# pangenome/smoothxg

Hardware: AMD Instinct MI355X
Metric: POA blocks/sec (+ DP cells/sec) on 1000-block synthetic (higher is better)
Workload: dtype int16

## Files before the change

### include/sxg_poa.h

```cpp
#ifndef SXG_POA_H
#define SXG_POA_H
#include <stdint.h>

#ifdef __cplusplus
extern "C" {
#endif

#define SXG_POA_ABI_VERSION 5

#define SXG_MODE_LOCAL 0
#define SXG_MODE_GLOBAL 1
#define SXG_ORDER_SPOA 0x10

#define SXG_OK 0
#define SXG_E_INVALID (-1)
#define SXG_E_NODEVICE (-2)
#define SXG_E_NOMEM (-3)
#define SXG_E_BLOCK (-4)
#define SXG_NOT_ROOT 1

#define SXG_ST_OK 0
#define SXG_ST_ROWS_OVERFLOW 1
#define SXG_ST_POOL_OVERFLOW 2
#define SXG_ST_TBX_OVERFLOW 3
#define SXG_ST_NODES_OVERFLOW 4
#define SXG_ST_TOO_LONG 5
#define SXG_ST_RANGE_OVERFLOW 6
#define SXG_ST_INTERNAL 8
#define SXG_ST_BAND_MISS 7

#define SXG_POA_MAX_SEQ_LEN 26623
#define SXG_POA_MAX_SEQ_LEN_WIDE 12287

typedef struct sxg_poa_params {
    int8_t m, n, g, e, q, c;
    uint8_t mode;
    uint8_t banded;
} sxg_poa_params;

typedef struct sxg_poa_handle sxg_poa_handle;

typedef struct sxg_poa_batch_in {
    int32_t n_blocks;
    const int32_t *blk_off;
    const int64_t *seq_off;
    const uint8_t *bases;
    const uint32_t *weights;
    const sxg_poa_params *params;
    int32_t per_block_params;
    int32_t want_consensus;
    int32_t want_msa;
    int32_t want_block_graph;
    int32_t bg_consensus_visited_only;
    const int32_t *bg_trim;
} sxg_poa_batch_in;

typedef struct sxg_poa_batch_out {
    int32_t n_blocks;
    int64_t n_seqs;
    int32_t *status;
    int64_t *node_off;
    uint8_t *node_code;
    int32_t *node_rank;
    int32_t *node_group;
    int64_t *edge_off;
    int32_t *edge_tail;
    int32_t *edge_head;
    uint32_t *edge_weight;
    int32_t *seq_path_nodes;
    int32_t *score;
    uint64_t *cells;
    int64_t *cons_off;
    int32_t *cons_nodes;
    int64_t *msa_off;
    int32_t *msa_cols;
    char *msa;
    int64_t *bg_node_off;
    int32_t *bg_node_len;
    int32_t *bg_node_outdeg;
    uint8_t *bg_node_indeg;
    int64_t *bg_seq_off;
    char *bg_seq;
    int64_t *bg_edge_off;
    int32_t *bg_edge_to;
    int64_t *bg_step_off;
    int32_t *bg_steps;
    int64_t *bg_cons_off;
    int32_t *bg_cons_steps;
    uint64_t *block_cycles;
    void *_owner;
} sxg_poa_batch_out;

typedef struct sxg_poa_align_in {
    int32_t n;
    const int64_t *row_off;
    const uint8_t *row_code;
    const uint8_t *row_sink;
    const int64_t *pred_off;
    const int32_t *preds;
    const int64_t *seq_off;
    const uint8_t *bases;
    const sxg_poa_params *params;
    int32_t per_problem_params;
} sxg_poa_align_in;

typedef struct sxg_poa_align_out {
    int32_t n;
    int32_t *status;
    int32_t *score;
    int64_t *pair_off;
    int32_t *pair_row;
    int32_t *pair_pos;
    void *_owner;
} sxg_poa_align_out;

typedef struct sxg_poa_stats {
    double kernel_ms;
    uint64_t cells;
    uint64_t dp_launches;
    uint64_t algo_bytes;
    int32_t n_slots;
    int32_t retries;
    uint64_t device_bytes;
    double dom_kernel_ms;
    uint64_t dom_cells, dom_algo_bytes;
    int32_t dom_threads, dom_cols_per_lane;
    int32_t dom_row_mode;
    int32_t dom_clock_mhz;
    double bg_ms;
} sxg_poa_stats;

int sxg_poa_abi_version(void);
int sxg_poa_measure_copy(sxg_poa_handle *h, uint64_t bytes, int reps, double *gbps);
int sxg_poa_roctx_available(void);
int sxg_poa_device_count(void);
const char *sxg_poa_last_error(void);

int sxg_poa_create(int device, sxg_poa_handle **out);
void sxg_poa_destroy(sxg_poa_handle *h);

int sxg_poa_batch_run(sxg_poa_handle *h, const sxg_poa_batch_in *in, sxg_poa_batch_out *out);
int sxg_poa_batch_upload(sxg_poa_handle *h, const sxg_poa_batch_in *in);
int sxg_poa_batch_execute(sxg_poa_handle *h);
int sxg_poa_batch_download(sxg_poa_handle *h, sxg_poa_batch_out *out);
void sxg_poa_batch_free(sxg_poa_batch_out *out);

typedef struct sxg_poa_device_view {
    int32_t n_blocks;
    int64_t n_seqs, n_bases;
    const int32_t *status, *n_nodes, *n_edges;
    const uint8_t *node_code;
    const int32_t *node_rank, *node_group;
    const int32_t *edge_tail, *edge_head;
    const uint32_t *edge_weight;
    const int32_t *seq_path_nodes;
    const int32_t *score;
} sxg_poa_device_view;
int sxg_poa_batch_device_view(sxg_poa_handle *h, sxg_poa_device_view *out);

#define SXG_POA_COMM_ID_BYTES 128
int sxg_poa_comm_unique_id(uint8_t *id);
int sxg_poa_comm_init(sxg_poa_handle *h, const uint8_t *id, int nranks, int rank);
int sxg_poa_comm_attach(sxg_poa_handle *h, void *nccl_comm, int nranks, int rank);
void sxg_poa_comm_destroy(sxg_poa_handle *h);
int sxg_poa_batch_run_sharded(sxg_poa_handle *h, const sxg_poa_batch_in *in, sxg_poa_batch_out *out);
int sxg_poa_batch_upload_sharded(sxg_poa_handle *h, const sxg_poa_batch_in *in);
int sxg_poa_batch_execute_sharded(sxg_poa_handle *h);
int sxg_poa_batch_download_sharded(sxg_poa_handle *h, const sxg_poa_batch_in *in, sxg_poa_batch_out *out);
int sxg_poa_sharded_info(sxg_poa_handle *h, int32_t *ranks_seen, uint64_t *bytes_received);
int sxg_poa_sharded_timing(sxg_poa_handle *h, double *pack_ms, double *exchange_ms);
int sxg_poa_batch_run_sharded_local(sxg_poa_handle *h, const sxg_poa_batch_in *in, int nranks, sxg_poa_batch_out *out);

int sxg_poa_align_batch(sxg_poa_handle *h, const sxg_poa_align_in *in, sxg_poa_align_out *out);
void sxg_poa_align_free(sxg_poa_align_out *out);

#define SXG_POA_SPLIT_PANEL 512
int sxg_poa_pair_identity_batch(sxg_poa_handle *h, int64_t n_seqs, const int64_t *seq_off, const uint8_t *bases, int64_t n_pairs,
                                const int32_t *pair_a, const int32_t *pair_b, const uint8_t *b_rev, const int32_t *cap,
                                int32_t *penalty, int32_t *cols, int32_t *matches);
typedef struct sxg_poa_split_in {
    int32_t n_blocks;
    const int32_t *blk_off;
    const int64_t *seq_off;
    const uint8_t *bases;
    const double *identity;
    const double *length_ratio_min;
} sxg_poa_split_in;
typedef struct sxg_poa_split_out {
    int32_t n_blocks;
    int64_t n_seqs;
    int32_t *group;
    int32_t *n_groups;
    int64_t *n_pairs;
    int32_t *status;
    void *_owner;
} sxg_poa_split_out;
int sxg_poa_split_batch(sxg_poa_handle *h, const sxg_poa_split_in *in, sxg_poa_split_out *out);
void sxg_poa_split_free(sxg_poa_split_out *out);

#define SXG_POA_MASH_SORT_TILE 1024
int sxg_poa_kmer_jaccard_batch(sxg_poa_handle *h, int64_t n_seqs, const int64_t *seq_off, const uint8_t *bases, int32_t kmer_size,
                               int64_t n_pairs, const int32_t *pair_a, const int32_t *pair_b,
                               int32_t *set_size, int32_t *inter, uint64_t *kmers);
typedef struct sxg_poa_split_mash {
    int32_t kmer_size;
    const int32_t *min_len;
    const double *est_identity;
} sxg_poa_split_mash;
int sxg_poa_split_mash_batch(sxg_poa_handle *h, const sxg_poa_split_in *in, const sxg_poa_split_mash *mash,
                             sxg_poa_split_out *out, int64_t *n_mash);

#define SXG_POA_SGD_LDS_NODES 8192
#define SXG_POA_SGD_LDS_TERMS (1ull << 30)
typedef struct sxg_poa_sgd_in {
    int64_t n_nodes; const int32_t *node_len;
    int64_t n_paths; const int64_t *path_off;
    const int32_t *step_node; const int64_t *step_pos;
    int32_t iter_max, cooling_start; const double *eta;
    uint64_t terms_per_iter, seed;
    int32_t mode;
} sxg_poa_sgd_in;
int sxg_poa_path_sgd_order(sxg_poa_handle *h, const sxg_poa_sgd_in *in, int32_t *order, int64_t *x);

int sxg_poa_get_stats(sxg_poa_handle *h, sxg_poa_stats *out);
int sxg_poa_set_memory_budget(sxg_poa_handle *h, uint64_t bytes);

uint64_t sxg_xxh64(const void *data, uint64_t len, uint64_t seed);

#ifdef __cplusplus
}
#endif
#endif
```

### smoothxg_amd/csrc/poa_classes.h

```cpp
#pragma once

struct Variant {
    int W, NW, TMAX, RM;
    int CB = 4;
    bool DS = false;
    constexpr int T() const { return 64 * NW; }
    constexpr int Lpad() const { return 64 * NW * W * (RM >= 2 ? 2 : 1); }
    constexpr bool operator==(const Variant& o) const { return W == o.W && NW == o.NW && TMAX == o.TMAX && RM == o.RM && CB == o.CB && DS == o.DS; }
    constexpr bool operator!=(const Variant& o) const { return !(*this == o); }
};
constexpr bool same_kind(const Variant& a, const Variant& b) { return a.RM == b.RM && a.CB == b.CB && a.DS == b.DS; }

struct ClassTraits {
    int rp;
    int tfix;
    int min_waves;
    int graph_batch;
};
constexpr ClassTraits class_traits(int TMAX, int W, int RM, int CB) {
    const bool p2 = RM == 2 && CB == 2;
    ClassTraits t{};
    t.rp = (p2 && TMAX <= 128) ? ((TMAX == 64 && W <= 11) ? 2 : 1) : 0;
#ifdef SXG_DEV_TFIX128
    t.tfix = (p2 && TMAX <= 512) ? TMAX : 0;
#else
    t.tfix = (p2 && TMAX <= 512 && TMAX != 128) ? TMAX : 0;
#endif
#ifdef SXG_DEV_WAVES
    t.min_waves = SXG_DEV_WAVES;
#else
    t.min_waves = TMAX > 512 ? 4 : (RM == 2 ? 4 : (W <= 12 ? 4 : 3));
#endif
    t.graph_batch = TMAX == 64 ? 16 : (TMAX <= 128 ? 8 : 4);
    return t;
}

enum ClassKind { CLASS_BLOCK = 0, CLASS_ALIGN = 1 };
enum : unsigned { CLS_LOCAL = 1, CLS_GLOBAL = 2, CLS_BOTH = 3, CLS_DS = 4 };
struct ClassRow { int part; ClassKind kind; unsigned rms; int cb, tmax; unsigned widths, modes; };
constexpr unsigned cw(int w) { return 1u << w; }
constexpr unsigned RM0 = cw(0), RM1 = cw(1), RM2 = cw(2), RM3 = cw(3), RM01 = RM0 | RM1;
constexpr unsigned cw_range(int lo, int hi) { unsigned m = 0; for (int w = lo; w <= hi; ++w) m |= cw(w); return m; }
constexpr int CLASS_W_MIN = 4, CLASS_W_MAX = 16, CLASS_RM_MAX = 3, CLASS_PARTS = 9;
constexpr ClassRow kClasses[] = {
    {1, CLASS_BLOCK, RM3, 2, 64, cw(6) | cw(8) | cw(11), CLS_LOCAL},
    {1, CLASS_BLOCK, RM3, 4, 64, cw(6) | cw(8) | cw(11), CLS_BOTH},
    {1, CLASS_BLOCK, RM01, 4, 256, cw(8) | cw(12) | cw(16), CLS_BOTH},
    {1, CLASS_BLOCK, RM01, 4, 512, cw(8) | cw(12) | cw(16), CLS_BOTH},
    {1, CLASS_BLOCK, RM01, 4, 1024, cw(8) | cw(12), CLS_BOTH},
    {1, CLASS_ALIGN, RM01, 4, 256, cw(8) | cw(12) | cw(16), CLS_BOTH},
    {1, CLASS_ALIGN, RM01, 4, 512, cw(8) | cw(12) | cw(16), CLS_BOTH},
    {1, CLASS_ALIGN, RM01, 4, 1024, cw(8) | cw(12), CLS_BOTH},
    {2, CLASS_BLOCK, RM2, 2, 256, cw_range(4, 12), CLS_BOTH | CLS_DS},
    {3, CLASS_BLOCK, RM2, 2, 512, cw_range(8, 12), CLS_BOTH | CLS_DS},
    {3, CLASS_BLOCK, RM2, 2, 1024, cw(8), CLS_BOTH | CLS_DS},
    {3, CLASS_BLOCK, RM2, 2, 1024, cw(10) | cw(12) | cw(13), CLS_LOCAL | CLS_DS},
    {4, CLASS_BLOCK, RM2, 4, 256, cw_range(4, 12), CLS_BOTH},
    {5, CLASS_BLOCK, RM2, 4, 512, cw_range(8, 12), CLS_BOTH},
    {5, CLASS_BLOCK, RM2, 4, 1024, cw(8), CLS_BOTH},
    {5, CLASS_BLOCK, RM2, 4, 1024, cw(10) | cw(12) | cw(13), CLS_LOCAL},
    {6, CLASS_ALIGN, RM2, 4, 256, cw_range(4, 12), CLS_BOTH},
    {6, CLASS_ALIGN, RM2, 4, 512, cw_range(8, 12), CLS_BOTH},
    {6, CLASS_ALIGN, RM2, 4, 1024, cw(8), CLS_BOTH},
    {6, CLASS_ALIGN, RM2, 4, 1024, cw(10) | cw(12) | cw(13), CLS_LOCAL},
    {7, CLASS_BLOCK, RM2, 2, 128, cw_range(4, 12), CLS_BOTH | CLS_DS},
    {8, CLASS_BLOCK, RM2, 2, 64, cw_range(4, 12), CLS_BOTH | CLS_DS},
    {9, CLASS_BLOCK, RM2, 2, 192, cw_range(4, 12), CLS_BOTH | CLS_DS},
};
constexpr int kNumClasses = (int)(sizeof(kClasses) / sizeof(kClasses[0]));

constexpr int class_row(ClassKind kind, const Variant& v, bool sw) {
    if (v.W < CLASS_W_MIN || v.W > CLASS_W_MAX || v.RM < 0 || v.RM > CLASS_RM_MAX) return -1;
    for (int r = 0; r < kNumClasses; ++r) {
        const ClassRow& c = kClasses[r];
        if (c.kind == kind && (c.rms & cw(v.RM)) && c.cb == v.CB && c.tmax == v.TMAX && (c.widths & cw(v.W)) && (c.modes & (sw ? CLS_LOCAL : CLS_GLOBAL)))
            return r;
    }
    return -1;
}
constexpr bool class_built(const Variant& v, bool , bool sw, ClassKind kind = CLASS_BLOCK) { return class_row(kind, v, sw) >= 0; }

constexpr int class_tmax(int W, int NW, int RM, int CB, bool full_plane) {
    if (RM == 3) return 64;
    int t = NW <= 4 ? 256 : (NW <= 8 ? 512 : 1024);
    if (RM == 2 && CB == 2 && NW <= 4) t = 64 * NW;
    if (class_traits(t, W, RM, CB).rp == 2 && !full_plane) t = 128;
    return t;
}

constexpr bool variant_for_len(int maxlen, int rm, Variant* v, bool sw = false, int cb = 4, int force_w = 0, int force_nw = 0) {
    constexpr int kNW[] = {1, 2, 3, 4, 8, 12, 16};
    if (rm == 2 && force_w > 0 && 128L * force_nw * force_w >= maxlen + 1 && (force_nw <= 4 || force_nw == 8 || force_nw == 12 || force_nw == 16)) {
        *v = Variant{force_w, force_nw, class_tmax(force_w, force_nw, rm, cb, true), rm, cb};
        return true;
    }
    constexpr int kW32[] = {16, 12, 8}, kW16[] = {13, 12, 11, 10, 9, 8, 7, 6, 5, 4};
    const int* ws = rm == 2 ? kW16 : kW32;
    const int nws = rm == 2 ? 10 : 3;
    const int need = maxlen + 1;
    long best_cols = -1;
    for (int wi = 0; wi < nws; ++wi)
        for (int NW : kNW) {
            const int W = ws[wi];
            const long cols = 64L * NW * W * (rm == 2 ? 2 : 1);
            if (cols < need) continue;
            const bool wide = rm == 2 ? W > 8 : W > 12;
            const bool long_class = rm == 2 && sw && NW == 16 && (W == 10 || W == 12 || W == 13);
            if (W == 13 && !long_class) continue;
            if (rm == 2 && W < 8 && NW > 4) continue;
            if (wide && NW > 8 && !long_class) continue;
            if (best_cols < 0 || cols < best_cols) {
                best_cols = cols;
                *v = Variant{W, NW, class_tmax(W, NW, rm, cb, true), rm, cb};
            }
            break;
        }
    return best_cols >= 0;
}
```

### smoothxg_amd/csrc/poa_kern_tables.hip.h

```cpp
#pragma once
#include <type_traits>
#include <utility>

#include "poa_kernels.hip.h"

template <class Args> using KernelFn = void (*)(const Args);
template <class Args> constexpr ClassKind kind_of = std::is_same_v<Args, AlignArgs> ? CLASS_ALIGN : CLASS_BLOCK;

template <class Args, int PART> KernelFn<Args> sxg_part_kernel(const Variant& v, bool cvx, bool sw);

#if defined(SXG_KERN_PART) || defined(SXG_DEV_ONLY_W)
template <class Args, int PART, int R, int W, int RM> constexpr bool class_here() {
    constexpr ClassRow c = kClasses[R];
#ifdef SXG_DEV_ONLY_W
#ifdef SXG_DEV_CB4
    constexpr bool dev = c.kind == CLASS_BLOCK && RM == 2 && c.tmax == SXG_DEV_ONLY_TMAX && W == SXG_DEV_ONLY_W;
#else
    constexpr bool dev = c.kind == CLASS_BLOCK && RM == 2 && c.cb == 2 && c.tmax == SXG_DEV_ONLY_TMAX && W == SXG_DEV_ONLY_W;
#endif
#else
    constexpr bool dev = true;
#endif
    return dev && c.part == PART && c.kind == kind_of<Args> && (c.widths & cw(W)) != 0 && (c.rms & cw(RM)) != 0;
}
template <class Args, int R, int W, int RM, bool CVX, bool SW, bool DS> static KernelFn<Args> class_kernel() {
    constexpr ClassRow c = kClasses[R];
    if constexpr (std::is_same_v<Args, AlignArgs>) return poa_align_kernel<c.tmax, W, CVX, RM, SW>;
    else return poa_block_kernel<c.tmax, W, CVX, RM, SW, c.cb, DS>;
}
template <class Args, int R, int W, int RM> static KernelFn<Args> pick_mode(bool cvx, bool sw, bool ds) {
    constexpr unsigned m = kClasses[R].modes;
    if constexpr ((m & CLS_DS) != 0) {
        if (cvx && ds) {
            if constexpr ((m & CLS_LOCAL) != 0) if (sw) return class_kernel<Args, R, W, RM, true, true, true>();
            if constexpr ((m & CLS_GLOBAL) != 0) if (!sw) return class_kernel<Args, R, W, RM, true, false, true>();
        }
    }
    if (cvx) {
        if constexpr ((m & CLS_LOCAL) != 0) if (sw) return class_kernel<Args, R, W, RM, true, true, false>();
        if constexpr ((m & CLS_GLOBAL) != 0) if (!sw) return class_kernel<Args, R, W, RM, true, false, false>();
    } else {
        if constexpr ((m & CLS_LOCAL) != 0) if (sw) return class_kernel<Args, R, W, RM, false, true, false>();
        if constexpr ((m & CLS_GLOBAL) != 0) if (!sw) return class_kernel<Args, R, W, RM, false, false, false>();
    }
    return nullptr;
}
template <int N, int... I> using rev_seq = std::integer_sequence<int, (N - 1 - I)...>;
template <int N, int... I> constexpr rev_seq<N, I...> rev_of(std::integer_sequence<int, I...>) { return {}; }
template <int N> constexpr auto rev_range() { return rev_of<N>(std::make_integer_sequence<int, N>()); }
template <class Args, int PART, int R, int W, int... RM> static void pick_rm(KernelFn<Args>& k, int row, const Variant& v, bool cvx, bool sw, std::integer_sequence<int, RM...>) {
    ((void)([&] { if constexpr (class_here<Args, PART, R, W, RM>()) if (row == R && v.W == W && v.RM == RM) k = pick_mode<Args, R, W, RM>(cvx, sw, v.DS); }()), ...);
}
template <class Args, int PART, int R, int... Wo> static void pick_width(KernelFn<Args>& k, int row, const Variant& v, bool cvx, bool sw, std::integer_sequence<int, Wo...>) {
    (pick_rm<Args, PART, R, CLASS_W_MIN + Wo>(k, row, v, cvx, sw, rev_range<CLASS_RM_MAX + 1>()), ...);
}
template <class Args, int PART, int... R> static KernelFn<Args> pick_class(const Variant& v, bool cvx, bool sw, std::integer_sequence<int, R...>) {
    KernelFn<Args> k = nullptr;
    const int row = class_row(kind_of<Args>, v, sw);
    (pick_width<Args, PART, R>(k, row, v, cvx, sw, rev_range<CLASS_W_MAX - CLASS_W_MIN + 1>()), ...);
    return k;
}
template <class Args, int PART> KernelFn<Args> sxg_part_kernel(const Variant& v, bool cvx, bool sw) {
    return pick_class<Args, PART>(v, cvx, sw, rev_range<kNumClasses>());
}
#endif
#ifdef SXG_KERN_PART
template KernelFn<BlockArgs> sxg_part_kernel<BlockArgs, SXG_KERN_PART>(const Variant&, bool, bool);
template KernelFn<AlignArgs> sxg_part_kernel<AlignArgs, SXG_KERN_PART>(const Variant&, bool, bool);
#endif

#ifndef SXG_KERN_PART
template <class Args, int... P> static KernelFn<Args> kernel_of(const Variant& v, bool cvx, bool sw, std::integer_sequence<int, P...>) {
    const int row = class_row(kind_of<Args>, v, sw);
    KernelFn<Args> k = nullptr;
    if (row >= 0) ((void)(kClasses[row].part == P + 1 ? (k = sxg_part_kernel<Args, P + 1>(v, cvx, sw), 0) : 0), ...);
    return k;
}
static inline KernelFn<BlockArgs> block_kernel(const Variant& v, bool cvx, bool sw) { return kernel_of<BlockArgs>(v, cvx, sw, std::make_integer_sequence<int, CLASS_PARTS>()); }
static inline KernelFn<AlignArgs> align_kernel(const Variant& v, bool cvx, bool sw) { return kernel_of<AlignArgs>(v, cvx, sw, std::make_integer_sequence<int, CLASS_PARTS>()); }
#endif
```

### smoothxg_amd/csrc/poa_kernels.hip.h

```cpp
#pragma once
#include <hip/hip_runtime.h>
#include <algorithm>
#include <cstring>

#include "../../include/sxg_poa.h"
#include "poa_classes.h"
#include "poa_dp.hip.h"
#include "poa_dp16.hip.h"
#include "poa_band16.hip.h"
#include "poa_graph_dev.h"
#include "poa_bgraph_dev.h"

using namespace sxg;


struct SlotLayout {
    size_t hdr, code, rank, order, order_tmp, leader, gmem, in_head, in_tail, out_head, out_tail, in_deg,
        out_deg, e_tail, e_head, e_next_in, e_next_out, e_w, posnode, target, newidx, nexta, preva, slotadd,
        kind, xpos, via, dfs_stack, dfs_rec, sp_rank, sp_first, sp_cnt, r_code, r_flags, r_pred_off, r_preds, r_slot, r_tbx, r_sseq, r_row_node, r_meta, tb, steps, pool,
        row0, park, cons_sc, cons_pr, pair_row, pair_pos, total;
    int nodes_cap, rows_cap, pool_slots, step_cap, scratch_len, Lpad, word_bytes, threads;
    int band_strips;
    int lds_rows;
};

inline size_t lay(size_t& cur, size_t bytes) {
    size_t o = cur;
    cur += (bytes + 255) & ~(size_t)255;
    return o;
}

inline SlotLayout make_layout(int nodes_cap, int rows_cap, int pool_slots, int step_cap, int threads, int Lpad,
                              int word_bytes, bool pairs, int band_strips = 0, int cell_bytes = 4, bool spoa_scratch = false) {
    SlotLayout L;
    memset(&L, 0, sizeof(L));
    L.nodes_cap = nodes_cap; L.rows_cap = rows_cap; L.pool_slots = pool_slots;
    L.step_cap = step_cap; L.threads = threads; L.Lpad = Lpad; L.word_bytes = word_bytes;
    L.band_strips = band_strips;
    const bool packed = band_strips > 0;
    const size_t C = (size_t)nodes_cap + 4, S = (size_t)std::max(nodes_cap, Lpad) + 4, Rr = (size_t)rows_cap + 4;
    L.scratch_len = (int)S;
    size_t cur = 0;
    L.hdr = lay(cur, 512);
    L.code = lay(cur, C);
    L.rank = lay(cur, 4 * C); L.order = lay(cur, 4 * C); L.order_tmp = lay(cur, 4 * C); L.leader = lay(cur, 4 * C);
    L.gmem = lay(cur, 20 * C);
    L.in_head = lay(cur, 4 * C); L.in_tail = lay(cur, 4 * C); L.out_head = lay(cur, 4 * C);
    L.out_tail = lay(cur, 4 * C); L.in_deg = lay(cur, 4 * C); L.out_deg = lay(cur, 4 * C);
    L.e_tail = lay(cur, 4 * C); L.e_head = lay(cur, 4 * C); L.e_next_in = lay(cur, 4 * C);
    L.e_next_out = lay(cur, 4 * C); L.e_w = lay(cur, 4 * C);
    L.posnode = lay(cur, 4 * S); L.target = lay(cur, 4 * S); L.newidx = lay(cur, 4 * S);
    L.nexta = lay(cur, 4 * S); L.preva = lay(cur, 4 * S); L.slotadd = lay(cur, 4 * S); L.kind = lay(cur, S);
    L.xpos = lay(cur, 4 * C);
    L.via = lay(cur, 4 * C);
    L.dfs_stack = lay(cur, spoa_scratch ? 4 * (7 * C + 8) : 256);
    L.dfs_rec = lay(cur, spoa_scratch ? 64 * C : 256);
    L.sp_rank = lay(cur, spoa_scratch ? 4 * C : 256); L.sp_first = lay(cur, spoa_scratch ? 4 * C : 256); L.sp_cnt = lay(cur, spoa_scratch ? 4 * C : 256);
    L.r_code = lay(cur, Rr); L.r_flags = lay(cur, Rr); L.r_pred_off = lay(cur, 4 * Rr);
    L.r_preds = lay(cur, 4 * C); L.r_slot = lay(cur, 4 * Rr); L.r_tbx = lay(cur, 4 * Rr);
    L.r_sseq = lay(cur, 4 * Rr); L.r_row_node = lay(cur, 4 * Rr); L.r_meta = lay(cur, 32 * Rr);
    L.tb = lay(cur, ((size_t)rows_cap + 1) * (packed ? (size_t)band_strips * (size_t)p16_slot_dwords(Lpad / (2 * threads), cell_bytes) * 4 : (size_t)Lpad));
    L.steps = lay(cur, packed ? 256 : (size_t)std::max(step_cap, 1) * 3 * threads * 4);
    const size_t row_bytes = (size_t)Lpad * (packed && cell_bytes == 2 ? 2 : word_bytes) + (size_t)threads * 4;
    L.pool = lay(cur, (size_t)pool_slots * row_bytes);
    L.row0 = lay(cur, row_bytes);
    L.park = lay(cur, (size_t)Lpad * word_bytes);
    L.cons_sc = lay(cur, 8 * C); L.cons_pr = lay(cur, 4 * C);
    if (pairs) { L.pair_row = lay(cur, 4 * (Rr + Lpad)); L.pair_pos = lay(cur, 4 * (Rr + Lpad)); }
    L.total = cur;
    return L;
}

struct SlotViews {
    GraphView G;
    RowsView R;
    DpBuffers B;
    int64_t* cons_sc;
    int32_t* cons_pr;
    int32_t *pair_row, *pair_pos;
};

__device__ static SlotViews slot_views(uint8_t* base, const SlotLayout& L) {
    SlotViews V;
    SXG_GP int32_t* hdr = (SXG_GP int32_t*)(base + L.hdr);
    V.G.n_nodes = hdr; V.G.n_edges = hdr + 1;
    V.G.code = (SXG_GP uint8_t*)(base + L.code);
#define P32(f) (SXG_GP int32_t*)(base + L.f)
    V.G.rank = P32(rank); V.G.order = P32(order); V.G.order_tmp = P32(order_tmp); V.G.leader = P32(leader);
    V.G.gmem = P32(gmem); V.G.in_head = P32(in_head); V.G.in_tail = P32(in_tail); V.G.out_head = P32(out_head);
    V.G.out_tail = P32(out_tail); V.G.in_deg = P32(in_deg); V.G.out_deg = P32(out_deg);
    V.G.e_tail = P32(e_tail); V.G.e_head = P32(e_head); V.G.e_next_in = P32(e_next_in);
    V.G.e_next_out = P32(e_next_out); V.G.e_w = (SXG_GP uint32_t*)(base + L.e_w);
    V.G.posnode = P32(posnode); V.G.target = P32(target); V.G.newidx = P32(newidx); V.G.nexta = P32(nexta);
    V.G.preva = P32(preva); V.G.slotadd = P32(slotadd); V.G.kind = (SXG_GP int8_t*)(base + L.kind);
    V.G.xpos = P32(xpos); V.G.via = P32(via); V.G.dfs_stack = P32(dfs_stack); V.G.dfs_rec = P32(dfs_rec);
    V.G.sp_rank = P32(sp_rank); V.G.sp_first = P32(sp_first); V.G.sp_cnt = P32(sp_cnt);
    V.R.code = (SXG_GP uint8_t*)(base + L.r_code); V.R.flags = (SXG_GP uint8_t*)(base + L.r_flags); V.R.pred_off = P32(r_pred_off);
    V.R.preds = P32(r_preds); V.R.slot = P32(r_slot); V.R.tbx = P32(r_tbx); V.R.sseq = P32(r_sseq);
    V.R.row_node = P32(r_row_node); V.R.meta = P32(r_meta);
    V.B.tb = base + L.tb; V.B.steps = (uint32_t*)(base + L.steps);
    V.B.pool = base + L.pool; V.B.row0 = base + L.row0; V.B.park = base + L.park;
    V.B.band_strips = L.band_strips; V.B.lds_rows = L.lds_rows;
    V.cons_sc = (int64_t*)(base + L.cons_sc); V.cons_pr = (int32_t*)(base + L.cons_pr);
    V.pair_row = (int32_t*)(base + L.pair_row); V.pair_pos = (int32_t*)(base + L.pair_pos);
#undef P32
    return V;
}

__host__ __device__ static inline Scoring normalise(const sxg_poa_params& p) {
    Scoring S;
    S.m = p.m; S.n = p.n; S.g = p.g; S.e = p.e; S.q = p.q; S.c = p.c;
    S.sw = (p.mode & 1) == SXG_MODE_LOCAL;
    S.convex = 0;
    if (S.g >= S.e) { S.e = S.g; S.q = S.g; S.c = S.g; }
    else if (S.g <= S.q || S.e >= S.c) { S.q = S.g; S.c = S.e; }
    else S.convex = 1;
    return S;
}

struct BlockArgs {
    const int32_t* blk_off; const int64_t* seq_off; const uint8_t* bases; const uint32_t* weights;
    const sxg_poa_params* params; int per_block_params;
    const int32_t* work; int n_work; int32_t* queue;
    uint8_t* arena; SlotLayout lay;
    int32_t* status; int32_t* n_nodes; int32_t* n_edges; int32_t* n_cons;
    uint8_t* node_code; int32_t* node_rank; int32_t* node_group;
    int32_t* edge_tail; int32_t* edge_head; uint32_t* edge_weight;
    int32_t* paths; int32_t* score; unsigned long long* cells; int32_t* cons_nodes;
    int want_consensus;
    int park_in_lds;
    int pf_off;
    int num_cu;
    uint32_t* prio_board;
    int prio_base;
    const unsigned long long* est;
    int lds_bytes;
    unsigned long long* blk_cycles;
    int band_floor, band_margin, band_full;
};

__host__ __device__ constexpr int sxg_min_waves(int TMAX, int W, int RM) { return class_traits(TMAX, W, RM, 4).min_waves; }

template <int TMAX, int W, bool CVX, int RM, bool SW, int CB = 4, bool DS = false>
__global__ __launch_bounds__(TMAX, sxg_min_waves(TMAX, W, RM)) void poa_block_kernel(const BlockArgs A) {
    constexpr bool H16 = RM != 1;
    constexpr int CPL = RM >= 2 ? 2 * W : W;
    constexpr ClassTraits CT = class_traits(TMAX, W, RM, CB);
    const int T = (int)blockDim.x;
    extern __shared__ __attribute__((aligned(16))) char smem[];
    int* lds = (int*)smem;
    int& s_work = lds[200];
    WgCtx ctx{(sxg_lds_int*)(size_t)((unsigned)__builtin_amdgcn_groupstaticsize() + 128u * 4u)};
    const int t = threadIdx.x;
    SlotViews V = slot_views(A.arena + (size_t)blockIdx.x * A.lay.total, A.lay);
    V.B.prio_rank = (int)(blockIdx.x / (unsigned)A.num_cu + (unsigned)A.prio_base) & (PRIO_BOARD_SLOTS - 1);
    V.B.prio_board = A.prio_board ? A.prio_board + (size_t)(__smid() & (PRIO_BOARD_CUS - 1)) * PRIO_BOARD_SLOTS : nullptr;
    const RowCaps caps{A.lay.rows_cap, A.lay.pool_slots, A.lay.step_cap, A.lay.lds_rows};
    bool first = true;
    for (;;) {
        __syncthreads();
        if (t == 0) s_work = first ? (int)blockIdx.x : (int)gridDim.x + atomicAdd(A.queue, 1);
        first = false;
        __syncthreads();
        const int wi = s_work;
        if (wi >= A.n_work) break;
        const int b = A.work[wi];
        const unsigned long long est_total = A.est ? A.est[wi] : 0ull;
        unsigned long long done_cells = 0;
        const int s0 = A.blk_off[b], s1 = A.blk_off[b + 1];
        const int64_t base0 = A.seq_off[s0];
        const Scoring S = normalise(A.params[A.per_block_params ? b : 0]);
        if (t == 0) { *V.G.n_nodes = 0; *V.G.n_edges = 0; }
        __syncthreads();
        int status = ST_OK;
        unsigned long long* prof = (unsigned long long*)(A.arena + (size_t)blockIdx.x * A.lay.total + A.lay.hdr + 64);
        V.B.row_prof = prof + 28;
        if ((t & 63) == 0) {
            prof[10 + (t >> 6)] = ((unsigned long long)__smid() << 32) | (unsigned long long)__builtin_amdgcn_s_getreg(GETREG_IMMED(31, 0, HW_ID));
            if (t == 0 && prof[8] == 0) { prof[8] = (unsigned long long)wall_clock64(); prof[6] = (unsigned long long)clock64(); }
        }
        unsigned long long tc0 = clock64(), tc1;
        const unsigned long long tblk0 = tc0;
        int band_drift = 0, band_min = 0;
#define PROF(k) do { if (t == 0) { tc1 = clock64(); prof[k] += tc1 - tc0; tc0 = tc1; } } while (0)
        for (int s = s0; s < s1 && status == ST_OK; ++s) {
            const int64_t so = A.seq_off[s];
            const int len = (int)(A.seq_off[s + 1] - so);
            const uint8_t* seq = A.bases + so;
            for (int i = t; i < len; i += T) V.G.posnode[i] = -1;
            __syncthreads();
            const int N = *V.G.n_nodes;
            int score = 0;
            if (RM != 3 && len + 1 > T * CPL) { status = ST_TOO_LONG; break; }
            if (N + len > A.lay.nodes_cap || *V.G.n_edges + len > A.lay.nodes_cap) { status = ST_NODES_OVERFLOW; break; }
            if (RM != 1 && RM != 2 && !S.sw &&
                -(sxg_gap_cost(S.g, S.e, S.q, S.c, N) + sxg_gap_cost(S.g, S.e, S.q, S.c, len)) >= (RM >= 2 ? 15800 : 30000)) {
                status = ST_RANGE_OVERFLOW;
                break;
            }
            if (N > 0 && len > 0) {
                PROF(0);
                const int band_mode = RM == 3 ? (int)A.params[A.per_block_params ? b : 0].banded : 0;
                const int hinted_ = RM == 3 ? (band_mode == 2 ? 3 : 2) : (RM == 2 ? 1 : 0);
                if (CT.graph_batch == 16 || (CT.graph_batch == 8 && T <= 64)) { WgCtxT<16> c16{ctx.lds}; status = prep_rows(c16, V.G, V.R, caps, hinted_); }
                else if (CT.graph_batch == 8) { WgCtxT<8> c8{ctx.lds}; status = prep_rows(c8, V.G, V.R, caps, hinted_); }
                else status = prep_rows(ctx, V.G, V.R, caps, hinted_);
                if (status != ST_OK) break;
                PROF(1);
                DpResult res;
                V.B.prio_rem0 = est_total > done_cells ? est_total - done_cells : 0ull;
                if constexpr (RM == 3) {
                    V.B.band_w = band_half_width(len);
                    V.B.band_mode = band_mode;
                    res = dp_fill_band16<CVX, W, SW, SW ? CB : 4>(S, V.R, N, seq, len, V.B, smem, A.cells + s);
                    __syncthreads();
                    PROF(2);
                    if (t == 0) lds[TBM_FLAG] = 0;
                    __syncthreads();
                    if (res.bi >= 0)
                        traceback_p16<false, W, CVX, true, SW ? CB : 4>(V.R, V.B, S, seq, len, res.best, T, min(256, (len << 8) / max(N, 1)), res.bi, res.bj,
                                                                        V.G.posnode, nullptr, nullptr, smem);
                    __syncthreads();
                    PROF(3);
                    if (lds[TBM_FLAG]) { status = ST_INTERNAL; break; }
                } else if constexpr (RM == 2) {
                    const int bs_cap = A.lay.band_strips;
                    int bs = bs_cap;
                    if (A.band_floor > 0 && bs_cap < 2 * T && s - s0 > A.band_full)
                        bs = max(p16_drift_strips(band_drift, A.band_margin, W, A.band_floor, bs_cap), band_min);
                    for (int att = 0;; ++att) {
                        V.B.band_strips = bs;
                        if (t == 0) { prof[47] += (unsigned long long)bs; prof[48] += 1; }
#ifdef SXG_EXP
                        if (att == 0) { res = dp_fill_p16<W, CVX, SW, CB, CT.rp, CT.tfix, DS, SXG_EXP>(S, V.R, N, seq, len, V.B, smem); __syncthreads(); if (res.best == 0x7fffffff) break; }
#endif
                        res = dp_fill_p16<W, CVX, SW, CB, CT.rp, CT.tfix, DS>(S, V.R, N, seq, len, V.B, smem);
                        __syncthreads();
                        PROF(2);
                        if (t == 0) { lds[TBM_FLAG] = 0; lds[TBM_RANGE] = 0; }
                        __syncthreads();
                        if (t < 64 && res.bi >= 0)
                            traceback_p16<false, W, CVX, false, CB>(V.R, V.B, S, seq, len, res.best, T, min(256, (len << 8) / max(N, 1)), res.bi, res.bj,
                                                                    V.G.posnode, nullptr, nullptr, smem);
                        __syncthreads();
                        PROF(3);
                        if (lds[TBM_RANGE]) { status = ST_RANGE_OVERFLOW; break; }
                        if (!lds[TBM_FLAG]) break;
                        if (att == 5) { status = ST_BAND_MISS; break; }
                        const int mrow = lds[TBM_ROW], mdelta = lds[TBM_DELTA];
                        __syncthreads();
                        for (int r2 = t; r2 < mrow; r2 += T) V.R.meta[8 * (size_t)r2 + 7] += mdelta;
                        for (int i2 = t; i2 < len; i2 += T) V.G.posnode[i2] = -1;
                        if (t == 0) prof[27] += 1;
                        band_min = bs = min(plane_round4(2 * bs), bs_cap);
                        __syncthreads();
                    }
                    if (status != ST_OK) break;
                    if (A.band_floor > 0 && bs_cap < 2 * T) {
                        int d = 0;
                        for (int j2 = t; j2 < len; j2 += T) {
                            const int v = V.G.posnode[j2];
                            if (v >= 0) d = max(d, abs(j2 + 1 - V.G.xpos[v]));
                        }
                        band_drift = max(band_drift, ctx.reduce_max(d));
                    }
                } else {
                    dp_fill<W, CVX, H16, SW>(S, V.R, N, seq, len, V.B, smem, A.park_in_lds != 0, A.pf_off, res);
                    __syncthreads();
                    PROF(2);
                    if (t == 0 && res.bi >= 0) traceback<false>(V.R, V.B, T, W, S.sw, res.bi, res.bj, V.G.posnode, nullptr, nullptr);
                    __syncthreads();
                    PROF(3);
                }
                score = res.bi >= 0 ? res.best : 0;
            }
            if (t == 0) { A.score[s] = score; if (RM != 3 || N == 0 || len == 0) A.cells[s] = RM == 3 ? 0ull : (unsigned long long)N * (unsigned long long)len; }
            done_cells += (unsigned long long)N * (unsigned long long)len;
            const bool spoa_order = (A.params[A.per_block_params ? b : 0].mode & SXG_ORDER_SPOA) != 0;
            if (CT.graph_batch == 16 || (CT.graph_batch == 8 && T <= 64)) { WgCtxT<16> c16{ctx.lds}; add_alignment(c16, V.G, seq, len, A.weights ? A.weights[s] : 1u, A.paths + so, !spoa_order); }
            else if (CT.graph_batch == 8) { WgCtxT<8> c8{ctx.lds}; add_alignment(c8, V.G, seq, len, A.weights ? A.weights[s] : 1u, A.paths + so, !spoa_order); }
            else add_alignment(ctx, V.G, seq, len, A.weights ? A.weights[s] : 1u, A.paths + so, !spoa_order);
            if (spoa_order) {
                typedef __attribute__((address_space(3))) uint8_t lds_u8;
                spoa_resort(ctx, V.G, (lds_u8*)(size_t)((unsigned)__builtin_amdgcn_groupstaticsize() + (unsigned)LDS_CTL_BYTES), A.lds_bytes - LDS_CTL_BYTES,
                            (int)(A.seq_off[s0 + 1] - A.seq_off[s0]), len, N, s == s0, prof + 41);
                __syncthreads();
            }
            PROF(4);
        }
        PROF(0);
        __syncthreads();
        const int N = *V.G.n_nodes, E = *V.G.n_edges;
        if (status == ST_OK) {
            for (int v = t; v < N; v += T) {
                A.node_code[base0 + v] = V.G.code[v];
                A.node_rank[base0 + v] = V.G.rank[v];
                A.node_group[base0 + v] = V.G.leader[v];
            }
            for (int e = t; e < E; e += T) {
                A.edge_tail[base0 + e] = V.G.e_tail[e];
                A.edge_head[base0 + e] = V.G.e_head[e];
                A.edge_weight[base0 + e] = V.G.e_w[e];
            }
            int nc = 0;
            if (A.want_consensus && t == 0) nc = consensus_serial(V.G, V.cons_sc, V.cons_pr, A.cons_nodes + base0);
            if (t == 0) { A.n_nodes[b] = N; A.n_edges[b] = E; A.n_cons[b] = nc; }
        } else if (t == 0) { A.n_nodes[b] = 0; A.n_edges[b] = 0; A.n_cons[b] = 0; }
        if (t == 0) { A.status[b] = status; if (A.blk_cycles) A.blk_cycles[b] = (unsigned long long)clock64() - tblk0; }
        if (t == 0 && V.B.prio_board) __hip_atomic_store(V.B.prio_board + V.B.prio_rank, 0u, __ATOMIC_RELAXED, __HIP_MEMORY_SCOPE_AGENT);
        PROF(5);
        if (t == 0) { prof[9] = (unsigned long long)wall_clock64(); prof[7] = (unsigned long long)clock64(); }
#undef PROF
    }
}

struct AlignArgs {
    const int64_t* row_off; const uint8_t* row_code; const uint8_t* row_sink; const int64_t* pred_off;
    const int32_t* preds; const int64_t* seq_off; const uint8_t* bases; const sxg_poa_params* params;
    int per_problem_params;
    const int32_t* work; int n_work; int32_t* queue;
    uint8_t* arena; SlotLayout lay;
    int32_t* status; int32_t* score; int32_t* n_pairs;
    int32_t* pair_row; int32_t* pair_pos;
    int park_in_lds;
    int pf_off;
    int num_cu;
};

template <int TMAX, int W, bool CVX, int RM, bool SW>
__global__ __launch_bounds__(TMAX, sxg_min_waves(TMAX, W, RM)) void poa_align_kernel(const AlignArgs A) {
    constexpr bool H16 = RM != 1;
    constexpr int CPL = RM == 2 ? 2 * W : W;
    const int T = (int)blockDim.x;
    extern __shared__ __attribute__((aligned(16))) char smem[];
    int* lds = (int*)smem;
    int& s_work = lds[200];
    WgCtx ctx{(sxg_lds_int*)(size_t)((unsigned)__builtin_amdgcn_groupstaticsize() + 128u * 4u)};
    const int t = threadIdx.x;
    SlotViews V = slot_views(A.arena + (size_t)blockIdx.x * A.lay.total, A.lay);
    V.B.prio_rank = (int)(blockIdx.x / (unsigned)A.num_cu) & (PRIO_BOARD_SLOTS - 1);
    V.B.prio_board = nullptr; V.B.prio_rem0 = 0; V.B.row_prof = nullptr;
    const RowCaps caps{A.lay.rows_cap, A.lay.pool_slots, A.lay.step_cap, A.lay.lds_rows};
    for (;;) {
        __syncthreads();
        if (t == 0) s_work = atomicAdd(A.queue, 1);
        __syncthreads();
        const int wi = s_work;
        if (wi >= A.n_work) break;
        const int p = A.work[wi];
        const int64_t r0 = A.row_off[p];
        const int N = (int)(A.row_off[p + 1] - r0);
        const int64_t so = A.seq_off[p];
        const int len = (int)(A.seq_off[p + 1] - so);
        const Scoring S = normalise(A.params[A.per_problem_params ? p : 0]);
        const int64_t e0 = A.pred_off[r0];
        int status = ST_OK, score = 0, npairs = 0;
        if (len + 1 > T * CPL) status = ST_TOO_LONG;
        else if (N > A.lay.rows_cap) status = ST_ROWS_OVERFLOW;
        else if (N > 0 && len > 0) {
            for (int r = t; r < N; r += T) {
                V.R.code[r] = A.row_code[r0 + r];
                V.R.pred_off[r] = (int)(A.pred_off[r0 + r] - e0);
                V.R.row_node[r] = r;
                V.R.slot[r] = r;
                V.R.tbx[r] = 0;
                int fl = A.row_sink[r0 + r] ? ROW_SINK : 0;
                for (int64_t k = A.pred_off[r0 + r]; k < A.pred_off[r0 + r + 1]; ++k)
                    if (A.preds[k] == r) fl |= ROW_REGPRED;
                V.R.flags[r] = (uint8_t)fl;
            }
            if (t == 0) V.R.pred_off[N] = (int)(A.pred_off[r0 + N] - e0);
            __syncthreads();
            const int E = V.R.pred_off[N];
            for (int k = t; k < E; k += T) V.R.preds[k] = A.preds[e0 + k];
            __syncthreads();
            for (int r = t; r < N; r += T)
                for (int k = V.R.pred_off[r]; k < V.R.pred_off[r + 1]; ++k) {
                    const int pr = V.R.preds[k];
                    if (pr >= 1 && pr != r) {
                        atomicOr((unsigned*)(V.R.flags + ((pr - 1) & ~3)), (unsigned)ROW_STORE << (8 * ((pr - 1) & 3)));
                        atomicMax(&V.R.slot[pr - 1], r);
                    }
                }
            status = finish_rows(ctx, N, V.R, caps, RM == 2 ? 1 : 0);
            if (status == ST_OK) {
                DpResult res;
                if constexpr (RM == 2) res = dp_fill_p16<W, CVX, SW, 4>(S, V.R, N, A.bases + so, len, V.B, smem);
                else dp_fill<W, CVX, H16, SW>(S, V.R, N, A.bases + so, len, V.B, smem, A.park_in_lds != 0, A.pf_off, res);
                __syncthreads();
                if constexpr (RM == 2) {
                    if (t == 0) { lds[TBM_FLAG] = 0; lds[TBM_RANGE] = 0; }
                    __syncthreads();
                    if (t < 64 && res.bi >= 0) npairs = traceback_p16<true, W, CVX, false, 4, true>(V.R, V.B, S, A.bases + so, len, res.best, T, min(256, (len << 8) / max(N, 1)), res.bi, res.bj, nullptr, V.pair_row, V.pair_pos, smem);
                    __syncthreads();
                    if (lds[TBM_FLAG]) status = ST_BAND_MISS;
                    else if (lds[TBM_RANGE]) status = ST_RANGE_OVERFLOW;
                } else if (t == 0 && res.bi >= 0) npairs = traceback<true>(V.R, V.B, T, W, S.sw, res.bi, res.bj, nullptr, V.pair_row, V.pair_pos);
                if (t == 0 && res.bi >= 0 && status == ST_OK) {
                    score = res.best;
                    const int64_t out0 = A.row_off[p] + A.seq_off[p];
                    for (int k = 0; k < npairs; ++k) {
                        A.pair_row[out0 + k] = V.pair_row[npairs - 1 - k] - 1;
                        A.pair_pos[out0 + k] = V.pair_pos[npairs - 1 - k];
                    }
                }
            }
        }
        if (t == 0) { A.status[p] = status; A.score[p] = score; A.n_pairs[p] = npairs; }
    }
}
```

### smoothxg_amd/csrc/sxg_poa.hip

```cpp
#include <hip/hip_runtime.h>
#include <algorithm>
#include <chrono>
#include <cmath>
#include <cstdio>
#include <cstdlib>
#include <cstring>
#include <memory>
#include <new>
#include <string>
#include <sys/mman.h>
#include <thread>
#include <vector>

#include "../../include/sxg_poa.h"
#include <rccl/rccl.h>
#include <dlfcn.h>
#include "poa_kernels.hip.h"
#include "poa_kern_tables.hip.h"
#include "poa_split.hip.h"
#include "poa_mash.hip.h"
#include "poa_sgd.hip.h"


struct BgArgs {
    const int32_t* blk_off; const int64_t* seq_off; const uint8_t* bases; const int32_t* paths;
    const uint8_t* node_code; const int32_t* edge_tail; const int32_t* edge_head; const int32_t* cons;
    const int32_t *nn, *ne, *nc; const int32_t* trim; int cons_mode;
    const int32_t* work; int n_work; int32_t* queue;
    uint8_t* arena; size_t slot_bytes; int capV, capE, capC, capT;
    const int64_t *node_o, *edge_o;
    int32_t *o_len, *o_outdeg; uint8_t* o_indeg; char* o_seq; int32_t* o_eto; int32_t* o_steps; int32_t* o_nsteps;
    int32_t* o_cons; int32_t* o_counts;
};
constexpr int BG_THREADS = 256, BG_HEAP = 3072;
static size_t bg_slot_bytes(int capV, int capE, int capC, int capT) {
    return 4 * (27 * ((size_t)capV + 2) + 3 * ((size_t)capE + capC + 2) + ((size_t)capC + 2) + ((size_t)capT + 2) + 4) + 256;
}
struct BgCtx : WgCtx {
    int* hp;
    __device__ __forceinline__ int load_fresh(const int32_t* p) const { return __hip_atomic_load(p, __ATOMIC_RELAXED, __HIP_MEMORY_SCOPE_AGENT); }
    __device__ __forceinline__ int* heap() const { return hp; }
    __device__ __forceinline__ int heap_cap() const { return BG_HEAP; }
};
__global__ __launch_bounds__(BG_THREADS) void block_graph_kernel(const BgArgs A) {
    __shared__ int s_scan[64];
    __shared__ int s_heap[BG_HEAP];
    __shared__ int s_work;
    BgCtx ctx;
    ctx.lds = (sxg_lds_int*)s_scan;
    ctx.hp = s_heap;
    const int t = threadIdx.x;
    int32_t* w = (int32_t*)(A.arena + (size_t)blockIdx.x * A.slot_bytes);
    const size_t C = (size_t)A.capV + 2, EC = (size_t)A.capE + A.capC + 2;
    BgScratch W;
    auto take = [&](size_t n) { int32_t* q = w; w += n; return q; };
    W.vis = take(C); W.front = take(C); W.back = take(C); W.ecnt = take(C); W.eoff = take(C);
    W.ehead = take(EC); W.eused = take(EC);
    W.outdeg = take(C); W.indeg = take(C); W.only = take(C); W.nxt = take(C); W.prv = take(C);
    W.pj0 = take(C); W.pj1 = take(C); W.pd0 = take(C); W.pd1 = take(C); W.cid = take(C);
    W.head_of = take(C); W.tail_of = take(C); W.clen = take(C); W.indc = take(C); W.coff = take(C); W.newid = take(C);
    W.csucc = take(EC); W.cc = take((size_t)A.capC + 2); W.tmp = take((size_t)A.capT + 2);
    W.lenN = take(C); W.odN = take(C); W.soffN = take(C); W.eoffN = take(C); W.flag = take(4);
    for (;;) {
        __syncthreads();
        if (t == 0) s_work = atomicAdd(A.queue, 1);
        __syncthreads();
        const int wi = s_work;
        if (wi >= A.n_work) break;
        const int b = A.work[wi];
        const int s0 = A.blk_off[b], s1 = A.blk_off[b + 1];
        const int64_t base0 = A.seq_off[s0];
        BgIn I;
        I.node_code = A.node_code + base0; I.V = A.nn[b]; I.E = A.ne[b];
        I.e_tail = A.edge_tail + base0; I.e_head = A.edge_head + base0;
        I.paths = A.paths + base0; I.bases = A.bases + base0; I.seq_off = A.seq_off; I.s0 = s0; I.s1 = s1;
        I.trim = A.trim ? A.trim[b] : 0;
        I.cons = A.cons ? A.cons + base0 : nullptr; I.n_cons = A.cons ? A.nc[b] : 0; I.cons_mode = A.cons ? A.cons_mode : 0;
        BgOut O;
        const int64_t no = A.node_o[b], eo = A.edge_o[b];
        O.node_len = A.o_len + no; O.node_outdeg = A.o_outdeg + no; O.node_indeg = A.o_indeg + no; O.seq = A.o_seq + no;
        O.eto = A.o_eto + eo; O.steps = A.o_steps + base0; O.nsteps = A.o_nsteps + s0; O.cons_steps = A.o_cons + no;
        O.counts = A.o_counts + (size_t)BGC_N * b;
        block_graph(ctx, I, W, O);
    }
}

__global__ void clamp_bases_kernel(uint8_t* bases, const int64_t n) {
    const int64_t n16 = (n + 15) / 16;
    for (int64_t i = (int64_t)blockIdx.x * blockDim.x + threadIdx.x; i < n16; i += (int64_t)gridDim.x * blockDim.x) {
        u32x4 v = ((const u32x4*)bases)[i];
        unsigned w[4] = {v.x, v.y, v.z, v.w};
        bool any = false;
#pragma unroll
        for (int k = 0; k < 4; ++k) {
            unsigned o = 0;
#pragma unroll
            for (int b = 0; b < 4; ++b) { const unsigned c = (w[k] >> (8 * b)) & 0xffu; o |= (c > 4u ? 4u : c) << (8 * b); }
            any |= o != w[k];
            w[k] = o;
        }
        if (any) ((u32x4*)bases)[i] = u32x4{w[0], w[1], w[2], w[3]};
    }
}

template <class Tv>
__global__ void gather_kernel(const Tv* __restrict__ src, Tv* __restrict__ dst, const int64_t* __restrict__ src_off,
                              const int64_t* __restrict__ dst_off, int n) {
    for (int b = blockIdx.x; b < n; b += gridDim.x) {
        const int64_t s = src_off[b], d = dst_off[b], cnt = dst_off[b + 1] - d;
        for (int64_t i = threadIdx.x; i < cnt; i += blockDim.x) dst[d + i] = src[s + i];
    }
}


static thread_local std::string g_err;
#include <mutex>
static std::mutex g_err_mu;
static std::string g_err_any;
static thread_local std::string g_err_ret;
static int fail(int code, const std::string& msg) {
    g_err = msg;
    { std::lock_guard<std::mutex> lk(g_err_mu); g_err_any = msg; }
    return code;
}
#define HIPCHK(x)                                                                              \
    do {                                                                                       \
        hipError_t _e = (x);                                                                   \
        if (_e != hipSuccess)                                                                  \
            return fail(_e == hipErrorOutOfMemory ? SXG_E_NOMEM : SXG_E_NODEVICE,              \
                        std::string(#x) + ": " + hipGetErrorString(_e));                       \
    } while (0)

static int p16_lds_rows(const int T, const int W, const int CB) {
    if (const char* e = getenv("SXG_POA_LDS_ROWS")) return std::max(0, std::min(8, atoi(e)));
    const int wg_per_cu = std::max(1, 16 / std::max(T / 64, 1));
    const int share = (160 * 1024) / wg_per_cu - 512;
    const int rows = (share - dp16_lds_bytes(T, W, 0, CB)) / dp16_row_bytes(T, W, CB);
    return std::max(0, std::min(8, rows));
}

static int plane_cell_bytes(const Scoring& S) {
    if (const char* e = getenv("SXG_POA_CELL_BYTES")) if (atoi(e) == 4) return 4;
    return p16_delta_fits(S) ? 2 : 4;
}
static int band_cell_bytes(const Scoring& S) {
    if (const char* e = getenv("SXG_POA_BAND_CELL_BYTES")) if (atoi(e) == 4) return 4;
    return S.sw ? plane_cell_bytes(S) : 4;
}

static long score_floor(const Scoring& S, int maxlen, int rows) {
    if (S.sw) return 0;
    return -(sxg_gap_cost(S.g, S.e, S.q, S.c, rows) + sxg_gap_cost(S.g, S.e, S.q, S.c, maxlen));
}
static bool h16_safe(const Scoring& S, int maxlen, int rows) {
    return (long)std::abs(S.m) * maxlen < 30000 && score_floor(S, maxlen, rows) < 30000;
}
static bool p16_safe(const Scoring& S, int maxlen, int rows, bool clamp_ok = false) {
    if (getenv("SXG_POA_NO_PACKED")) return false;
    if (std::abs(S.g) > 120 || std::abs(S.q) > 120) return false;
    if (S.sw) return (long)std::abs(S.m) * maxlen < 30000;
    if ((long)std::abs(S.m) * maxlen >= 15800) return false;
    if (clamp_ok && !getenv("SXG_POA_NO_NW_CLAMP")) return (long)std::abs(S.m) * maxlen + std::abs(S.m) < 14500;
    return score_floor(S, maxlen, rows) < 15800;
}
static int row_mode(const Scoring& S, int maxlen, int rows, int at_least = 2, bool clamp_ok = false) {
    if (at_least == 2 && p16_safe(S, maxlen, rows, clamp_ok)) return 2;
    if (at_least != 1 && h16_safe(S, maxlen, rows)) return 0;
    return 1;
}

static void forced_p16(int* w, int* nw) {
    *w = *nw = 0;
    if (const char* e = getenv("SXG_POA_FORCE_P16"))
        if (sscanf(e, "%d,%d", w, nw) != 2) *w = *nw = 0;
}

struct HostLaps {
    bool on = getenv("SXG_POA_DEBUG") != nullptr;
    std::chrono::steady_clock::time_point t0 = std::chrono::steady_clock::now();
    void lap(const char* what) {
        if (!on) return;
        const auto t1 = std::chrono::steady_clock::now();
        fprintf(stderr, "[sxg] host %-22s %.3f ms\n", what, std::chrono::duration<double, std::milli>(t1 - t0).count());
        t0 = t1;
    }
};

struct DevBuf {
    void* p = nullptr;
    size_t cap = 0;
    int ensure(size_t bytes) {
        if (bytes <= cap) return SXG_OK;
        if (p) { (void)hipFree(p); p = nullptr; cap = 0; }
        size_t want = bytes + bytes / 8 + 256;
        hipError_t e = hipMalloc(&p, want);
        if (e != hipSuccess) {
            want = bytes;
            e = hipMalloc(&p, want);
        }
        if (e != hipSuccess) { p = nullptr; return fail(SXG_E_NOMEM, "hipMalloc failed for " + std::to_string(bytes) + " bytes"); }
        cap = want;
        return SXG_OK;
    }
    void release() { if (p) (void)hipFree(p); p = nullptr; cap = 0; }
    template <class Tp> Tp* as() const { return (Tp*)p; }
};

struct BlockMeta {
    int maxlen = 0, nseq = 0, rm = 0; bool fits = false; Variant variant{16, 1, 256, 0};
    int tier = 0;
    bool wide_band = false;
    bool no_wide = false;
    int64_t sumlen = 0;
    double cost = 0;
    bool cvx = false, sw = true;
    Scoring S;
};

static void classify_block(BlockMeta& m, int at_least, bool clamp_ok) {
    m.rm = row_mode(m.S, m.maxlen, m.maxlen, at_least, clamp_ok);
    const int cb = m.rm == 2 ? plane_cell_bytes(m.S) : 4;
    int fw, fnw;
    forced_p16(&fw, &fnw);
    m.fits = variant_for_len(m.maxlen, m.rm, &m.variant, m.S.sw, cb, fw, fnw);
    m.variant.CB = cb;
    m.variant.DS = m.rm == 2 && cb == 2 && p16_default_scores(m.S) && !getenv("SXG_POA_NO_DEFAULT_CLASS");
}

struct PlanRes {
    DevBuf arena, work, queue, est;
    hipStream_t stream = nullptr;
    hipEvent_t e0 = nullptr, e1 = nullptr;
};

struct PinPool {
    struct Buf { void* p; size_t cap; bool busy; };
    std::mutex mu;
    std::vector<Buf> bufs;
    void* acquire(size_t bytes) {
        std::lock_guard<std::mutex> g(mu);
        for (auto& b : bufs) if (!b.busy && b.cap >= bytes) { b.busy = true; return b.p; }
        for (size_t i = 0; i < bufs.size(); ++i)
            if (!bufs[i].busy) { (void)hipHostFree(bufs[i].p); bufs.erase(bufs.begin() + (long)i); break; }
        if (bufs.size() >= 4) return nullptr;
        void* q = nullptr;
        const size_t cap = bytes + bytes / 8;
        if (hipHostMalloc(&q, cap, hipHostMallocDefault) != hipSuccess || !q) { (void)hipGetLastError(); return nullptr; }
        bufs.push_back(Buf{q, cap, true});
        return q;
    }
    void release(void* p) {
        std::lock_guard<std::mutex> g(mu);
        for (auto& b : bufs) if (b.p == p) b.busy = false;
    }
    void prewarm(size_t bytes) { if (void* p = acquire(bytes)) release(p); }
    ~PinPool() { for (auto& b : bufs) (void)hipHostFree(b.p); }
};
struct sxg_poa_handle {
    std::vector<PlanRes*> planres;
    int device = 0;
    hipStream_t stream = nullptr;
    hipEvent_t ev0 = nullptr, ev1 = nullptr;
    int num_cu = 256;
    uint64_t mem_budget = 0;
    bool have_batch = false, executed = false;
    int n_blocks = 0;
    int64_t n_seqs = 0, n_bases = 0;
    int want_consensus = 0, want_msa = 0, per_block_params = 0;
    std::vector<int32_t> h_blk_off;
    std::vector<int64_t> h_seq_off;
    std::vector<sxg_poa_params> h_params;
    std::vector<BlockMeta> meta;
    DevBuf d_blk_off, d_seq_off, d_bases, d_weights, d_params;
    bool has_weights = false;
    DevBuf d_status, d_nn, d_ne, d_nc, d_node_code, d_node_rank, d_node_group, d_edge_tail, d_edge_head, d_edge_w,
        d_paths, d_score, d_cells, d_cons, d_work, d_queue, d_arena, d_blk_cycles;
    DevBuf d_tmp_a, d_tmp_b, d_tmp_c, d_tmp_d;
    DevBuf d_board;
    int want_block_graph = 0, bg_cons_visited_only = 0;
    std::shared_ptr<PinPool> pins;
    std::thread pin_thread;
    bool bg_done = false;
    DevBuf d_trim, d_bg_no, d_bg_eo, d_bg_len, d_bg_od, d_bg_id, d_bg_seq, d_bg_eto, d_bg_steps, d_bg_nsteps, d_bg_cons, d_bg_counts,
        d_bg_work, d_bg_queue, d_bg_arena;
    std::vector<int64_t> bg_node_o, bg_edge_o;
    std::vector<int32_t> bg_counts;
    sxg_poa_stats stats{};
    ncclComm_t comm = nullptr;
    bool own_comm = false;
    int nranks = 1, rank = 0;
    DevBuf d_blob, d_recv, d_counts;
    std::vector<std::vector<int32_t>> sh_parts;
    std::vector<int64_t> sh_counts;
    std::vector<size_t> sh_at;
    bool sh_dealt = false, sh_exchanged = false;
    uint64_t sh_bytes_received = 0;
    int sh_ranks_seen = 0;
    double sh_pack_ms = 0, sh_exchange_ms = 0;
};

namespace {
struct Roctx {
    int (*push)(const char*) = nullptr;
    int (*pop)() = nullptr;
    Roctx() {
        if (getenv("SXG_POA_NO_ROCTX")) return;
        void* lib = dlopen("librocprofiler-sdk-roctx.so", RTLD_NOW | RTLD_GLOBAL);
        if (!lib) lib = dlopen("librocprofiler-sdk-roctx.so.1", RTLD_NOW | RTLD_GLOBAL);
        if (!lib) lib = dlopen("libroctx64.so", RTLD_NOW | RTLD_GLOBAL);
        if (!lib) lib = dlopen("libroctx64.so.4", RTLD_NOW | RTLD_GLOBAL);
        if (!lib) return;
        push = (int (*)(const char*))dlsym(lib, "roctxRangePushA");
        pop = (int (*)())dlsym(lib, "roctxRangePop");
        if (!push || !pop) { push = nullptr; pop = nullptr; }
    }
};
static Roctx& roctx() { static Roctx r; return r; }
struct RoctxRange {
    bool on;
    explicit RoctxRange(const char* name) : on(roctx().push != nullptr) { if (on) roctx().push(name); }
    ~RoctxRange() { if (on) roctx().pop(); }
    RoctxRange(const RoctxRange&) = delete;
    RoctxRange& operator=(const RoctxRange&) = delete;
};
}
extern "C" int sxg_poa_roctx_available(void) { return roctx().push != nullptr ? 1 : 0; }

__global__ __launch_bounds__(256) void sxg_copy_kernel(const u32x4* __restrict__ src, u32x4* __restrict__ dst, const size_t n16) {
    const size_t stride = (size_t)gridDim.x * blockDim.x;
    for (size_t i = (size_t)blockIdx.x * blockDim.x + threadIdx.x; i < n16; i += stride)
        __builtin_nontemporal_store(__builtin_nontemporal_load(src + i), dst + i);
}
extern "C" int sxg_poa_measure_copy(sxg_poa_handle* h, uint64_t bytes, int reps, double* gbps) {
    if (!h || !gbps) return fail(SXG_E_INVALID, "NULL argument");
    *gbps = 0;
    HIPCHK(hipSetDevice(h->device));
    const size_t n16 = (size_t)std::max<uint64_t>(bytes, 1u << 20) / 16;
    DevBuf a, b;
    if (int rc = a.ensure(n16 * 16)) return rc;
    if (int rc = b.ensure(n16 * 16)) return rc;
    HIPCHK(hipMemsetAsync(a.p, 1, n16 * 16, h->stream));
    hipEvent_t e0, e1;
    HIPCHK(hipEventCreate(&e0)); HIPCHK(hipEventCreate(&e1));
    const int grid = std::max(h->num_cu, 1) * 16;
    reps = std::max(reps, 1);
    hipLaunchKernelGGL(sxg_copy_kernel, dim3((unsigned)grid), dim3(256), 0, h->stream, a.as<u32x4>(), b.as<u32x4>(), n16);
    HIPCHK(hipEventRecord(e0, h->stream));
    for (int r = 0; r < reps; ++r)
        hipLaunchKernelGGL(sxg_copy_kernel, dim3((unsigned)grid), dim3(256), 0, h->stream, a.as<u32x4>(), b.as<u32x4>(), n16);
    HIPCHK(hipEventRecord(e1, h->stream));
    HIPCHK(hipEventSynchronize(e1));
    float ms = 0;
    HIPCHK(hipEventElapsedTime(&ms, e0, e1));
    (void)hipEventDestroy(e0); (void)hipEventDestroy(e1);
    a.release(); b.release();
    if (ms > 0) *gbps = 2.0 * (double)(n16 * 16) * reps / ((double)ms * 1e-3) / 1e9;
    return SXG_OK;
}

extern "C" int sxg_poa_abi_version(void) { return SXG_POA_ABI_VERSION; }
extern "C" const char* sxg_poa_last_error(void) {
    if (!g_err.empty()) return g_err.c_str();
    { std::lock_guard<std::mutex> lk(g_err_mu); g_err_ret = g_err_any; }
    return g_err_ret.c_str();
}
extern "C" int sxg_poa_device_count(void) {
    int n = 0;
    if (hipGetDeviceCount(&n) != hipSuccess) return 0;
    return n;
}

extern "C" int sxg_poa_create(int device, sxg_poa_handle** out) {
    if (!out) return fail(SXG_E_INVALID, "out is NULL");
    *out = nullptr;
    setenv("GPU_MAX_HW_QUEUES", "16", 0);
    int n = 0;
    if (hipGetDeviceCount(&n) != hipSuccess || n <= 0) return fail(SXG_E_NODEVICE, "no HIP device available");
    if (device < 0 || device >= n) return fail(SXG_E_INVALID, "device index out of range");
    HIPCHK(hipSetDevice(device));
    sxg_poa_handle* h = new sxg_poa_handle();
    h->device = device;
    h->pins = std::make_shared<PinPool>();
    hipDeviceProp_t prop;
    HIPCHK(hipGetDeviceProperties(&prop, device));
    h->num_cu = prop.multiProcessorCount;
    HIPCHK(hipStreamCreateWithFlags(&h->stream, hipStreamNonBlocking));
    HIPCHK(hipEventCreate(&h->ev0));
    HIPCHK(hipEventCreate(&h->ev1));
    *out = h;
    return SXG_OK;
}

static void release_all(sxg_poa_handle* h) {
    DevBuf* bufs[] = {&h->d_blk_off, &h->d_seq_off, &h->d_bases, &h->d_weights, &h->d_params, &h->d_status, &h->d_nn,
                      &h->d_ne, &h->d_nc, &h->d_node_code, &h->d_node_rank, &h->d_node_group, &h->d_edge_tail,
                      &h->d_edge_head, &h->d_edge_w, &h->d_paths, &h->d_score, &h->d_cells, &h->d_cons, &h->d_work,
                      &h->d_queue, &h->d_arena, &h->d_blk_cycles, &h->d_tmp_a, &h->d_tmp_b, &h->d_tmp_c, &h->d_tmp_d, &h->d_board, &h->d_trim, &h->d_bg_no, &h->d_bg_eo,
                      &h->d_bg_len, &h->d_bg_od, &h->d_bg_id, &h->d_bg_seq, &h->d_bg_eto, &h->d_bg_steps, &h->d_bg_nsteps, &h->d_bg_cons,
                      &h->d_bg_counts, &h->d_bg_work, &h->d_bg_queue, &h->d_bg_arena};
    for (DevBuf* b : bufs) b->release();
}

extern "C" void sxg_poa_comm_destroy(sxg_poa_handle* h);
extern "C" void sxg_poa_destroy(sxg_poa_handle* h) {
    if (!h) return;
    if (h->pin_thread.joinable()) h->pin_thread.join();
    (void)hipSetDevice(h->device);
    sxg_poa_comm_destroy(h);
    h->d_blob.release(); h->d_recv.release(); h->d_counts.release();
    release_all(h);
    for (PlanRes* r : h->planres) {
        r->arena.release(); r->work.release(); r->queue.release(); r->est.release();
        if (r->e0) (void)hipEventDestroy(r->e0);
        if (r->e1) (void)hipEventDestroy(r->e1);
        if (r->stream) (void)hipStreamDestroy(r->stream);
        delete r;
    }
    if (h->ev0) (void)hipEventDestroy(h->ev0);
    if (h->ev1) (void)hipEventDestroy(h->ev1);
    if (h->stream) (void)hipStreamDestroy(h->stream);
    delete h;
}

extern "C" int sxg_poa_set_memory_budget(sxg_poa_handle* h, uint64_t bytes) {
    if (!h) return fail(SXG_E_INVALID, "handle is NULL");
    h->mem_budget = bytes;
    return SXG_OK;
}

extern "C" int sxg_poa_get_stats(sxg_poa_handle* h, sxg_poa_stats* out) {
    if (!h || !out) return fail(SXG_E_INVALID, "NULL argument");
    *out = h->stats;
    return SXG_OK;
}

static uint64_t arena_budget(sxg_poa_handle* h) {
    size_t fr = 0, tot = 0;
    if (hipMemGetInfo(&fr, &tot) != hipSuccess) return 8ull << 30;
    uint64_t avail = (uint64_t)fr + h->d_arena.cap;
    for (PlanRes* r : h->planres) avail += r->arena.cap;
    uint64_t b = avail / 4 * 3;
    if (h->mem_budget && h->mem_budget < b) b = h->mem_budget;
    return b;
}

extern "C" int sxg_poa_batch_upload(sxg_poa_handle* h, const sxg_poa_batch_in* in) {
    if (!h || !in) return fail(SXG_E_INVALID, "NULL argument");
    if (in->n_blocks < 0 || (in->n_blocks > 0 && (!in->blk_off || !in->seq_off || !in->params)))
        return fail(SXG_E_INVALID, "batch_in has NULL arrays");
    HIPCHK(hipSetDevice(h->device));
    const RoctxRange range_("sxg_poa_batch_upload");
    HostLaps laps;
    h->have_batch = false; h->executed = false;
    const int nb = in->n_blocks;
    if (nb > 0 && in->blk_off[0] != 0) return fail(SXG_E_INVALID, "blk_off[0] must be 0");
    const int64_t ns = nb ? in->blk_off[nb] : 0;
    for (int b = 0; b < nb; ++b)
        if (in->blk_off[b + 1] < in->blk_off[b]) return fail(SXG_E_INVALID, "blk_off not monotone");
    if (ns > 0 && in->seq_off[0] != 0) return fail(SXG_E_INVALID, "seq_off[0] must be 0");
    for (int64_t s = 0; s < ns; ++s)
        if (in->seq_off[s + 1] < in->seq_off[s]) return fail(SXG_E_INVALID, "seq_off not monotone");
    const int64_t nbases = ns ? in->seq_off[ns] : 0;
    if (nbases > 0 && !in->bases) return fail(SXG_E_INVALID, "bases is NULL");
    const int np = in->per_block_params ? nb : 1;
    for (int k = 0; k < np && nb > 0; ++k) {
        const sxg_poa_params& p = in->params[k];
        if (p.m < 0 || p.n > 0 || p.g > 0 || p.e > 0 || p.q > 0 || p.c > 0 || (p.mode & ~(1 | SXG_ORDER_SPOA)) != 0 || p.banded > 2)
            return fail(SXG_E_INVALID, "scores must follow spoa's sign convention (m>=0, others <=0), mode 0|1");
    }
    h->n_blocks = nb; h->n_seqs = ns; h->n_bases = nbases;
    h->want_consensus = in->want_consensus; h->want_msa = in->want_msa;
    h->want_block_graph = in->want_block_graph < 0 || in->want_block_graph > 3 ? 0 : in->want_block_graph;
    if (h->want_block_graph >= 2 && in->want_msa) h->want_block_graph = 1;
    h->bg_cons_visited_only = in->bg_consensus_visited_only ? 1 : 0;
    h->bg_done = false;
    h->per_block_params = in->per_block_params;
    h->h_blk_off.assign(in->blk_off, in->blk_off + nb + 1);
    h->h_seq_off.assign(in->seq_off, in->seq_off + ns + 1);
    h->h_params.assign(in->params, in->params + np);
    h->meta.assign(nb, BlockMeta());
    for (int b = 0; b < nb; ++b) {
        BlockMeta& m = h->meta[b];
        m.S = normalise(h->h_params[in->per_block_params ? b : 0]);
        m.cvx = m.S.convex; m.sw = m.S.sw;
        m.nseq = in->blk_off[b + 1] - in->blk_off[b];
        double prev = 0;
        for (int s = in->blk_off[b]; s < in->blk_off[b + 1]; ++s) {
            const int64_t len = in->seq_off[s + 1] - in->seq_off[s];
            m.maxlen = (int)std::max<int64_t>(m.maxlen, len);
            m.sumlen += len;
            const double l1 = (double)(in->seq_off[in->blk_off[b] + 1] - in->seq_off[in->blk_off[b]]);
            if (s > in->blk_off[b]) m.cost += (double)len * (l1 + 0.05 * prev);
            prev += (double)len;
        }
        classify_block(m, 2, h->h_params[in->per_block_params ? b : 0].banded == 0);
        const int bnd = h->h_params[in->per_block_params ? b : 0].banded;
        if (bnd && (m.S.sw || bnd == 2) && m.rm == 2 && m.maxlen <= SXG_POA_MAX_SEQ_LEN) {
            m.rm = 3;
            const int bw = band_strip_width(m.maxlen), bcb = band_cell_bytes(m.S);
            m.variant = Variant{bw, 1, class_tmax(bw, 1, 3, bcb, true), 3, bcb};
            m.fits = true;
        }
    }
    laps.lap("upload: checks");
    const uint8_t* host_bases = in->bases;
    int rc;
    if ((rc = h->d_blk_off.ensure(4 * (size_t)(nb + 1)))) return rc;
    if ((rc = h->d_seq_off.ensure(8 * (size_t)(ns + 1)))) return rc;
    if ((rc = h->d_bases.ensure((size_t)nbases + 16))) return rc;
    if ((rc = h->d_params.ensure(sizeof(sxg_poa_params) * (size_t)std::max(np, 1)))) return rc;
    HIPCHK(hipMemcpyAsync(h->d_blk_off.p, in->blk_off, 4 * (size_t)(nb + 1), hipMemcpyHostToDevice, h->stream));
    HIPCHK(hipMemcpyAsync(h->d_seq_off.p, in->seq_off, 8 * (size_t)(ns + 1), hipMemcpyHostToDevice, h->stream));
    if (nbases) HIPCHK(hipMemcpyAsync(h->d_bases.p, host_bases, (size_t)nbases, hipMemcpyHostToDevice, h->stream));
    if (nbases) {
        hipLaunchKernelGGL(clamp_bases_kernel, dim3((unsigned)std::min<int64_t>((nbases / 16 + 255) / 256 + 1, 16384)), dim3(256), 0, h->stream,
                           h->d_bases.as<uint8_t>(), nbases);
        HIPCHK(hipGetLastError());
    }
    if (nb) HIPCHK(hipMemcpyAsync(h->d_params.p, in->params, sizeof(sxg_poa_params) * (size_t)np, hipMemcpyHostToDevice, h->stream));
    h->has_weights = in->weights != nullptr;
    if (h->has_weights) {
        if ((rc = h->d_weights.ensure(4 * (size_t)std::max<int64_t>(ns, 1)))) return rc;
        if (ns) HIPCHK(hipMemcpyAsync(h->d_weights.p, in->weights, 4 * (size_t)ns, hipMemcpyHostToDevice, h->stream));
    }
    if (h->want_block_graph) {
        std::vector<int32_t> trim((size_t)std::max(nb, 1), 0);
        for (int b = 0; b < nb; ++b) {
            trim[b] = in->bg_trim ? in->bg_trim[b] : 0;
            if (trim[b] < 0) return fail(SXG_E_INVALID, "bg_trim must not be negative");
        }
        if ((rc = h->d_trim.ensure(4 * trim.size()))) return rc;
        HIPCHK(hipMemcpy(h->d_trim.p, trim.data(), 4 * trim.size(), hipMemcpyHostToDevice));
    }
    const size_t NB = (size_t)std::max<int64_t>(nbases, 1), NS = (size_t)std::max<int64_t>(ns, 1), NBL = (size_t)std::max(nb, 1);
    if ((rc = h->d_status.ensure(4 * NBL)) || (rc = h->d_nn.ensure(4 * NBL)) || (rc = h->d_ne.ensure(4 * NBL)) ||
        (rc = h->d_nc.ensure(4 * NBL)) || (rc = h->d_node_code.ensure(NB)) || (rc = h->d_node_rank.ensure(4 * NB)) ||
        (rc = h->d_node_group.ensure(4 * NB)) || (rc = h->d_edge_tail.ensure(4 * NB)) ||
        (rc = h->d_edge_head.ensure(4 * NB)) || (rc = h->d_edge_w.ensure(4 * NB)) || (rc = h->d_paths.ensure(4 * NB)) ||
        (rc = h->d_score.ensure(4 * NS)) || (rc = h->d_cells.ensure(8 * NS)) || (rc = h->d_queue.ensure(256)) ||
        (rc = h->d_work.ensure(4 * NBL)) || (rc = h->d_blk_cycles.ensure(8 * NBL)))
        return rc;
    if (h->want_consensus && (rc = h->d_cons.ensure(4 * NB))) return rc;
    HIPCHK(hipStreamSynchronize(h->stream));
    laps.lap("upload: copies");
    h->have_batch = true;
    h->sh_dealt = false; h->sh_exchanged = false;
    return SXG_OK;
}

struct LaunchPlan {
    Variant variant; bool cvx, sw; int tier = 0; bool wide_band = false;
    std::vector<int32_t> work;
    std::vector<unsigned long long> est;
    SlotLayout lay; KernelFn<BlockArgs> kern = nullptr; std::string why; int per_cu = 1; int64_t want_slots = 0, n_slots = 0;
    int clock_mhz = 0;
    int smem = 0, pf_off = -1; bool park_lds = true; uint64_t cells = 0, bytes = 0; float ms = 0;
};

static int plane_strips_p16(int T, int W) {
    if (const char* e = getenv("SXG_POA_BAND_COLS")) {
        const int cols = std::max(atoi(e), W);
        return std::min(plane_round4((cols + W - 1) / W), 2 * T);
    }
    return p16_band_strips(T, W);
}

static void band_adapt_args(BlockArgs& A) {
    A.band_floor = P16_BAND_FLOOR; A.band_margin = P16_BAND_MARGIN; A.band_full = P16_BAND_FULL;
    if (const char* e = getenv("SXG_POA_BAND_ADAPT")) {
        int f = 0, m = A.band_margin, n = A.band_full;
        const int k = sscanf(e, "%d,%d,%d", &f, &m, &n);
        A.band_floor = k >= 1 && f > 0 ? plane_round4(f) : 0;
        if (k >= 2) A.band_margin = std::max(m, 0);
        if (k >= 3) A.band_full = std::max(n, 0);
    }
}

static void prepare_plan(sxg_poa_handle* h, LaunchPlan& P, int attempt) {
    const Variant V = P.variant;
    const int Lpad = V.Lpad();
    int nodes_cap = 0, maxlen = 0;
    bool any_adaptive = false;
    bool any_spoa = false;
    double rows_est = 0;
    for (int b : P.work) {
        const BlockMeta& m = h->meta[b];
        any_adaptive = any_adaptive || h->h_params[h->per_block_params ? b : 0].banded == 2;
        any_spoa = any_spoa || (h->h_params[h->per_block_params ? b : 0].mode & SXG_ORDER_SPOA) != 0;
        nodes_cap = (int)std::max<int64_t>(nodes_cap, m.sumlen);
        maxlen = std::max(maxlen, m.maxlen);
        rows_est = std::max(rows_est, (double)m.maxlen * std::max(2.0, 1.0 + 0.0165 * m.nseq));
    }
    nodes_cap += 8;
    const int nodes_full = nodes_cap;
    int rows_cap, pool_slots, step_cap;
    if (attempt == 0) {
        rows_cap = (int)std::min<double>(nodes_cap, rows_est + 1024);
        pool_slots = std::min(rows_cap + 1, 768);
        step_cap = rows_cap;
        nodes_cap = (int)std::min<int64_t>(nodes_full, 2LL * rows_cap + maxlen + 8);
    } else if (attempt == 1) {
        rows_cap = (int)std::min<double>(nodes_cap, 2.5 * rows_est + 4096);
        pool_slots = std::min(rows_cap + 1, 4096);
        step_cap = 3 * rows_cap;
        nodes_cap = (int)std::min<int64_t>(nodes_full, 2LL * rows_cap + maxlen + 8);
    } else if (attempt == 2) {
        rows_cap = nodes_cap; pool_slots = std::min(rows_cap + 1, 32768); step_cap = nodes_cap;
    } else {
        rows_cap = nodes_cap; pool_slots = rows_cap + 1; step_cap = nodes_cap;
    }
    if (rows_cap >= (1 << 20)) rows_cap = (1 << 20) - 1;
    const int wb = V.RM == 1 ? 8 : 4;
    if (V.RM == 3) pool_slots = 1;
    P.lay = make_layout(nodes_cap, rows_cap, pool_slots, step_cap, V.T(), Lpad, wb, false,
                        V.RM == 3 ? (any_adaptive ? BAND_WIN : band_plane_strips(maxlen, V.W)) : (V.RM == 2 ? (P.wide_band ? 2 * V.T() : plane_strips_p16(V.T(), V.W)) : 0),
                        V.RM >= 2 ? V.CB : 4, any_spoa);
    P.variant.TMAX = class_tmax(V.W, V.NW, V.RM, V.CB, P.lay.band_strips == 2 * V.T());
    P.kern = block_kernel(P.variant, P.cvx, P.sw);
    const int tfix = class_traits(P.variant.TMAX, V.W, V.RM, V.CB).tfix;
    if (tfix && tfix != V.T()) { P.kern = nullptr; P.why = "kernel class compiled for " + std::to_string(tfix) + " threads asked to run at " + std::to_string(V.T()); }
    if (!P.kern && P.why.empty()) P.why = "no kernel class built for this geometry";
    P.smem = dp_lds_launch_bytes(Lpad, wb);
    P.park_lds = dp_park_in_lds(Lpad, wb);
    if (V.RM == 2) { P.lay.lds_rows = p16_lds_rows(V.T(), V.W, V.CB); P.smem = dp16_lds_bytes(V.T(), V.W, P.lay.lds_rows, V.CB); P.park_lds = true; }
    if (V.RM == 3) { P.smem = band_lds_bytes(V.W); P.park_lds = true; }
    P.pf_off = (V.RM < 2 && getenv("SXG_POA_PREFETCH")) ? dp_pf_offset(Lpad, wb, V.T()) : -1;
    if (P.pf_off >= 0) P.smem += dp_pf_bytes(Lpad, wb, V.T());
    if (P.smem > 48 * 1024)
        (void)hipFuncSetAttribute((const void*)P.kern, hipFuncAttributeMaxDynamicSharedMemorySize, P.smem);
    P.per_cu = 1;
    if (hipOccupancyMaxActiveBlocksPerMultiprocessor(&P.per_cu, (const void*)P.kern, V.T(), (size_t)P.smem) != hipSuccess || P.per_cu < 1)
        P.per_cu = 1;
    P.want_slots = std::min<int64_t>((int64_t)P.work.size(), (int64_t)h->num_cu * P.per_cu);
}

static int sample_clock(const LaunchPlan& P, const PlanRes& R) {
    unsigned long long cyc = 0, ticks = 0;
    const int64_t step = std::max<int64_t>(1, P.n_slots / 24);
    for (int64_t sl = 0; sl < P.n_slots; sl += step) {
        unsigned long long v[10];
        if (hipMemcpy(v, R.arena.as<uint8_t>() + (size_t)sl * P.lay.total + P.lay.hdr + 64, sizeof(v), hipMemcpyDeviceToHost) != hipSuccess) return 0;
        if (v[9] <= v[8] || v[7] <= v[6]) continue;
        cyc += v[7] - v[6];
        ticks += v[9] - v[8];
    }
    return ticks ? (int)((double)cyc / (double)ticks * 100.0 + 0.5) : 0;
}

static int launch_plan(sxg_poa_handle* h, LaunchPlan& P, PlanRes& R, const int prio_base) {
    const Variant V = P.variant;
    int rc;
    if (!P.kern) return fail(SXG_E_INVALID, P.why);
    if ((rc = R.arena.ensure((size_t)P.n_slots * P.lay.total))) return rc;
    {
        const int64_t ns = P.n_slots, ncu = std::max(h->num_cu, 1);
        const int64_t rem = ns % ncu, full = ns / ncu;
        if (rem > 0 && full >= 1 && (int64_t)P.work.size() >= ns) {
            std::vector<int32_t> first((size_t)ns, -1);
            size_t next = 0;
            for (int64_t p = 0; p < ns; ++p)
                if (p % ncu >= rem && p / ncu < full) first[(size_t)p] = P.work[next++];
            for (int64_t round = 0; round <= full; ++round)
                for (int64_t c = 0; c < rem; ++c) {
                    const int64_t cu = (round & 1) ? rem - 1 - c : c, p = round * ncu + cu;
                    if (p < ns && first[(size_t)p] < 0) first[(size_t)p] = P.work[next++];
                }
            std::copy(first.begin(), first.end(), P.work.begin());
        }
    }
    if ((rc = R.work.ensure(4 * P.work.size())) || (rc = R.queue.ensure(256)) || (rc = R.est.ensure(8 * P.work.size()))) return rc;
    HIPCHK(hipMemcpyAsync(R.work.p, P.work.data(), 4 * P.work.size(), hipMemcpyHostToDevice, R.stream));
    P.est.resize(P.work.size());
    for (size_t k = 0; k < P.work.size(); ++k) P.est[k] = (unsigned long long)std::max(h->meta[P.work[k]].cost, 1.0);
    HIPCHK(hipMemcpyAsync(R.est.p, P.est.data(), 8 * P.est.size(), hipMemcpyHostToDevice, R.stream));
    HIPCHK(hipMemsetAsync(R.queue.p, 0, 256, R.stream));
    BlockArgs A;
    A.blk_off = h->d_blk_off.as<int32_t>(); A.seq_off = h->d_seq_off.as<int64_t>(); A.bases = h->d_bases.as<uint8_t>();
    A.weights = h->has_weights ? h->d_weights.as<uint32_t>() : nullptr;
    A.params = h->d_params.as<sxg_poa_params>(); A.per_block_params = h->per_block_params;
    A.work = R.work.as<int32_t>(); A.n_work = (int)P.work.size(); A.queue = R.queue.as<int32_t>();
    A.arena = R.arena.as<uint8_t>(); A.lay = P.lay;
    A.status = h->d_status.as<int32_t>(); A.n_nodes = h->d_nn.as<int32_t>(); A.n_edges = h->d_ne.as<int32_t>();
    A.n_cons = h->d_nc.as<int32_t>(); A.node_code = h->d_node_code.as<uint8_t>();
    A.node_rank = h->d_node_rank.as<int32_t>(); A.node_group = h->d_node_group.as<int32_t>();
    A.edge_tail = h->d_edge_tail.as<int32_t>(); A.edge_head = h->d_edge_head.as<int32_t>();
    A.edge_weight = h->d_edge_w.as<uint32_t>(); A.paths = h->d_paths.as<int32_t>(); A.score = h->d_score.as<int32_t>();
    A.cells = h->d_cells.as<unsigned long long>(); A.cons_nodes = h->d_cons.as<int32_t>();
    A.want_consensus = h->want_consensus;
    A.park_in_lds = P.park_lds ? 1 : 0;
    A.pf_off = P.pf_off;
    A.num_cu = std::max(h->num_cu, 1);
    A.prio_board = getenv("SXG_POA_NO_BALANCE") ? nullptr : h->d_board.as<uint32_t>();
    A.prio_base = prio_base;
    A.est = R.est.as<unsigned long long>();
    A.blk_cycles = h->d_blk_cycles.as<unsigned long long>();
    A.lds_bytes = getenv("SXG_POA_RESORT_NO_LDS") ? 0 : P.smem;
    band_adapt_args(A);
    HIPCHK(hipMemset2DAsync(R.arena.as<uint8_t>() + P.lay.hdr, P.lay.total, 0, 512, (size_t)P.n_slots, R.stream));
    HIPCHK(hipStreamWaitEvent(R.stream, h->ev0, 0));
    HIPCHK(hipEventRecord(R.e0, R.stream));
    hipLaunchKernelGGL(P.kern, dim3((unsigned)P.n_slots), dim3(V.T()), (size_t)P.smem, R.stream, A);
    HIPCHK(hipGetLastError());
    HIPCHK(hipEventRecord(R.e1, R.stream));
    HIPCHK(hipStreamWaitEvent(h->stream, R.e1, 0));
    return SXG_OK;
}

static int debug_plan(sxg_poa_handle* h, LaunchPlan& P, PlanRes& R, int attempt) {
    const Variant V = P.variant;
    unsigned long long acc[8] = {0}, smin = ~0ull, smax = 0;
    for (int64_t sl = 0; sl < P.n_slots; ++sl) {
        unsigned long long one[8];
        HIPCHK(hipMemcpy(one, R.arena.as<uint8_t>() + (size_t)sl * P.lay.total + P.lay.hdr + 64, 64, hipMemcpyDeviceToHost));
        for (int k = 0; k < 8; ++k) acc[k] += one[k];
        unsigned long long st = 0;
        for (int k = 0; k < 6; ++k) st += one[k];
        smin = std::min(smin, st); smax = std::max(smax, st);
    }
    if (V.RM == 2) {
        unsigned long long rep = 0, wsum = 0, nsw = 0;
        for (int64_t sl = 0; sl < P.n_slots; ++sl) {
            unsigned long long v[49];
            HIPCHK(hipMemcpy(v, R.arena.as<uint8_t>() + (size_t)sl * P.lay.total + P.lay.hdr + 64, sizeof(v), hipMemcpyDeviceToHost));
            rep += v[27]; wsum += v[47]; nsw += v[48];
        }
        fprintf(stderr, "[sxg]   band: %llu sweeps, mean width %.1f strips of %d (%.0f columns), %llu hint-shift repeats\n", nsw,
                (double)wsum / (double)std::max(nsw, 1ull), P.lay.band_strips, (double)wsum / (double)std::max(nsw, 1ull) * V.W, rep);
    }
    if (const char* path = getenv("SXG_POA_SLOT_CSV")) {
        if (FILE* f = fopen(path, "a")) {
            for (int64_t sl = 0; sl < P.n_slots; ++sl) {
                unsigned long long v[26];
                HIPCHK(hipMemcpy(v, R.arena.as<uint8_t>() + (size_t)sl * P.lay.total + P.lay.hdr + 64, sizeof(v), hipMemcpyDeviceToHost));
                fprintf(f, "%lld,%llu,%llu", (long long)sl, v[8], v[9]);
                for (int w = 0; w < V.NW && w < 16; ++w) fprintf(f, ",%llx", v[10 + w]);
                fprintf(f, "\n");
            }
            fclose(f);
        }
    }
#ifdef SXG_ROW_PROF
    {
        unsigned long long ra[13] = {0};
        for (int64_t sl = 0; sl < P.n_slots; ++sl) {
            unsigned long long one[13];
            HIPCHK(hipMemcpy(one, R.arena.as<uint8_t>() + (size_t)sl * P.lay.total + P.lay.hdr + 64 + 28 * 8, sizeof(one), hipMemcpyDeviceToHost));
            for (int k = 0; k < 13; ++k) ra[k] += one[k];
        }
        double rt = 1e-9;
        for (int k = 0; k < 8; ++k) rt += (double)ra[k];
        static const char* seg16[8] = {"setup", "pass1+scan", "wait left wave", "combine+pass2", "wait right wave", "hand-over+end cell", "stored row fetch", "outgoing+row store"};
        static const char* segb[8] = {"descriptor+band", "predecessor fetch+fold", "pass1+scan+pass2", "end cell+best-cell search", "outgoing+band stores", "-", "-", "-"};
        const char* const* seg = V.RM == 3 ? segb : seg16;
        fprintf(stderr, "[sxg]   row profile:");
        for (int k = 0; k < 8; ++k) fprintf(stderr, " %s %.1f%%", seg[k], 100.0 * (double)ra[k] / rt);
        fprintf(stderr, "\n");
        fprintf(stderr, "[sxg]   traceback: %.3g steps, %.1f steps per window, %.0f %% of the windows prefetched, %.0f cycles per step of which %.0f in window fills\n",
                (double)ra[8], (double)ra[8] / std::max<double>((double)ra[9], 1), 100.0 * (double)ra[12] / std::max<double>((double)ra[9], 1),
                (double)ra[10] / std::max<double>((double)ra[8], 1), (double)ra[11] / std::max<double>((double)ra[8], 1));
    }
#endif
#ifdef SXG_RESORT_PROF
    {
        unsigned long long ra[6] = {0};
        for (int64_t sl = 0; sl < P.n_slots; ++sl) {
            unsigned long long one[6];
            HIPCHK(hipMemcpy(one, R.arena.as<uint8_t>() + (size_t)sl * P.lay.total + P.lay.hdr + 64 + 41 * 8, sizeof(one), hipMemcpyDeviceToHost));
            for (int k = 0; k < 6; ++k) ra[k] += one[k];
        }
        double rt = 1e-9;
        for (int k = 0; k < 5; ++k) rt += (double)ra[k];
        fprintf(stderr, "[sxg]   re-sort: records %.1f%% first() %.1f%% counts %.1f%% walks %.1f%% ranks %.1f%%; %.3g cycles per slot, %.1f rounds per slot\n",
                100 * ra[0] / rt, 100 * ra[1] / rt, 100 * ra[2] / rt, 100 * ra[3] / rt, 100 * ra[4] / rt, rt / (double)P.n_slots, (double)ra[5] / (double)P.n_slots);
    }
#endif
    double tot = 1e-9;
    for (int k = 0; k < 6; ++k) tot += (double)acc[k];
    size_t fr = 0, tt = 0;
    (void)hipMemGetInfo(&fr, &tt);
    fprintf(stderr, "[sxg] variant T=%d W=%d cvx=%d rowmode=%d attempt=%d work=%zu slots=%lld per_cu=%d smem=%d slot_bytes=%zu free=%zu ms=%.2f\n",
            V.T(), V.W, (int)P.cvx, V.RM, attempt, P.work.size(), (long long)P.n_slots, P.per_cu, P.smem, P.lay.total, fr, P.ms);
    fprintf(stderr, "[sxg]   slot busy (of the longest slot): min %.1f%% mean %.1f%%\n", 100.0 * (double)smin / (double)std::max(smax, 1ull),
            100.0 * tot / (double)P.n_slots / (double)std::max(smax, 1ull));
    fprintf(stderr, "[sxg]   slot time: other %.1f%% prep_rows %.1f%% dp_fill %.1f%% traceback %.1f%% add_alignment %.1f%% output %.1f%%\n",
            100 * acc[0] / tot, 100 * acc[1] / tot, 100 * acc[2] / tot, 100 * acc[3] / tot, 100 * acc[4] / tot, 100 * acc[5] / tot);
    return SXG_OK;
}

static int run_block_graphs(sxg_poa_handle* h, std::vector<int32_t>& status) {
    const int nb = h->n_blocks;
    h->bg_done = false;
    std::vector<int32_t> nn(std::max(nb, 1), 0), ne(std::max(nb, 1), 0), nc(std::max(nb, 1), 0);
    if (nb) {
        HIPCHK(hipMemcpy(nn.data(), h->d_nn.p, 4 * (size_t)nb, hipMemcpyDeviceToHost));
        HIPCHK(hipMemcpy(ne.data(), h->d_ne.p, 4 * (size_t)nb, hipMemcpyDeviceToHost));
        HIPCHK(hipMemcpy(nc.data(), h->d_nc.p, 4 * (size_t)nb, hipMemcpyDeviceToHost));
    }
    h->bg_node_o.assign((size_t)nb + 1, 0); h->bg_edge_o.assign((size_t)nb + 1, 0);
    int capV = 1, capE = 1, capC = 1, capT = 1;
    std::vector<int32_t> work;
    for (int b = 0; b < nb; ++b) {
        const bool ok = status[b] == ST_OK && h->meta[b].nseq > 0;
        const int cn = h->want_consensus ? nc[b] : 0;
        h->bg_node_o[(size_t)b + 1] = h->bg_node_o[(size_t)b] + (ok ? nn[b] : 0);
        h->bg_edge_o[(size_t)b + 1] = h->bg_edge_o[(size_t)b] + (ok ? ne[b] + cn : 0);
        if (!ok) continue;
        work.push_back(b);
        capV = std::max(capV, nn[b]); capE = std::max(capE, ne[b]); capC = std::max(capC, cn);
        capT = std::max(capT, std::max(std::max(nn[b], h->meta[b].maxlen), cn));
    }
    std::stable_sort(work.begin(), work.end(), [&](int a, int b) { return h->meta[a].sumlen > h->meta[b].sumlen; });
    const size_t NT = (size_t)std::max<int64_t>(h->bg_node_o[(size_t)nb], 1), ET = (size_t)std::max<int64_t>(h->bg_edge_o[(size_t)nb], 1);
    const size_t NB = (size_t)std::max<int64_t>(h->n_bases, 1), NS = (size_t)std::max<int64_t>(h->n_seqs, 1), NBL = (size_t)std::max(nb, 1);
    int rc;
    if ((rc = h->d_bg_no.ensure(8 * (NBL + 1))) || (rc = h->d_bg_eo.ensure(8 * (NBL + 1))) || (rc = h->d_bg_len.ensure(4 * NT)) ||
        (rc = h->d_bg_od.ensure(4 * NT)) || (rc = h->d_bg_id.ensure(NT)) || (rc = h->d_bg_seq.ensure(NT)) || (rc = h->d_bg_eto.ensure(4 * ET)) ||
        (rc = h->d_bg_steps.ensure(4 * NB)) || (rc = h->d_bg_nsteps.ensure(4 * NS)) || (rc = h->d_bg_cons.ensure(4 * NT)) ||
        (rc = h->d_bg_counts.ensure(4 * (size_t)BGC_N * NBL)) || (rc = h->d_bg_work.ensure(4 * std::max<size_t>(work.size(), 1))) ||
        (rc = h->d_bg_queue.ensure(256)))
        return rc;
    HIPCHK(hipMemcpyAsync(h->d_bg_no.p, h->bg_node_o.data(), 8 * ((size_t)nb + 1), hipMemcpyHostToDevice, h->stream));
    HIPCHK(hipMemcpyAsync(h->d_bg_eo.p, h->bg_edge_o.data(), 8 * ((size_t)nb + 1), hipMemcpyHostToDevice, h->stream));
    HIPCHK(hipMemsetAsync(h->d_bg_counts.p, 0, 4 * (size_t)BGC_N * NBL, h->stream));
    HIPCHK(hipMemsetAsync(h->d_bg_nsteps.p, 0, 4 * NS, h->stream));
    HIPCHK(hipMemsetAsync(h->d_bg_queue.p, 0, 256, h->stream));
    if (!work.empty()) {
        HIPCHK(hipMemcpyAsync(h->d_bg_work.p, work.data(), 4 * work.size(), hipMemcpyHostToDevice, h->stream));
        const size_t slot = bg_slot_bytes(capV, capE, capC, capT);
        int per_cu = 1;
        if (hipOccupancyMaxActiveBlocksPerMultiprocessor(&per_cu, (const void*)block_graph_kernel, BG_THREADS, 0) != hipSuccess || per_cu < 1) per_cu = 1;
        int64_t slots = std::min<int64_t>((int64_t)work.size(), (int64_t)h->num_cu * per_cu);
        slots = std::max<int64_t>(1, std::min<int64_t>(slots, (int64_t)(arena_budget(h) / slot)));
        if ((rc = h->d_bg_arena.ensure((size_t)slots * slot))) return rc;
        BgArgs A;
        A.blk_off = h->d_blk_off.as<int32_t>(); A.seq_off = h->d_seq_off.as<int64_t>(); A.bases = h->d_bases.as<uint8_t>();
        A.paths = h->d_paths.as<int32_t>(); A.node_code = h->d_node_code.as<uint8_t>(); A.edge_tail = h->d_edge_tail.as<int32_t>();
        A.edge_head = h->d_edge_head.as<int32_t>(); A.cons = h->want_consensus ? h->d_cons.as<int32_t>() : nullptr;
        A.nn = h->d_nn.as<int32_t>(); A.ne = h->d_ne.as<int32_t>(); A.nc = h->d_nc.as<int32_t>(); A.trim = h->d_trim.as<int32_t>();
        A.cons_mode = h->bg_cons_visited_only ? 2 : 1;
        A.work = h->d_bg_work.as<int32_t>(); A.n_work = (int)work.size(); A.queue = h->d_bg_queue.as<int32_t>();
        A.arena = h->d_bg_arena.as<uint8_t>(); A.slot_bytes = slot; A.capV = capV; A.capE = capE; A.capC = capC; A.capT = capT;
        A.node_o = h->d_bg_no.as<int64_t>(); A.edge_o = h->d_bg_eo.as<int64_t>();
        A.o_len = h->d_bg_len.as<int32_t>(); A.o_outdeg = h->d_bg_od.as<int32_t>(); A.o_indeg = h->d_bg_id.as<uint8_t>();
        A.o_seq = h->d_bg_seq.as<char>(); A.o_eto = h->d_bg_eto.as<int32_t>(); A.o_steps = h->d_bg_steps.as<int32_t>();
        A.o_nsteps = h->d_bg_nsteps.as<int32_t>(); A.o_cons = h->d_bg_cons.as<int32_t>(); A.o_counts = h->d_bg_counts.as<int32_t>();
        HIPCHK(hipEventRecord(h->ev0, h->stream));
        hipLaunchKernelGGL(block_graph_kernel, dim3((unsigned)slots), dim3(BG_THREADS), 0, h->stream, A);
        HIPCHK(hipGetLastError());
        HIPCHK(hipEventRecord(h->ev1, h->stream));
    }
    HIPCHK(hipStreamSynchronize(h->stream));
    if (!work.empty()) { float ms = 0; HIPCHK(hipEventElapsedTime(&ms, h->ev0, h->ev1)); h->stats.bg_ms = ms; }
    h->bg_counts.assign((size_t)BGC_N * NBL, 0);
    if (nb) HIPCHK(hipMemcpy(h->bg_counts.data(), h->d_bg_counts.p, 4 * (size_t)BGC_N * (size_t)nb, hipMemcpyDeviceToHost));
    bool changed = false;
    for (int b : work)
        if (h->bg_counts[(size_t)BGC_N * b + BGC_STATUS] != ST_OK) { status[b] = ST_INTERNAL; changed = true; }
    if (changed) HIPCHK(hipMemcpy(h->d_status.p, status.data(), 4 * (size_t)nb, hipMemcpyHostToDevice));
    h->bg_done = true;
    return SXG_OK;
}

extern "C" int sxg_poa_batch_execute(sxg_poa_handle* h) {
    if (!h) return fail(SXG_E_INVALID, "handle is NULL");
    if (!h->have_batch) return fail(SXG_E_INVALID, "no batch uploaded");
    HIPCHK(hipSetDevice(h->device));
    const RoctxRange range_("sxg_poa_batch_execute");
    h->stats = sxg_poa_stats{};
    const bool dbg = getenv("SXG_POA_DEBUG") != nullptr;
    auto T0 = std::chrono::steady_clock::now();
    auto lap = [&](const char* what) {
        if (!dbg) return;
        auto T1 = std::chrono::steady_clock::now();
        fprintf(stderr, "[sxg] host %-18s %.3f ms\n", what, std::chrono::duration<double, std::milli>(T1 - T0).count());
        T0 = T1;
    };
    const int nb = h->n_blocks;
    std::vector<int32_t> status(std::max(nb, 1), 0);
    float ms_total = 0;
    std::vector<int32_t> pending;
    for (int b = 0; b < nb; ++b) {
        if (!h->meta[b].fits) status[b] = ST_TOO_LONG; else pending.push_back(b);
    }
    if (nb) HIPCHK(hipMemcpyAsync(h->d_status.p, status.data(), 4 * (size_t)nb, hipMemcpyHostToDevice, h->stream));
    if (nb) {
        HIPCHK(hipMemsetAsync(h->d_nn.p, 0, 4 * (size_t)nb, h->stream));
        HIPCHK(hipMemsetAsync(h->d_ne.p, 0, 4 * (size_t)nb, h->stream));
        HIPCHK(hipMemsetAsync(h->d_nc.p, 0, 4 * (size_t)nb, h->stream));
        HIPCHK(hipMemsetAsync(h->d_blk_cycles.p, 0, 8 * (size_t)nb, h->stream));
    }
    lap("setup");
    std::vector<LaunchPlan> all_plans;
    std::vector<int32_t> nomem_blocks;
    for (int b = 0; b < nb; ++b) h->meta[b].tier = 0;
    for (int attempt = 0; attempt < 7 && !pending.empty(); ++attempt) {
        std::vector<LaunchPlan> plans;
        for (int b : pending) {
            const BlockMeta& m = h->meta[b];
            LaunchPlan* pl = nullptr;
            for (auto& q : plans)
                if (q.variant == m.variant && q.cvx == m.cvx && q.sw == m.sw && q.tier == m.tier && q.wide_band == m.wide_band) { pl = &q; break; }
            if (!pl) { plans.emplace_back(); pl = &plans.back(); pl->variant = m.variant; pl->cvx = m.cvx; pl->sw = m.sw; pl->tier = m.tier; pl->wide_band = m.wide_band; }
            pl->work.push_back(b);
        }
        std::sort(plans.begin(), plans.end(), [](const LaunchPlan& a, const LaunchPlan& b) { return a.variant.Lpad() > b.variant.Lpad(); });
        const double merge_env = getenv("SXG_POA_MERGE") ? atof(getenv("SXG_POA_MERGE")) : 0.0;
        for (size_t i = 0; i < plans.size(); ++i)
            for (size_t j = i + 1; j < plans.size();) {
                const LaunchPlan &a = plans[i], &b = plans[j];
                if (same_kind(a.variant, b.variant) && a.variant.RM != 3 && a.cvx == b.cvx && a.sw == b.sw && a.tier == b.tier && a.wide_band == b.wide_band &&
                    (double)b.variant.Lpad() >= (merge_env > 0 ? merge_env : (a.variant.Lpad() >= 4096 ? 0.92 : 0.75)) * (double)a.variant.Lpad()) {
                    plans[i].work.insert(plans[i].work.end(), b.work.begin(), b.work.end());
                    plans.erase(plans.begin() + (long)j);
                } else ++j;
            }
        if (!getenv("SXG_POA_NO_SPREAD")) {
            uint64_t waves = 0;
            for (auto& pl : plans) waves += (uint64_t)pl.work.size() * (uint64_t)pl.variant.NW;
            for (auto& pl : plans) {
                Variant& v = pl.variant;
                while (v.RM == 2 && v.NW <= 2 && v.W % 2 == 0 && v.W / 2 >= 4 && 2 * waves <= (uint64_t)h->num_cu * 16u) {
                    waves += (uint64_t)pl.work.size() * (uint64_t)v.NW;
                    v = Variant{v.W / 2, 2 * v.NW, class_tmax(v.W / 2, 2 * v.NW, 2, v.CB, true), 2, v.CB, v.DS};
                }
            }
        }
        const uint64_t budget = arena_budget(h);
        uint64_t want_bytes = 0;
        for (auto& pl : plans) {
            std::stable_sort(pl.work.begin(), pl.work.end(), [&](int a, int b) { return h->meta[a].cost > h->meta[b].cost; });
            prepare_plan(h, pl, pl.tier);
            want_bytes += (uint64_t)pl.want_slots * pl.lay.total;
        }
        for (size_t i = 0; i < plans.size();) {
            if ((uint64_t)plans[i].lay.total > budget && plans[i].wide_band) {
                for (int b : plans[i].work) { h->meta[b].wide_band = false; h->meta[b].no_wide = true; }
                plans.erase(plans.begin() + (long)i);
            } else if ((uint64_t)plans[i].lay.total > budget) {
                for (int b : plans[i].work) status[b] = plans[i].tier >= 2 ? ST_POOL_OVERFLOW : ST_ROWS_OVERFLOW;
                g_err = "memory budget too small for a block arena of " + std::to_string(plans[i].lay.total) + " bytes";
                nomem_blocks.insert(nomem_blocks.end(), plans[i].work.begin(), plans[i].work.end());
                plans.erase(plans.begin() + (long)i);
            } else ++i;
        }
        std::vector<double> pcost(plans.size(), 0.0);
        for (size_t i = 0; i < plans.size(); ++i)
            for (int b : plans[i].work)
                pcost[i] += std::max(h->meta[b].cost, 1.0) * (plans[i].variant.RM == 3 ? 1.0 : (double)plans[i].variant.Lpad() / (double)std::max(h->meta[b].maxlen, 1));
        const int oversub = getenv("SXG_POA_OVERSUB") ? std::max(1, atoi(getenv("SXG_POA_OVERSUB"))) : 2;
        auto slots_at = [&](size_t i, double lambda) {
            const double s = lambda * pcost[i] / (double)plans[i].variant.NW;
            return (int64_t)std::min<double>((double)plans[i].want_slots, std::max(1.0, std::floor(s)));
        };
        auto fits = [&](double lambda) {
            uint64_t bytes = 0, waves = 0;
            for (size_t i = 0; i < plans.size(); ++i) {
                const int64_t n = slots_at(i, lambda);
                bytes += (uint64_t)n * plans[i].lay.total;
                waves += (uint64_t)n * (uint64_t)plans[i].variant.NW;
            }
            return bytes <= budget && (plans.size() == 1 || waves <= (uint64_t)h->num_cu * 16u * (uint64_t)oversub);
        };
        double lam_lo = 0.0, lam_hi = 1.0;
        while (lam_hi < 1e30 && fits(lam_hi)) {
            bool all_full = true;
            for (size_t i = 0; i < plans.size(); ++i) all_full = all_full && slots_at(i, lam_hi) >= plans[i].want_slots;
            if (all_full) break;
            lam_hi *= 2.0;
        }
        if (!fits(lam_hi))
            for (int it = 0; it < 100; ++it) {
                const double mid = 0.5 * (lam_lo + lam_hi);
                if (fits(mid)) lam_lo = mid; else lam_hi = mid;
            }
        const double lambda = fits(lam_hi) ? lam_hi : lam_lo;
        (void)want_bytes;
        while (h->planres.size() < plans.size()) {
            PlanRes* r = new PlanRes();
            HIPCHK(hipStreamCreateWithFlags(&r->stream, hipStreamNonBlocking));
            HIPCHK(hipEventCreate(&r->e0));
            HIPCHK(hipEventCreate(&r->e1));
            h->planres.push_back(r);
        }
        for (size_t i = 0; i < plans.size(); ++i) plans[i].n_slots = slots_at(i, lambda);
        lap("plan");
        {
            const size_t board_bytes = (size_t)PRIO_BOARD_CUS * PRIO_BOARD_SLOTS * 4;
            int rcb = h->d_board.ensure(board_bytes);
            if (rcb) return rcb;
            HIPCHK(hipMemsetAsync(h->d_board.p, 0, board_bytes, h->stream));
        }
        HIPCHK(hipEventRecord(h->ev0, h->stream));
        int prio_base = 0;
        for (size_t i = 0; i < plans.size(); ++i) {
            int rc = launch_plan(h, plans[i], *h->planres[i], prio_base);
            if (rc) return rc;
            prio_base += (int)((plans[i].n_slots + h->num_cu - 1) / std::max(h->num_cu, 1));
        }
        HIPCHK(hipEventRecord(h->ev1, h->stream));
        if (attempt == 0 && h->want_block_graph && h->pins && h->n_bases >= ((int64_t)16 << 20) && !getenv("SXG_POA_NO_PINNED")) {
            if (h->pin_thread.joinable()) h->pin_thread.join();
            try {
                h->pin_thread = std::thread([pool = h->pins, dev = h->device, bytes = 4 * (size_t)h->n_bases] {
                    if (hipSetDevice(dev) == hipSuccess) pool->prewarm(bytes);
                });
            } catch (...) {}
        }
        HIPCHK(hipStreamSynchronize(h->stream));
        float ms = 0;
        HIPCHK(hipEventElapsedTime(&ms, h->ev0, h->ev1));
        ms_total += ms;
        for (size_t i = 0; i < plans.size(); ++i) {
            HIPCHK(hipEventElapsedTime(&plans[i].ms, h->planres[i]->e0, h->planres[i]->e1));
            plans[i].clock_mhz = sample_clock(plans[i], *h->planres[i]);
            h->stats.dp_launches += 1;
            h->stats.n_slots += (int)plans[i].n_slots;
            h->stats.device_bytes += (uint64_t)plans[i].n_slots * plans[i].lay.total;
            if (dbg) debug_plan(h, plans[i], *h->planres[i], attempt);
        }
        lap("launches");
        {
            std::vector<int32_t> dev(std::max(nb, 1));
            HIPCHK(hipMemcpy(dev.data(), h->d_status.p, 4 * (size_t)nb, hipMemcpyDeviceToHost));
            for (auto& pl : plans) for (int b : pl.work) status[b] = dev[b];
        }
        std::vector<int32_t> again;
        if (dbg) {
            int cnt[16] = {0};
            for (int b : pending) cnt[status[b] & 15]++;
            fprintf(stderr, "[sxg] round %d: ok %d rows %d pool %d steps %d nodes %d long %d range %d band %d\n", attempt, cnt[0], cnt[1], cnt[2], cnt[3],
                    cnt[4], cnt[5], cnt[6], cnt[7]);
        }
        for (int b : pending) {
            BlockMeta& m = h->meta[b];
            if (std::find(nomem_blocks.begin(), nomem_blocks.end(), b) != nomem_blocks.end()) continue;
            if (status[b] == ST_ROWS_OVERFLOW || status[b] == ST_POOL_OVERFLOW || status[b] == ST_TBX_OVERFLOW || status[b] == ST_NODES_OVERFLOW) {
                if (m.tier < 3) { m.tier += 1; again.push_back(b); }
            } else if (status[b] == ST_BAND_MISS && m.rm == 2 && !m.wide_band && !m.no_wide) {
                m.wide_band = true;
                again.push_back(b);
            } else if (status[b] == ST_RANGE_OVERFLOW || status[b] == ST_BAND_MISS) {
                if (m.rm != 1) {
                    classify_block(m, m.rm >= 2 ? 0 : 1, false);
                    if (m.fits) again.push_back(b);
                    else status[b] = ST_TOO_LONG;
                } else status[b] = ST_TOO_LONG;
            }
        }
        h->stats.retries += (int)again.size();
        pending.swap(again);
        for (auto& pl : plans) all_plans.push_back(std::move(pl));
    }
    for (int b : pending) status[b] = ST_POOL_OVERFLOW;
    if (nb) HIPCHK(hipMemcpy(h->d_status.p, status.data(), 4 * (size_t)nb, hipMemcpyHostToDevice));
    lap("status");
    std::vector<unsigned long long> cells((size_t)std::max<int64_t>(h->n_seqs, 1));
    if (h->n_seqs) HIPCHK(hipMemcpy(cells.data(), h->d_cells.p, 8 * (size_t)h->n_seqs, hipMemcpyDeviceToHost));
    uint64_t total = 0, bytes = 0;
    std::vector<uint64_t> blk_cells(std::max(nb, 1), 0), blk_bytes(std::max(nb, 1), 0);
    for (int b = 0; b < nb; ++b) {
        if (status[b] != ST_OK) continue;
        uint64_t cb = 0;
        for (int s = h->h_blk_off[b]; s < h->h_blk_off[b + 1]; ++s) cb += cells[s];
        const BlockMeta& m = h->meta[b];
        const int ncross = m.S.convex ? 3 : (m.S.g == m.S.e ? 1 : 2);
        const int sz = m.rm == 1 ? 4 : 2;
        blk_cells[b] = cb; blk_bytes[b] = cb * (uint64_t)(2 * ncross * sz + 1);
        total += cb;
        bytes += blk_bytes[b];
    }
    for (auto& pl : all_plans) {
        for (int b : pl.work) if (status[b] == ST_OK) { pl.cells += blk_cells[b]; pl.bytes += blk_bytes[b]; }
        if (pl.cells >= h->stats.dom_cells) {
            h->stats.dom_cells = pl.cells; h->stats.dom_algo_bytes = pl.bytes; h->stats.dom_kernel_ms = pl.ms;
            h->stats.dom_threads = pl.variant.T(); h->stats.dom_cols_per_lane = pl.variant.W * (pl.variant.RM >= 2 ? 2 : 1);
            h->stats.dom_row_mode = pl.variant.RM;
            h->stats.dom_clock_mhz = pl.clock_mhz;
        }
    }
    lap("accounting");
    h->stats.kernel_ms = ms_total;
    h->stats.cells = total;
    h->stats.algo_bytes = bytes;
    h->executed = true;
    if (h->want_block_graph) {
        int rc = run_block_graphs(h, status);
        if (rc) return rc;
        lap("block graphs");
    }
    for (int b = 0; b < nb; ++b)
        if (status[b] != ST_OK) return fail(SXG_E_BLOCK, "block " + std::to_string(b) + " failed with status " + std::to_string(status[b]));
    return SXG_OK;
}

static void* host_big_alloc(size_t bytes) {
    if (bytes < ((size_t)8 << 20)) return malloc(bytes ? bytes : 1);
    void* q = nullptr;
    if (posix_memalign(&q, (size_t)2 << 20, bytes)) return nullptr;
    madvise(q, bytes, MADV_HUGEPAGE);
    return q;
}
template <class T> struct host_noinit_alloc : std::allocator<T> {
    template <class U> struct rebind { typedef host_noinit_alloc<U> other; };
    T* allocate(size_t n) {
        void* q = host_big_alloc(n * sizeof(T));
        if (!q) throw std::bad_alloc();
        return (T*)q;
    }
    void deallocate(T* q, size_t) noexcept { free(q); }
    template <class U> void construct(U* q) noexcept { ::new ((void*)q) U; }
    template <class U, class... A> void construct(U* q, A&&... a) { ::new ((void*)q) U(std::forward<A>(a)...); }
};
template <class T> using hvec = std::vector<T, host_noinit_alloc<T>>;
struct OutOwner {
    std::shared_ptr<PinPool> pin_pool;
    int32_t* bg_steps_pinned = nullptr;
    std::vector<int32_t> status, score, msa_cols;
    hvec<int32_t> node_rank, node_group, edge_tail, edge_head, cons_nodes;
    int32_t* seq_path_nodes = nullptr;
    ~OutOwner() { free(seq_path_nodes); if (bg_steps_pinned && pin_pool) pin_pool->release(bg_steps_pinned); }
    std::vector<int64_t> node_off, edge_off, cons_off, msa_off;
    hvec<uint8_t> node_code;
    hvec<uint32_t> edge_weight;
    std::vector<uint64_t> cells, block_cycles;
    std::vector<char> msa;
    std::vector<int64_t> bg_node_off, bg_seq_off, bg_edge_off, bg_step_off, bg_cons_off;
    hvec<int32_t> bg_node_len, bg_node_outdeg, bg_edge_to, bg_steps, bg_cons_steps;
    hvec<uint8_t> bg_node_indeg, bg_seq;
};

template <class Tv>
static int gather_download(sxg_poa_handle* h, const DevBuf& src, const std::vector<int64_t>& dst_off, DevBuf& d_srcoff,
                           DevBuf& d_dstoff, DevBuf& d_dense, hvec<Tv>& out) {
    const int nb = h->n_blocks;
    const int64_t total = dst_off[nb];
    out.resize((size_t)std::max<int64_t>(total, 1));
    if (total == 0) return SXG_OK;
    int rc;
    if ((rc = d_dense.ensure(sizeof(Tv) * (size_t)total))) return rc;
    hipLaunchKernelGGL((gather_kernel<Tv>), dim3((unsigned)std::min(nb, 4096)), dim3(256), 0, h->stream, src.as<Tv>(),
                       d_dense.as<Tv>(), d_srcoff.as<int64_t>(), d_dstoff.as<int64_t>(), nb);
    HIPCHK(hipGetLastError());
    HIPCHK(hipMemcpyAsync(out.data(), d_dense.p, sizeof(Tv) * (size_t)total, hipMemcpyDeviceToHost, h->stream));
    HIPCHK(hipStreamSynchronize(h->stream));
    return SXG_OK;
}

extern "C" int sxg_poa_batch_download(sxg_poa_handle* h, sxg_poa_batch_out* out) {
    if (!h || !out) return fail(SXG_E_INVALID, "NULL argument");
    memset(out, 0, sizeof(*out));
    if (!h->have_batch || !h->executed) return fail(SXG_E_INVALID, "no executed batch to download");
    HIPCHK(hipSetDevice(h->device));
    const RoctxRange range_("sxg_poa_batch_download");
    HostLaps laps;
    const int nb = h->n_blocks;
    const int64_t ns = h->n_seqs;
    OutOwner* o = new OutOwner();
    out->_owner = o;
    out->n_blocks = nb; out->n_seqs = ns;
    o->status.resize(std::max(nb, 1));
    std::vector<int32_t> nn(std::max(nb, 1)), ne(std::max(nb, 1)), nc(std::max(nb, 1));
    if (nb) {
        HIPCHK(hipMemcpy(o->status.data(), h->d_status.p, 4 * (size_t)nb, hipMemcpyDeviceToHost));
        HIPCHK(hipMemcpy(nn.data(), h->d_nn.p, 4 * (size_t)nb, hipMemcpyDeviceToHost));
        HIPCHK(hipMemcpy(ne.data(), h->d_ne.p, 4 * (size_t)nb, hipMemcpyDeviceToHost));
        HIPCHK(hipMemcpy(nc.data(), h->d_nc.p, 4 * (size_t)nb, hipMemcpyDeviceToHost));
    }
    o->node_off.assign(nb + 1, 0); o->edge_off.assign(nb + 1, 0); o->cons_off.assign(nb + 1, 0);
    std::vector<int64_t> src_off(nb + 1, 0);
    for (int b = 0; b < nb; ++b) {
        o->node_off[b + 1] = o->node_off[b] + nn[b];
        o->edge_off[b + 1] = o->edge_off[b] + ne[b];
        o->cons_off[b + 1] = o->cons_off[b] + nc[b];
        src_off[b] = h->h_seq_off[h->h_blk_off[b]];
    }
    int rc;
    if ((rc = h->d_tmp_a.ensure(8 * (size_t)(nb + 1))) || (rc = h->d_tmp_b.ensure(8 * (size_t)(nb + 1)))) { sxg_poa_batch_free(out); return rc; }
    HIPCHK(hipMemcpy(h->d_tmp_a.p, src_off.data(), 8 * (size_t)(nb + 1), hipMemcpyHostToDevice));
    auto put_off = [&](const std::vector<int64_t>& off) -> int {
        hipError_t e = hipMemcpy(h->d_tmp_b.p, off.data(), 8 * (size_t)(nb + 1), hipMemcpyHostToDevice);
        return e == hipSuccess ? SXG_OK : fail(SXG_E_NODEVICE, hipGetErrorString(e));
    };
#define GD(T, src, off, dst)                                                                         \
    if ((rc = put_off(off)) || (rc = gather_download<T>(h, src, off, h->d_tmp_a, h->d_tmp_b, h->d_tmp_c, dst))) { \
        sxg_poa_batch_free(out);                                                                     \
        return rc;                                                                                   \
    }
    const bool with_graphs = !(h->want_block_graph == 3 && h->bg_done);
    if (with_graphs) {
    GD(uint8_t, h->d_node_code, o->node_off, o->node_code)
    GD(int32_t, h->d_node_rank, o->node_off, o->node_rank)
    GD(int32_t, h->d_node_group, o->node_off, o->node_group)
    GD(int32_t, h->d_edge_tail, o->edge_off, o->edge_tail)
    GD(int32_t, h->d_edge_head, o->edge_off, o->edge_head)
    GD(uint32_t, h->d_edge_w, o->edge_off, o->edge_weight)
    if (h->want_consensus) { GD(int32_t, h->d_cons, o->cons_off, o->cons_nodes) }
    }
#undef GD
    laps.lap("download: POA graphs");
    const bool with_paths = !(h->want_block_graph >= 2 && h->bg_done);
    if (with_paths) {
        o->seq_path_nodes = (int32_t*)host_big_alloc(4 * (size_t)std::max<int64_t>(h->n_bases, 1));
        if (!o->seq_path_nodes) { sxg_poa_batch_free(out); return fail(SXG_E_NOMEM, "host allocation of the path array failed"); }
        if (h->n_bases) HIPCHK(hipMemcpy(o->seq_path_nodes, h->d_paths.p, 4 * (size_t)h->n_bases, hipMemcpyDeviceToHost));
    }
    o->score.resize((size_t)std::max<int64_t>(ns, 1));
    o->cells.resize((size_t)std::max<int64_t>(ns, 1));
    laps.lap("download: paths");
    if (h->want_block_graph && h->bg_done) {
        o->bg_node_off.assign(nb + 1, 0); o->bg_seq_off.assign(nb + 1, 0); o->bg_edge_off.assign(nb + 1, 0); o->bg_cons_off.assign(nb + 1, 0);
        std::vector<int64_t> blk_steps(nb + 1, 0), src_no(nb + 1, 0), src_eo(nb + 1, 0);
        std::vector<int32_t> nsteps((size_t)std::max<int64_t>(ns, 1), 0);
        if (ns) HIPCHK(hipMemcpy(nsteps.data(), h->d_bg_nsteps.p, 4 * (size_t)ns, hipMemcpyDeviceToHost));
        o->bg_step_off.assign((size_t)ns + 1, 0);
        for (int64_t sq = 0; sq < ns; ++sq) o->bg_step_off[(size_t)sq + 1] = o->bg_step_off[(size_t)sq] + nsteps[(size_t)sq];
        for (int b = 0; b < nb; ++b) {
            const int32_t* c = h->bg_counts.data() + (size_t)BGC_N * b;
            const bool ok = o->status[b] == ST_OK;
            o->bg_node_off[b + 1] = o->bg_node_off[b] + (ok ? c[BGC_NODES] : 0);
            o->bg_seq_off[b + 1] = o->bg_seq_off[b] + (ok ? c[BGC_SEQ] : 0);
            o->bg_edge_off[b + 1] = o->bg_edge_off[b] + (ok ? c[BGC_EDGES] : 0);
            o->bg_cons_off[b + 1] = o->bg_cons_off[b] + (ok && h->want_consensus ? c[BGC_CONS] : 0);
            blk_steps[b + 1] = o->bg_step_off[(size_t)h->h_blk_off[b + 1]];
            src_no[b] = h->bg_node_o[(size_t)b]; src_eo[b] = h->bg_edge_o[(size_t)b];
        }
        auto put_src = [&](const std::vector<int64_t>& off) -> int {
            hipError_t e = hipMemcpy(h->d_tmp_a.p, off.data(), 8 * (size_t)(nb + 1), hipMemcpyHostToDevice);
            return e == hipSuccess ? SXG_OK : fail(SXG_E_NODEVICE, hipGetErrorString(e));
        };
#define GB_(T, srcoff, src, off, dst)                                                                                      \
        if ((rc = put_src(srcoff)) || (rc = put_off(off)) || (rc = gather_download<T>(h, src, off, h->d_tmp_a, h->d_tmp_b, h->d_tmp_c, dst))) { \
            sxg_poa_batch_free(out);                                                                                       \
            return rc;                                                                                                     \
        }
        GB_(int32_t, src_no, h->d_bg_len, o->bg_node_off, o->bg_node_len)
        GB_(int32_t, src_no, h->d_bg_od, o->bg_node_off, o->bg_node_outdeg)
        GB_(uint8_t, src_no, h->d_bg_id, o->bg_node_off, o->bg_node_indeg)
        GB_(uint8_t, src_no, h->d_bg_seq, o->bg_seq_off, o->bg_seq)
        GB_(int32_t, src_eo, h->d_bg_eto, o->bg_edge_off, o->bg_edge_to)
        {
            const int64_t total = blk_steps[nb];
            if (h->pin_thread.joinable()) h->pin_thread.join();
            if (total >= ((int64_t)16 << 20) && h->pins && !getenv("SXG_POA_NO_PINNED")) {
                if (void* q = h->pins->acquire(4 * (size_t)total)) { o->pin_pool = h->pins; o->bg_steps_pinned = (int32_t*)q; }
            }
            if (o->bg_steps_pinned) {
                if ((rc = put_src(src_off)) || (rc = put_off(blk_steps)) || (rc = h->d_tmp_c.ensure(4 * (size_t)total))) { sxg_poa_batch_free(out); return rc; }
                hipLaunchKernelGGL((gather_kernel<int32_t>), dim3((unsigned)std::min(nb, 4096)), dim3(256), 0, h->stream, h->d_bg_steps.as<int32_t>(),
                                   h->d_tmp_c.as<int32_t>(), h->d_tmp_a.as<int64_t>(), h->d_tmp_b.as<int64_t>(), nb);
                hipError_t e = hipGetLastError();
                if (e == hipSuccess) e = hipMemcpyAsync(o->bg_steps_pinned, h->d_tmp_c.p, 4 * (size_t)total, hipMemcpyDeviceToHost, h->stream);
                if (e == hipSuccess) e = hipStreamSynchronize(h->stream);
                if (e != hipSuccess) { sxg_poa_batch_free(out); return fail(SXG_E_NODEVICE, std::string("download of the step lists: ") + hipGetErrorString(e)); }
            } else {
                GB_(int32_t, src_off, h->d_bg_steps, blk_steps, o->bg_steps)
            }
        }
        if (h->want_consensus) { GB_(int32_t, src_no, h->d_bg_cons, o->bg_cons_off, o->bg_cons_steps) }
#undef GB_
        out->bg_node_off = o->bg_node_off.data(); out->bg_node_len = o->bg_node_len.data(); out->bg_node_outdeg = o->bg_node_outdeg.data();
        out->bg_node_indeg = o->bg_node_indeg.data(); out->bg_seq_off = o->bg_seq_off.data(); out->bg_seq = (char*)o->bg_seq.data();
        out->bg_edge_off = o->bg_edge_off.data(); out->bg_edge_to = o->bg_edge_to.data(); out->bg_step_off = o->bg_step_off.data();
        out->bg_steps = o->bg_steps_pinned ? o->bg_steps_pinned : o->bg_steps.data();
        if (h->want_consensus) { out->bg_cons_off = o->bg_cons_off.data(); out->bg_cons_steps = o->bg_cons_steps.data(); }
        laps.lap("download: block graphs");
    }
    o->block_cycles.assign((size_t)std::max(nb, 1), 0);
    if (nb) HIPCHK(hipMemcpy(o->block_cycles.data(), h->d_blk_cycles.p, 8 * (size_t)nb, hipMemcpyDeviceToHost));
    out->block_cycles = o->block_cycles.data();
    if (ns) {
        HIPCHK(hipMemcpy(o->score.data(), h->d_score.p, 4 * (size_t)ns, hipMemcpyDeviceToHost));
        HIPCHK(hipMemcpy(o->cells.data(), h->d_cells.p, 8 * (size_t)ns, hipMemcpyDeviceToHost));
    }
    out->status = o->status.data();
    out->node_off = o->node_off.data(); out->edge_off = o->edge_off.data();
    if (with_graphs) {
        out->node_code = o->node_code.data(); out->node_rank = o->node_rank.data(); out->node_group = o->node_group.data();
        out->edge_tail = o->edge_tail.data(); out->edge_head = o->edge_head.data(); out->edge_weight = o->edge_weight.data();
    }
    out->seq_path_nodes = o->seq_path_nodes; out->score = o->score.data(); out->cells = o->cells.data();
    if (h->want_consensus) { out->cons_off = o->cons_off.data(); if (with_graphs) out->cons_nodes = o->cons_nodes.data(); }
    if (h->want_msa && o->seq_path_nodes) {
        static const char dec[5] = {'A', 'C', 'G', 'T', 'N'};
        o->msa_off.assign(nb + 1, 0); o->msa_cols.assign(std::max(nb, 1), 0);
        std::vector<std::vector<int32_t>> cols(nb);
        for (int b = 0; b < nb; ++b) {
            const int64_t n0 = o->node_off[b];
            const int n = nn[b];
            std::vector<int32_t> by_rank(n);
            for (int v = 0; v < n; ++v) by_rank[o->node_rank[n0 + v]] = v;
            cols[b].assign(n, 0);
            int ncol = 0;
            for (int r = 0; r < n; ++r) {
                const int v = by_rank[r];
                if (r > 0 && o->node_group[n0 + by_rank[r - 1]] == o->node_group[n0 + v]) cols[b][v] = ncol - 1;
                else cols[b][v] = ncol++;
            }
            o->msa_cols[b] = ncol;
            const int rows = (h->h_blk_off[b + 1] - h->h_blk_off[b]) + (h->want_consensus ? 1 : 0);
            o->msa_off[b + 1] = o->msa_off[b] + (o->status[b] == ST_OK ? (int64_t)rows * ncol : 0);
        }
        o->msa.assign((size_t)std::max<int64_t>(o->msa_off[nb], 1), '-');
        for (int b = 0; b < nb; ++b) {
            if (o->status[b] != ST_OK) continue;
            const int64_t n0 = o->node_off[b];
            const int ncol = o->msa_cols[b];
            char* base = o->msa.data() + o->msa_off[b];
            int row = 0;
            for (int s = h->h_blk_off[b]; s < h->h_blk_off[b + 1]; ++s, ++row)
                for (int64_t k = h->h_seq_off[s]; k < h->h_seq_off[s + 1]; ++k) {
                    const int v = o->seq_path_nodes[k];
                    base[(int64_t)row * ncol + cols[b][v]] = dec[o->node_code[n0 + v]];
                }
            if (h->want_consensus)
                for (int64_t k = o->cons_off[b]; k < o->cons_off[b + 1]; ++k) {
                    const int v = o->cons_nodes[k];
                    base[(int64_t)row * ncol + cols[b][v]] = dec[o->node_code[n0 + v]];
                }
        }
        out->msa_off = o->msa_off.data(); out->msa_cols = o->msa_cols.data(); out->msa = o->msa.data();
    }
    return SXG_OK;
}

extern "C" int sxg_poa_batch_device_view(sxg_poa_handle* h, sxg_poa_device_view* v) {
    if (!h || !v) return fail(SXG_E_INVALID, "NULL argument");
    memset(v, 0, sizeof(*v));
    if (!h->have_batch || !h->executed) return fail(SXG_E_INVALID, "no executed batch");
    v->n_blocks = h->n_blocks; v->n_seqs = h->n_seqs; v->n_bases = h->n_bases;
    v->status = h->d_status.as<int32_t>(); v->n_nodes = h->d_nn.as<int32_t>(); v->n_edges = h->d_ne.as<int32_t>();
    v->node_code = h->d_node_code.as<uint8_t>(); v->node_rank = h->d_node_rank.as<int32_t>();
    v->node_group = h->d_node_group.as<int32_t>(); v->edge_tail = h->d_edge_tail.as<int32_t>();
    v->edge_head = h->d_edge_head.as<int32_t>(); v->edge_weight = h->d_edge_w.as<uint32_t>();
    v->seq_path_nodes = h->d_paths.as<int32_t>(); v->score = h->d_score.as<int32_t>();
    return SXG_OK;
}

extern "C" void sxg_poa_batch_free(sxg_poa_batch_out* out) {
    if (!out) return;
    delete (OutOwner*)out->_owner;
    memset(out, 0, sizeof(*out));
}

extern "C" int sxg_poa_batch_run(sxg_poa_handle* h, const sxg_poa_batch_in* in, sxg_poa_batch_out* out) {
    if (out) memset(out, 0, sizeof(*out));
    int rc = sxg_poa_batch_upload(h, in);
    if (rc) return rc;
    rc = sxg_poa_batch_execute(h);
    if (rc && rc != SXG_E_BLOCK) return rc;
    const std::string keep = g_err;
    int rc2 = sxg_poa_batch_download(h, out);
    if (rc2) return rc2;
    if (rc) g_err = keep;
    return rc;
}

namespace {
struct RcclApi {
    decltype(&::ncclGetUniqueId) GetUniqueId = nullptr;
    decltype(&::ncclCommInitRank) CommInitRank = nullptr;
    decltype(&::ncclCommDestroy) CommDestroy = nullptr;
    decltype(&::ncclCommAbort) CommAbort = nullptr;
    decltype(&::ncclCommGetAsyncError) CommGetAsyncError = nullptr;
    decltype(&::ncclAllGather) AllGather = nullptr;
    decltype(&::ncclGroupStart) GroupStart = nullptr;
    decltype(&::ncclGroupEnd) GroupEnd = nullptr;
    decltype(&::ncclSend) Send = nullptr;
    decltype(&::ncclRecv) Recv = nullptr;
    decltype(&::ncclGetErrorString) GetErrorString = nullptr;
    bool ok = false;
    std::string why;
};
RcclApi& rccl_api() {
    static RcclApi A = [] {
        RcclApi a;
        void* lib = nullptr;
        if (const char* forced = getenv("SXG_POA_RCCL_LIB")) lib = dlopen(forced, RTLD_NOW | RTLD_GLOBAL);
        else
            for (const char* name : {"librccl.so.1", "librccl.so", "/opt/rocm/lib/librccl.so.1"})
                if ((lib = dlopen(name, RTLD_NOW | RTLD_GLOBAL))) break;
// ... 1242 lines not shown
```

### smoothxg_amd/poa.py

```python
import ctypes as C
import os

import numpy as np

from . import build as _build

MODE_LOCAL, MODE_GLOBAL = 0, 1


class Params(C.Structure):
    _fields_ = [("m", C.c_int8), ("n", C.c_int8), ("g", C.c_int8), ("e", C.c_int8),
                ("q", C.c_int8), ("c", C.c_int8), ("mode", C.c_uint8), ("banded", C.c_uint8)]


def params_from_cli(m=1, n=4, g=6, e=2, q=26, c=1, local=True):
    return Params(m, -n, -g, -e, -q, -c, MODE_LOCAL if local else MODE_GLOBAL, 0)


_i32p, _i64p, _u8p, _u32p, _u64p = (C.POINTER(C.c_int32), C.POINTER(C.c_int64), C.POINTER(C.c_uint8),
                                    C.POINTER(C.c_uint32), C.POINTER(C.c_uint64))


class BatchIn(C.Structure):
    _fields_ = [("n_blocks", C.c_int32), ("blk_off", _i32p), ("seq_off", _i64p), ("bases", _u8p),
                ("weights", _u32p), ("params", C.POINTER(Params)), ("per_block_params", C.c_int32),
                ("want_consensus", C.c_int32), ("want_msa", C.c_int32),
                ("want_block_graph", C.c_int32), ("bg_consensus_visited_only", C.c_int32), ("bg_trim", _i32p)]


class BatchOut(C.Structure):
    _fields_ = [("n_blocks", C.c_int32), ("n_seqs", C.c_int64), ("status", _i32p), ("node_off", _i64p),
                ("node_code", _u8p), ("node_rank", _i32p), ("node_group", _i32p), ("edge_off", _i64p),
                ("edge_tail", _i32p), ("edge_head", _i32p), ("edge_weight", _u32p),
                ("seq_path_nodes", _i32p), ("score", _i32p), ("cells", _u64p), ("cons_off", _i64p),
                ("cons_nodes", _i32p), ("msa_off", _i64p), ("msa_cols", _i32p), ("msa", C.c_void_p),
                ("bg_node_off", _i64p), ("bg_node_len", _i32p), ("bg_node_outdeg", _i32p), ("bg_node_indeg", _u8p),
                ("bg_seq_off", _i64p), ("bg_seq", C.c_void_p), ("bg_edge_off", _i64p), ("bg_edge_to", _i32p),
                ("bg_step_off", _i64p), ("bg_steps", _i32p), ("bg_cons_off", _i64p), ("bg_cons_steps", _i32p),
                ("block_cycles", _u64p), ("_owner", C.c_void_p)]


class AlignIn(C.Structure):
    _fields_ = [("n", C.c_int32), ("row_off", _i64p), ("row_code", _u8p), ("row_sink", _u8p),
                ("pred_off", _i64p), ("preds", _i32p), ("seq_off", _i64p), ("bases", _u8p),
                ("params", C.POINTER(Params)), ("per_problem_params", C.c_int32)]


class AlignOut(C.Structure):
    _fields_ = [("n", C.c_int32), ("status", _i32p), ("score", _i32p), ("pair_off", _i64p),
                ("pair_row", _i32p), ("pair_pos", _i32p), ("_owner", C.c_void_p)]


class Stats(C.Structure):
    _fields_ = [("kernel_ms", C.c_double), ("cells", C.c_uint64), ("dp_launches", C.c_uint64),
                ("algo_bytes", C.c_uint64), ("n_slots", C.c_int32), ("retries", C.c_int32),
                ("device_bytes", C.c_uint64), ("dom_kernel_ms", C.c_double), ("dom_cells", C.c_uint64),
                ("dom_algo_bytes", C.c_uint64), ("dom_threads", C.c_int32), ("dom_cols_per_lane", C.c_int32),
                ("dom_row_mode", C.c_int32), ("dom_clock_mhz", C.c_int32), ("bg_ms", C.c_double)]


class DeviceView(C.Structure):
    _fields_ = [("n_blocks", C.c_int32), ("n_seqs", C.c_int64), ("n_bases", C.c_int64),
                ("status", C.c_void_p), ("n_nodes", C.c_void_p), ("n_edges", C.c_void_p),
                ("node_code", C.c_void_p), ("node_rank", C.c_void_p), ("node_group", C.c_void_p),
                ("edge_tail", C.c_void_p), ("edge_head", C.c_void_p), ("edge_weight", C.c_void_p),
                ("seq_path_nodes", C.c_void_p), ("score", C.c_void_p)]


class SplitIn(C.Structure):
    _fields_ = [("n_blocks", C.c_int32), ("blk_off", _i32p), ("seq_off", _i64p), ("bases", _u8p),
                ("identity", C.POINTER(C.c_double)), ("length_ratio_min", C.POINTER(C.c_double))]


class SplitOut(C.Structure):
    _fields_ = [("n_blocks", C.c_int32), ("n_seqs", C.c_int64), ("group", _i32p), ("n_groups", _i32p),
                ("n_pairs", _i64p), ("status", _i32p), ("_owner", C.c_void_p)]


class SplitMash(C.Structure):
    _fields_ = [("kmer_size", C.c_int32), ("min_len", _i32p), ("est_identity", C.POINTER(C.c_double))]


class SgdIn(C.Structure):
    _fields_ = [("n_nodes", C.c_int64), ("node_len", _i32p), ("n_paths", C.c_int64), ("path_off", _i64p), ("step_node", _i32p),
                ("step_pos", _i64p), ("iter_max", C.c_int32), ("cooling_start", C.c_int32), ("eta", C.POINTER(C.c_double)),
                ("terms_per_iter", C.c_uint64), ("seed", C.c_uint64), ("mode", C.c_int32)]


SGD_LDS_NODES = 8192
MASH_SORT_TILE = 1024
SPLIT_PANEL = 512
MAX_SEQ_LEN = 26623
ST_TOO_LONG = 5

EXPORTS = ["sxg_poa_path_sgd_order", "sxg_poa_kmer_jaccard_batch", "sxg_poa_split_mash_batch", "sxg_poa_pair_identity_batch", "sxg_poa_split_batch", "sxg_poa_split_free", "sxg_poa_batch_device_view", "sxg_poa_abi_version", "sxg_poa_device_count", "sxg_poa_last_error", "sxg_poa_create",
           "sxg_poa_destroy", "sxg_poa_batch_run", "sxg_poa_batch_upload", "sxg_poa_batch_execute",
           "sxg_poa_batch_download", "sxg_poa_batch_free", "sxg_poa_align_batch", "sxg_poa_align_free",
           "sxg_poa_get_stats", "sxg_poa_set_memory_budget", "sxg_xxh64", "sxg_poa_comm_unique_id", "sxg_poa_comm_init",
           "sxg_poa_comm_attach", "sxg_poa_comm_destroy", "sxg_poa_batch_run_sharded", "sxg_poa_batch_run_sharded_local",
           "sxg_poa_batch_upload_sharded", "sxg_poa_batch_execute_sharded", "sxg_poa_batch_download_sharded", "sxg_poa_sharded_info",
           "sxg_poa_sharded_timing", "sxg_poa_measure_copy", "sxg_poa_roctx_available"]
COMM_ID_BYTES = 128
NOT_ROOT = 1

_lib = None


def load_library(build_if_missing=True):
    global _lib
    if _lib is not None:
        return _lib
    so = os.environ.get("SXG_POA_LIB", _build.SO)
    if not os.path.exists(so):
        if not build_if_missing:
            raise RuntimeError("libsxgpoa.so is missing: run `python -m smoothxg_amd.build`")
        _build.build()
    L = C.CDLL(so)
    vp = C.c_void_p
    L.sxg_poa_last_error.restype = C.c_char_p
    L.sxg_poa_create.argtypes = [C.c_int, C.POINTER(vp)]
    L.sxg_poa_destroy.argtypes = [vp]
    L.sxg_poa_batch_run.argtypes = [vp, C.POINTER(BatchIn), C.POINTER(BatchOut)]
    L.sxg_poa_batch_upload.argtypes = [vp, C.POINTER(BatchIn)]
    L.sxg_poa_batch_execute.argtypes = [vp]
    L.sxg_poa_batch_download.argtypes = [vp, C.POINTER(BatchOut)]
    L.sxg_poa_batch_free.argtypes = [C.POINTER(BatchOut)]
    L.sxg_poa_batch_device_view.argtypes = [vp, C.POINTER(DeviceView)]
    L.sxg_poa_align_batch.argtypes = [vp, C.POINTER(AlignIn), C.POINTER(AlignOut)]
    L.sxg_poa_align_free.argtypes = [C.POINTER(AlignOut)]
    L.sxg_poa_get_stats.argtypes = [vp, C.POINTER(Stats)]
    L.sxg_poa_set_memory_budget.argtypes = [vp, C.c_uint64]
    L.sxg_poa_measure_copy.argtypes = [vp, C.c_uint64, C.c_int, C.POINTER(C.c_double)]
    L.sxg_poa_comm_unique_id.argtypes = [C.POINTER(C.c_uint8)]
    L.sxg_poa_comm_init.argtypes = [vp, C.POINTER(C.c_uint8), C.c_int, C.c_int]
    L.sxg_poa_comm_attach.argtypes = [vp, vp, C.c_int, C.c_int]
    L.sxg_poa_comm_destroy.argtypes = [vp]
    L.sxg_poa_comm_destroy.restype = None
    L.sxg_poa_batch_run_sharded.argtypes = [vp, C.POINTER(BatchIn), C.POINTER(BatchOut)]
    L.sxg_poa_batch_run_sharded_local.argtypes = [vp, C.POINTER(BatchIn), C.c_int, C.POINTER(BatchOut)]
    L.sxg_poa_batch_upload_sharded.argtypes = [vp, C.POINTER(BatchIn)]
    L.sxg_poa_batch_execute_sharded.argtypes = [vp]
    L.sxg_poa_batch_download_sharded.argtypes = [vp, C.POINTER(BatchIn), C.POINTER(BatchOut)]
    L.sxg_poa_sharded_info.argtypes = [vp, C.POINTER(C.c_int32), C.POINTER(C.c_uint64)]
    L.sxg_poa_sharded_timing.argtypes = [vp, C.POINTER(C.c_double), C.POINTER(C.c_double)]
    L.sxg_poa_pair_identity_batch.argtypes = [vp, C.c_int64, _i64p, _u8p, C.c_int64, _i32p, _i32p, _u8p, _i32p, _i32p, _i32p, _i32p]
    L.sxg_poa_split_batch.argtypes = [vp, C.POINTER(SplitIn), C.POINTER(SplitOut)]
    L.sxg_poa_split_free.argtypes = [C.POINTER(SplitOut)]
    L.sxg_poa_kmer_jaccard_batch.argtypes = [vp, C.c_int64, _i64p, _u8p, C.c_int32, C.c_int64, _i32p, _i32p, _i32p, _i32p, C.POINTER(C.c_uint64)]
    L.sxg_poa_split_mash_batch.argtypes = [vp, C.POINTER(SplitIn), C.POINTER(SplitMash), C.POINTER(SplitOut), _i64p]
    L.sxg_poa_split_free.restype = None
    L.sxg_poa_path_sgd_order.argtypes = [vp, C.POINTER(SgdIn), _i32p, _i64p]
    L.sxg_xxh64.restype = C.c_uint64
    L.sxg_xxh64.argtypes = [C.c_char_p, C.c_uint64, C.c_uint64]
    _lib = L
    return L


class PoaError(RuntimeError):
    pass


def _p(a, t):
    return a.ctypes.data_as(C.POINTER(t))


def _arr(ptr, n, dtype):
    if n == 0 or not ptr:
        return np.zeros(0, dtype)
    return np.ctypeslib.as_array(ptr, shape=(n,)).astype(dtype, copy=True)


class BlockResult:
    __slots__ = ("status", "node_code", "node_rank", "node_group", "edge_tail", "edge_head", "edge_weight",
                 "paths", "scores", "cells", "consensus", "msa", "bg", "device_cycles")


class BlockGraph:
    __slots__ = ("node_seq", "node_indeg", "edges", "paths", "consensus")

    def gfa(self, names, revs=None, consensus_name=None):
        o = ["H\tVN:Z:1.0"]
        o += ["S\t%d\t%s" % (i + 1, s) for i, s in enumerate(self.node_seq)]
        o += ["L\t%d\t+\t%d\t+\t0M" % (a + 1, b + 1) for a, b in self.edges]
        for i, p in enumerate(self.paths):
            for j, nm in enumerate(names[i]):
                st = ["%d-" % (v + 1) for v in p[::-1]] if revs is not None and revs[i][j] else ["%d+" % (v + 1) for v in p]
                o.append("P\t%s\t%s\t*" % (nm, ",".join(st)))
        if consensus_name is not None:
            o.append("P\t%s\t%s\t*" % (consensus_name, ",".join("%d+" % (v + 1) for v in self.consensus)))
        return "\n".join(o) + "\n"


class PoaEngine:

    def __init__(self, device=0):
        self.lib = load_library()
        if self.lib.sxg_poa_device_count() <= 0:
            raise PoaError("no HIP device: the blocked-POA engine has no CPU fallback")
        h = C.c_void_p()
        rc = self.lib.sxg_poa_create(device, C.byref(h))
        if rc:
            raise PoaError("sxg_poa_create: %s" % self.lib.sxg_poa_last_error().decode())
        self.h = h
        self._keep = None
        self._shape = None

    def close(self):
        if getattr(self, "h", None):
            self.lib.sxg_poa_destroy(self.h)
            self.h = None

    def __del__(self):
        try:
            self.close()
        except Exception:
            pass

    def _err(self, what):
        return PoaError("%s: %s" % (what, self.lib.sxg_poa_last_error().decode()))

    def set_memory_budget(self, nbytes):
        self.lib.sxg_poa_set_memory_budget(self.h, int(nbytes))

    def _mk_in(self, bases, seq_off, blk_off, weights, params, want_consensus, want_msa, block_graph=0, bg_trim=None,
               bg_cons_visited_only=False):
        bases = np.ascontiguousarray(bases, np.uint8)
        seq_off = np.ascontiguousarray(seq_off, np.int64)
        blk_off = np.ascontiguousarray(blk_off, np.int32)
        nb = len(blk_off) - 1
        if isinstance(params, Params):
            parr = (Params * 1)(params)
            per = 0
        else:
            parr = (Params * max(len(params), 1))(*params)
            per = 1
        w = None if weights is None else np.ascontiguousarray(weights, np.uint32)
        bpad = bases if len(bases) else np.zeros(1, np.uint8)
        trim = None if bg_trim is None else np.ascontiguousarray(bg_trim, np.int32)
        bi = BatchIn(nb, _p(blk_off, C.c_int32), _p(seq_off, C.c_int64), _p(bpad, C.c_uint8),
                     _p(w, C.c_uint32) if w is not None else None, parr, per, int(want_consensus),
                     int(want_msa), int(block_graph), int(bool(bg_cons_visited_only)),
                     _p(trim, C.c_int32) if trim is not None else None)
        self._keep = (bpad, seq_off, blk_off, w, parr, trim)
        return bi

    def upload(self, bases, seq_off, blk_off, weights, params, want_consensus=False, want_msa=False, block_graph=0,
               bg_trim=None, bg_cons_visited_only=False):
        bi = self._mk_in(bases, seq_off, blk_off, weights, params, want_consensus, want_msa, block_graph, bg_trim,
                         bg_cons_visited_only)
        if self.lib.sxg_poa_batch_upload(self.h, C.byref(bi)):
            raise self._err("sxg_poa_batch_upload")
        self._shape = (np.asarray(blk_off).copy(), np.asarray(seq_off).copy())

    def execute(self, check=True):
        rc = self.lib.sxg_poa_batch_execute(self.h)
        if rc and (check or rc != -4):
            raise self._err("sxg_poa_batch_execute")
        return rc

    def stats(self):
        s = Stats()
        self.lib.sxg_poa_get_stats(self.h, C.byref(s))
        return {f[0]: getattr(s, f[0]) for f in Stats._fields_}

    def device_view(self):
        v = DeviceView()
        if self.lib.sxg_poa_batch_device_view(self.h, C.byref(v)):
            raise self._err("sxg_poa_batch_device_view")
        return v

    def download(self):
        out = BatchOut()
        if self.lib.sxg_poa_batch_download(self.h, C.byref(out)):
            raise self._err("sxg_poa_batch_download")
        try:
            return self._unpack(out)
        finally:
            self.lib.sxg_poa_batch_free(C.byref(out))

    def _unpack(self, out):
        blk_off, seq_off = self._shape
        nb = out.n_blocks
        ns = int(out.n_seqs)
        status = _arr(out.status, nb, np.int32)
        node_off = _arr(out.node_off, nb + 1, np.int64)
        edge_off = _arr(out.edge_off, nb + 1, np.int64)
        nn, ne = (int(node_off[-1]), int(edge_off[-1])) if nb else (0, 0)
        has_raw = bool(out.node_code) or nn == 0
        node_code = _arr(out.node_code, nn, np.uint8) if has_raw else None
        node_rank = _arr(out.node_rank, nn, np.int32) if has_raw else None
        node_group = _arr(out.node_group, nn, np.int32) if has_raw else None
        et = _arr(out.edge_tail, ne, np.int32) if has_raw else None
        eh = _arr(out.edge_head, ne, np.int32) if has_raw else None
        ew = _arr(out.edge_weight, ne, np.uint32) if has_raw else None
        nbases = int(seq_off[-1]) if ns else 0
        paths = _arr(out.seq_path_nodes, nbases, np.int32) if out.seq_path_nodes else None
        bg = None
        if out.bg_node_off:
            bno = _arr(out.bg_node_off, nb + 1, np.int64)
            bso = _arr(out.bg_seq_off, nb + 1, np.int64)
            beo = _arr(out.bg_edge_off, nb + 1, np.int64)
            bpo = _arr(out.bg_step_off, ns + 1, np.int64)
            bg = dict(no=bno, so=bso, eo=beo, po=bpo, ln=_arr(out.bg_node_len, int(bno[-1]), np.int32),
                      od=_arr(out.bg_node_outdeg, int(bno[-1]), np.int32), idg=_arr(out.bg_node_indeg, int(bno[-1]), np.uint8),
                      sq=C.string_at(out.bg_seq, int(bso[-1])) if bso[-1] else b"", to=_arr(out.bg_edge_to, int(beo[-1]), np.int32),
                      st=_arr(out.bg_steps, int(bpo[-1]), np.int32))
            if out.bg_cons_off:
                bg["co"] = _arr(out.bg_cons_off, nb + 1, np.int64)
                bg["cs"] = _arr(out.bg_cons_steps, int(bg["co"][-1]), np.int32)
        score = _arr(out.score, ns, np.int32)
        cells = _arr(out.cells, ns, np.uint64)
        cycles = _arr(out.block_cycles, nb, np.uint64) if out.block_cycles else None
        cons_off = _arr(out.cons_off, nb + 1, np.int64) if out.cons_off else None
        cons = _arr(out.cons_nodes, int(cons_off[-1]), np.int32) if cons_off is not None and nb and out.cons_nodes else None
        msa_off = _arr(out.msa_off, nb + 1, np.int64) if out.msa_off else None
        msa_cols = _arr(out.msa_cols, nb, np.int32) if out.msa_cols else None
        msa_raw = None
        if msa_off is not None and nb and msa_off[-1] > 0:
            msa_raw = C.string_at(out.msa, int(msa_off[-1]))
        res = []
        for b in range(nb):
            r = BlockResult()
            r.status = int(status[b])
            a, z = node_off[b], node_off[b + 1]
            r.node_code, r.node_rank, r.node_group = (node_code[a:z], node_rank[a:z], node_group[a:z]) if has_raw else (None, None, None)
            a, z = edge_off[b], edge_off[b + 1]
            r.edge_tail, r.edge_head, r.edge_weight = (et[a:z], eh[a:z], ew[a:z]) if has_raw else (None, None, None)
            s0, s1 = int(blk_off[b]), int(blk_off[b + 1])
            r.paths = [paths[int(seq_off[s]):int(seq_off[s + 1])] for s in range(s0, s1)] if paths is not None else None
            r.bg = None
            if bg is not None:
                g = BlockGraph()
                a, z = int(bg["no"][b]), int(bg["no"][b + 1])
                ln, od = bg["ln"][a:z], bg["od"][a:z]
                g.node_indeg = bg["idg"][a:z]
                so = int(bg["so"][b]) + np.concatenate([[0], np.cumsum(ln)]).astype(np.int64)
                g.node_seq = [bg["sq"][int(so[i]):int(so[i + 1])].decode() for i in range(z - a)]
                to = bg["to"][int(bg["eo"][b]):int(bg["eo"][b + 1])]
                g.edges = list(zip(np.repeat(np.arange(z - a), od).tolist(), to.tolist()))
                g.paths = [bg["st"][int(bg["po"][s]):int(bg["po"][s + 1])] for s in range(s0, s1)]
                g.consensus = bg["cs"][int(bg["co"][b]):int(bg["co"][b + 1])] if "co" in bg else None
                r.bg = g
            r.scores, r.cells = score[s0:s1], cells[s0:s1]
            r.device_cycles = int(cycles[b]) if cycles is not None else None
            r.consensus = cons[cons_off[b]:cons_off[b + 1]] if cons is not None else None
            r.msa = None
            if msa_raw is not None and r.status == 0:
                ncol = int(msa_cols[b])
                raw = msa_raw[int(msa_off[b]):int(msa_off[b + 1])]
                r.msa = [raw[i * ncol:(i + 1) * ncol].decode() for i in range(len(raw) // ncol)] if ncol else []
            res.append(r)
        return res

    def run_flat(self, bases, seq_off, blk_off, weights, params, want_consensus=False, want_msa=False,
                 check=True, block_graph=0, bg_trim=None, bg_cons_visited_only=False):
        self.upload(bases, seq_off, blk_off, weights, params, want_consensus, want_msa, block_graph, bg_trim,
                    bg_cons_visited_only)
        self.execute(check=check)
        return self.download()

    def comm_unique_id(self):
        buf = (C.c_uint8 * COMM_ID_BYTES)()
        if self.lib.sxg_poa_comm_unique_id(buf):
            raise self._err("sxg_poa_comm_unique_id")
        return bytes(buf)

    def comm_init(self, comm_id, nranks, rank):
        buf = (C.c_uint8 * COMM_ID_BYTES)(*comm_id)
        if self.lib.sxg_poa_comm_init(self.h, buf, nranks, rank):
            raise self._err("sxg_poa_comm_init")

    def run_flat_sharded(self, bases, seq_off, blk_off, weights, params, want_consensus=False, want_msa=False, check=True,
                         simulate_ranks=0, block_graph=0, bg_trim=None, bg_cons_visited_only=False):
        bi = self._mk_in(bases, seq_off, blk_off, weights, params, want_consensus, want_msa, block_graph, bg_trim, bg_cons_visited_only)
        self._shape = (np.asarray(blk_off).copy(), np.asarray(seq_off).copy())
        out = BatchOut()
        if simulate_ranks:
            rc = self.lib.sxg_poa_batch_run_sharded_local(self.h, C.byref(bi), simulate_ranks, C.byref(out))
        else:
            rc = self.lib.sxg_poa_batch_run_sharded(self.h, C.byref(bi), C.byref(out))
        if rc == NOT_ROOT:
            return None
        try:
            if rc and (check or rc != -4):
                raise self._err("sxg_poa_batch_run_sharded")
            return self._unpack(out)
        finally:
            self.lib.sxg_poa_batch_free(C.byref(out))

    def upload_sharded(self, bases, seq_off, blk_off, weights, params, want_consensus=False, want_msa=False):
        self._sh_in = self._mk_in(bases, seq_off, blk_off, weights, params, want_consensus, want_msa)
        self._shape = (np.asarray(blk_off).copy(), np.asarray(seq_off).copy())
        if self.lib.sxg_poa_batch_upload_sharded(self.h, C.byref(self._sh_in)):
            raise self._err("sxg_poa_batch_upload_sharded")

    def execute_sharded(self):
        if self.lib.sxg_poa_batch_execute_sharded(self.h):
            raise self._err("sxg_poa_batch_execute_sharded")

    def download_sharded(self, check=True):
        out = BatchOut()
        rc = self.lib.sxg_poa_batch_download_sharded(self.h, C.byref(self._sh_in), C.byref(out))
        if rc == NOT_ROOT:
            return None
        try:
            if rc and (check or rc != -4):
                raise self._err("sxg_poa_batch_download_sharded")
            return self._unpack(out)
        finally:
            self.lib.sxg_poa_batch_free(C.byref(out))

    def measure_copy(self, nbytes=1 << 30, reps=5):
        g = C.c_double()
        if self.lib.sxg_poa_measure_copy(self.h, C.c_uint64(int(nbytes)), int(reps), C.byref(g)):
            raise self._err("sxg_poa_measure_copy")
        return g.value

    def roctx_available(self):
        return int(self.lib.sxg_poa_roctx_available())

    def sharded_info(self):
        n, b = C.c_int32(), C.c_uint64()
        self.lib.sxg_poa_sharded_info(self.h, C.byref(n), C.byref(b))
        pk, ex = C.c_double(), C.c_double()
        self.lib.sxg_poa_sharded_timing(self.h, C.byref(pk), C.byref(ex))
        return {"ranks_seen": n.value, "bytes_received": b.value, "pack_ms": pk.value, "exchange_ms": ex.value}

    def run_blocks(self, blocks, params, weights=None, want_consensus=False, want_msa=False, check=True):
        seqs = [s for blk in blocks for s in blk]
        bases = np.concatenate([np.asarray(s, np.uint8) for s in seqs]) if seqs else np.zeros(0, np.uint8)
        seq_off = np.zeros(len(seqs) + 1, np.int64)
        if seqs:
            seq_off[1:] = np.cumsum([len(s) for s in seqs])
        blk_off = np.zeros(len(blocks) + 1, np.int32)
        if blocks:
            blk_off[1:] = np.cumsum([len(b) for b in blocks])
        w = None if weights is None else np.concatenate([np.asarray(x, np.uint32) for x in weights])
        return self.run_flat(bases, seq_off, blk_off, w, params, want_consensus, want_msa, check)

    @staticmethod
    def _flat(seqs):
        seqs = [np.ascontiguousarray(x, np.uint8) for x in seqs]
        seq_off = np.zeros(len(seqs) + 1, np.int64)
        if seqs:
            seq_off[1:] = np.cumsum([len(x) for x in seqs])
        bases = np.concatenate(seqs) if seqs else np.zeros(0, np.uint8)
        return (bases if len(bases) else np.zeros(1, np.uint8)), seq_off

    def pair_identity(self, seqs, pairs, caps, rev=None):
        bases, seq_off = self._flat(seqs)
        n = len(pairs)
        pa = np.ascontiguousarray([p[0] for p in pairs], np.int32) if n else np.zeros(1, np.int32)
        pb = np.ascontiguousarray([p[1] for p in pairs], np.int32) if n else np.zeros(1, np.int32)
        cap = np.ascontiguousarray(caps, np.int32) if n else np.zeros(1, np.int32)
        rv = None if rev is None else (np.ascontiguousarray(rev, np.uint8) if n else np.zeros(1, np.uint8))
        pen, cols, mat = (np.zeros(max(n, 1), np.int32) for _ in range(3))
        rc = self.lib.sxg_poa_pair_identity_batch(self.h, len(seqs), _p(seq_off, C.c_int64), _p(bases, C.c_uint8), n, _p(pa, C.c_int32),
                                                  _p(pb, C.c_int32), _p(rv, C.c_uint8) if rv is not None else None, _p(cap, C.c_int32),
                                                  _p(pen, C.c_int32), _p(cols, C.c_int32), _p(mat, C.c_int32))
        if rc:
            raise self._err("sxg_poa_pair_identity_batch")
        return pen[:n], cols[:n], mat[:n]

    def split(self, blocks, identity, length_ratio_min=0.0, check=True):
        nb = len(blocks)
        bases, seq_off = self._flat([x for blk in blocks for x in blk])
        blk_off = np.zeros(nb + 1, np.int32)
        if nb:
            blk_off[1:] = np.cumsum([len(b) for b in blocks])
        ident = np.ascontiguousarray(np.broadcast_to(np.asarray(identity, np.float64), (nb,)) if nb else np.zeros(1), np.float64)
        ratio = np.ascontiguousarray(np.broadcast_to(np.asarray(length_ratio_min, np.float64), (nb,)) if nb else np.zeros(1), np.float64)
        si = SplitIn(nb, _p(blk_off, C.c_int32), _p(seq_off, C.c_int64), _p(bases, C.c_uint8), _p(ident, C.c_double), _p(ratio, C.c_double))
        out = SplitOut()
        rc = self.lib.sxg_poa_split_batch(self.h, C.byref(si), C.byref(out))
        try:
            if rc and (check or rc != -4):
                raise self._err("sxg_poa_split_batch")
            grp = _arr(out.group, int(blk_off[-1]), np.int32)
            ng, npairs, st = _arr(out.n_groups, nb, np.int32), _arr(out.n_pairs, nb, np.int64), _arr(out.status, nb, np.int32)
            return [(grp[blk_off[b]:blk_off[b + 1]], int(ng[b]), int(npairs[b]), int(st[b])) for b in range(nb)]
        finally:
            self.lib.sxg_poa_split_free(C.byref(out))

    def kmer_jaccard(self, seqs, pairs, k, want_sets=False):
        bases, seq_off = self._flat(seqs)
        ns, n = len(seqs), len(pairs)
        pa = np.ascontiguousarray([p[0] for p in pairs], np.int32) if n else np.zeros(1, np.int32)
        pb = np.ascontiguousarray([p[1] for p in pairs], np.int32) if n else np.zeros(1, np.int32)
        size, inter = np.zeros(max(ns, 1), np.int32), np.zeros(max(n, 1), np.int32)
        kmers = np.zeros(max(int(seq_off[-1]), 1), np.uint64) if want_sets else None
        rc = self.lib.sxg_poa_kmer_jaccard_batch(self.h, ns, _p(seq_off, C.c_int64), _p(bases, C.c_uint8), int(k), n, _p(pa, C.c_int32),
                                                 _p(pb, C.c_int32), _p(size, C.c_int32), _p(inter, C.c_int32),
                                                 _p(kmers, C.c_uint64) if want_sets else None)
        if rc:
            raise self._err("sxg_poa_kmer_jaccard_batch")
        if want_sets:
            return size[:ns], inter[:n], [kmers[seq_off[s]:seq_off[s] + size[s]].copy() for s in range(ns)]
        return size[:ns], inter[:n]

    def split_mash(self, blocks, identity, length_ratio_min, kmer_size, min_len, est_identity=None, check=True):
        nb = len(blocks)
        bases, seq_off = self._flat([x for blk in blocks for x in blk])
        blk_off = np.zeros(nb + 1, np.int32)
        if nb:
            blk_off[1:] = np.cumsum([len(b) for b in blocks])
        per_block = lambda v, dt: np.ascontiguousarray(np.broadcast_to(np.asarray(v, dt), (nb,)) if nb else np.zeros(1), dt)
        ident, ratio = per_block(identity, np.float64), per_block(length_ratio_min, np.float64)
        est = ident.copy() if est_identity is None else per_block(est_identity, np.float64)
        ml = per_block(min_len, np.int32)
        si = SplitIn(nb, _p(blk_off, C.c_int32), _p(seq_off, C.c_int64), _p(bases, C.c_uint8), _p(ident, C.c_double), _p(ratio, C.c_double))
        sm = SplitMash(int(kmer_size), _p(ml, C.c_int32), _p(est, C.c_double))
        nm = np.zeros(max(nb, 1), np.int64)
        out = SplitOut()
        rc = self.lib.sxg_poa_split_mash_batch(self.h, C.byref(si), C.byref(sm), C.byref(out), _p(nm, C.c_int64))
        try:
            if rc and (check or rc != -4):
                raise self._err("sxg_poa_split_mash_batch")
            grp = _arr(out.group, int(blk_off[-1]), np.int32)
            ng, npairs, st = _arr(out.n_groups, nb, np.int32), _arr(out.n_pairs, nb, np.int64), _arr(out.status, nb, np.int32)
            return [(grp[blk_off[b]:blk_off[b + 1]], int(ng[b]), int(npairs[b]), int(nm[b]), int(st[b])) for b in range(nb)]
        finally:
            self.lib.sxg_poa_split_free(C.byref(out))

    def path_sgd_order(self, node_len, path_off, step_node, step_pos, eta, cooling_start, terms_per_iter, seed, mode=0, want_x=True):
        def arr(a, t):
            a = np.ascontiguousarray(a, t)
            return a if len(a) else np.zeros(1, t)
        n, n_paths = len(node_len), len(path_off) - 1
        node_len, path_off, step_node, step_pos = arr(node_len, np.int32), arr(path_off, np.int64), arr(step_node, np.int32), arr(step_pos, np.int64)
        si = SgdIn(n, _p(node_len, C.c_int32), n_paths, _p(path_off, C.c_int64), _p(step_node, C.c_int32), _p(step_pos, C.c_int64),
                   1, int(cooling_start), None, int(terms_per_iter), int(seed), int(mode))
        if eta is not None:
            si.iter_max = len(eta)
            eta = arr(eta, np.float64)
            si.eta = _p(eta, C.c_double)
        order, x = np.zeros(max(n, 1), np.int32), np.zeros(max(n, 1), np.int64)
        if self.lib.sxg_poa_path_sgd_order(self.h, C.byref(si), _p(order, C.c_int32), _p(x, C.c_int64) if want_x else None):
            raise self._err("sxg_poa_path_sgd_order")
        return order[:n], (x[:n] if want_x else None)

    def align(self, problems, params, check=True):
        n = len(problems)
        row_off = np.zeros(n + 1, np.int64)
        seq_off = np.zeros(n + 1, np.int64)
        codes, sinks, preds, poffs, bases = [], [], [], [np.zeros(1, np.int64)], []
        eo = 0
        for k, (cd, off, pr, sk, sq) in enumerate(problems):
            row_off[k + 1] = row_off[k] + len(cd)
            seq_off[k + 1] = seq_off[k] + len(sq)
            codes.append(np.asarray(cd, np.uint8))
            sinks.append(np.asarray(sk, np.uint8))
            preds.append(np.asarray(pr, np.int32))
            bases.append(np.asarray(sq, np.uint8))
            poffs.append(np.asarray(off[1:], np.int64) + eo)
            eo += int(off[-1]) if len(off) else 0

        def cat(xs, dt):
            return np.ascontiguousarray(np.concatenate(xs) if xs else np.zeros(0, dt), dt)

        def pad(a):
            return a if len(a) else np.zeros(1, a.dtype)

        codes, sinks, preds, bases = cat(codes, np.uint8), cat(sinks, np.uint8), cat(preds, np.int32), cat(bases, np.uint8)
        poff = cat(poffs, np.int64)
        if isinstance(params, Params):
            parr, per = (Params * 1)(params), 0
# ... 26 lines not shown
```

Baseline: 674.5.

## Add narrower second strip width for packed int16 DP sweeps on short reads

Packed (RM=2) block kernels for some classes are now compiled with a second, narrower strip width (W-1). At runtime each sequence whose length fits in T*2*(W-1) columns is swept with the narrower width, which cuts the number of DP columns and cells computed per row. The layout is sized for both widths and the kernel body is turned into a width-templated lambda, so more code gets instantiated and register pressure may rise. The change also adds per-width sweep counters that are copied back to the host after every launch, an extra hipMemcpy2D per plan, plus an optional plan merge across the two widths.

```diff
diff --git a/include/sxg_poa.h b/include/sxg_poa.h
--- a/include/sxg_poa.h
+++ b/include/sxg_poa.h
@@ -130,6 +130,14 @@
     double bg_ms;
 } sxg_poa_stats;
 
+typedef struct sxg_poa_width_stats {
+    uint64_t sweeps[2];
+    uint64_t swept_cols[2];
+    uint64_t swept_cells[2];
+    uint64_t hint_shift_repeats;
+    int32_t dom_width, dom_width2;
+} sxg_poa_width_stats;
+
 int sxg_poa_abi_version(void);
 int sxg_poa_measure_copy(sxg_poa_handle *h, uint64_t bytes, int reps, double *gbps);
 int sxg_poa_roctx_available(void);
@@ -223,6 +231,7 @@
 int sxg_poa_path_sgd_order(sxg_poa_handle *h, const sxg_poa_sgd_in *in, int32_t *order, int64_t *x);
 
 int sxg_poa_get_stats(sxg_poa_handle *h, sxg_poa_stats *out);
+int sxg_poa_get_width_stats(sxg_poa_handle *h, sxg_poa_width_stats *out);
 int sxg_poa_set_memory_budget(sxg_poa_handle *h, uint64_t bytes);
 
 uint64_t sxg_xxh64(const void *data, uint64_t len, uint64_t seed);
diff --git a/smoothxg_amd/csrc/poa_classes.h b/smoothxg_amd/csrc/poa_classes.h
--- a/smoothxg_amd/csrc/poa_classes.h
+++ b/smoothxg_amd/csrc/poa_classes.h
@@ -4,6 +4,7 @@
     int W, NW, TMAX, RM;
     int CB = 4;
     bool DS = false;
+    int W2 = 0;
     constexpr int T() const { return 64 * NW; }
     constexpr int Lpad() const { return 64 * NW * W * (RM >= 2 ? 2 : 1); }
     constexpr bool operator==(const Variant& o) const { return W == o.W && NW == o.NW && TMAX == o.TMAX && RM == o.RM && CB == o.CB && DS == o.DS; }
@@ -37,7 +38,7 @@
 
 enum ClassKind { CLASS_BLOCK = 0, CLASS_ALIGN = 1 };
 enum : unsigned { CLS_LOCAL = 1, CLS_GLOBAL = 2, CLS_BOTH = 3, CLS_DS = 4 };
-struct ClassRow { int part; ClassKind kind; unsigned rms; int cb, tmax; unsigned widths, modes; };
+struct ClassRow { int part; ClassKind kind; unsigned rms; int cb, tmax; unsigned widths, modes; unsigned widths2 = 0; };
 constexpr unsigned cw(int w) { return 1u << w; }
 constexpr unsigned RM0 = cw(0), RM1 = cw(1), RM2 = cw(2), RM3 = cw(3), RM01 = RM0 | RM1;
 constexpr unsigned cw_range(int lo, int hi) { unsigned m = 0; for (int w = lo; w <= hi; ++w) m |= cw(w); return m; }
@@ -51,8 +52,8 @@
     {1, CLASS_ALIGN, RM01, 4, 256, cw(8) | cw(12) | cw(16), CLS_BOTH},
     {1, CLASS_ALIGN, RM01, 4, 512, cw(8) | cw(12) | cw(16), CLS_BOTH},
     {1, CLASS_ALIGN, RM01, 4, 1024, cw(8) | cw(12), CLS_BOTH},
-    {2, CLASS_BLOCK, RM2, 2, 256, cw_range(4, 12), CLS_BOTH | CLS_DS},
-    {3, CLASS_BLOCK, RM2, 2, 512, cw_range(8, 12), CLS_BOTH | CLS_DS},
+    {2, CLASS_BLOCK, RM2, 2, 256, cw_range(4, 12), CLS_BOTH | CLS_DS, cw_range(9, 12)},
+    {3, CLASS_BLOCK, RM2, 2, 512, cw_range(8, 12), CLS_BOTH | CLS_DS, cw_range(9, 12)},
     {3, CLASS_BLOCK, RM2, 2, 1024, cw(8), CLS_BOTH | CLS_DS},
     {3, CLASS_BLOCK, RM2, 2, 1024, cw(10) | cw(12) | cw(13), CLS_LOCAL | CLS_DS},
     {4, CLASS_BLOCK, RM2, 4, 256, cw_range(4, 12), CLS_BOTH},
@@ -78,6 +79,11 @@
     }
     return -1;
 }
+constexpr int class_w2(ClassKind kind, const Variant& v, bool sw) {
+    const int r = class_row(kind, v, sw);
+    return r >= 0 && (kClasses[r].widths2 & cw(v.W)) ? v.W - 1 : 0;
+}
+constexpr int width_for_len(int W, int W2, int T, int len) { return W2 != 0 && len + 1 <= T * 2 * W2 ? W2 : W; }
 constexpr bool class_built(const Variant& v, bool , bool sw, ClassKind kind = CLASS_BLOCK) { return class_row(kind, v, sw) >= 0; }
 
 constexpr int class_tmax(int W, int NW, int RM, int CB, bool full_plane) {
diff --git a/smoothxg_amd/csrc/poa_kern_tables.hip.h b/smoothxg_amd/csrc/poa_kern_tables.hip.h
--- a/smoothxg_amd/csrc/poa_kern_tables.hip.h
+++ b/smoothxg_amd/csrc/poa_kern_tables.hip.h
@@ -26,7 +26,7 @@
 template <class Args, int R, int W, int RM, bool CVX, bool SW, bool DS> static KernelFn<Args> class_kernel() {
     constexpr ClassRow c = kClasses[R];
     if constexpr (std::is_same_v<Args, AlignArgs>) return poa_align_kernel<c.tmax, W, CVX, RM, SW>;
-    else return poa_block_kernel<c.tmax, W, CVX, RM, SW, c.cb, DS>;
+    else return poa_block_kernel<c.tmax, W, CVX, RM, SW, c.cb, DS, (c.widths2 & cw(W)) != 0 ? W - 1 : 0>;
 }
 template <class Args, int R, int W, int RM> static KernelFn<Args> pick_mode(bool cvx, bool sw, bool ds) {
     constexpr unsigned m = kClasses[R].modes;
diff --git a/smoothxg_amd/csrc/poa_kernels.hip.h b/smoothxg_amd/csrc/poa_kernels.hip.h
--- a/smoothxg_amd/csrc/poa_kernels.hip.h
+++ b/smoothxg_amd/csrc/poa_kernels.hip.h
@@ -1,6 +1,7 @@
 #pragma once
 #include <hip/hip_runtime.h>
 #include <algorithm>
+#include <cstdlib>
 #include <cstring>
 
 #include "../../include/sxg_poa.h"
@@ -22,6 +23,7 @@
     int nodes_cap, rows_cap, pool_slots, step_cap, scratch_len, Lpad, word_bytes, threads;
     int band_strips;
     int lds_rows;
+    int W2, band_strips2;
 };
 
 inline size_t lay(size_t& cur, size_t bytes) {
@@ -31,13 +33,15 @@
 }
 
 inline SlotLayout make_layout(int nodes_cap, int rows_cap, int pool_slots, int step_cap, int threads, int Lpad,
-                              int word_bytes, bool pairs, int band_strips = 0, int cell_bytes = 4, bool spoa_scratch = false) {
+                              int word_bytes, bool pairs, int band_strips = 0, int cell_bytes = 4, bool spoa_scratch = false,
+                              int W2 = 0, int band_strips2 = 0) {
     SlotLayout L;
     memset(&L, 0, sizeof(L));
     L.nodes_cap = nodes_cap; L.rows_cap = rows_cap; L.pool_slots = pool_slots;
     L.step_cap = step_cap; L.threads = threads; L.Lpad = Lpad; L.word_bytes = word_bytes;
     L.band_strips = band_strips;
     const bool packed = band_strips > 0;
+    L.W2 = packed ? W2 : 0; L.band_strips2 = L.W2 ? band_strips2 : 0;
     const size_t C = (size_t)nodes_cap + 4, S = (size_t)std::max(nodes_cap, Lpad) + 4, Rr = (size_t)rows_cap + 4;
     L.scratch_len = (int)S;
     size_t cur = 0;
@@ -59,7 +63,9 @@
     L.r_code = lay(cur, Rr); L.r_flags = lay(cur, Rr); L.r_pred_off = lay(cur, 4 * Rr);
     L.r_preds = lay(cur, 4 * C); L.r_slot = lay(cur, 4 * Rr); L.r_tbx = lay(cur, 4 * Rr);
     L.r_sseq = lay(cur, 4 * Rr); L.r_row_node = lay(cur, 4 * Rr); L.r_meta = lay(cur, 32 * Rr);
-    L.tb = lay(cur, ((size_t)rows_cap + 1) * (packed ? (size_t)band_strips * (size_t)p16_slot_dwords(Lpad / (2 * threads), cell_bytes) * 4 : (size_t)Lpad));
+    size_t plane_row = packed ? (size_t)band_strips * (size_t)p16_slot_dwords(Lpad / (2 * threads), cell_bytes) * 4 : (size_t)Lpad;
+    if (L.W2) plane_row = std::max(plane_row, (size_t)L.band_strips2 * (size_t)p16_slot_dwords(L.W2, cell_bytes) * 4);
+    L.tb = lay(cur, ((size_t)rows_cap + 1) * plane_row);
     L.steps = lay(cur, packed ? 256 : (size_t)std::max(step_cap, 1) * 3 * threads * 4);
     const size_t row_bytes = (size_t)Lpad * (packed && cell_bytes == 2 ? 2 : word_bytes) + (size_t)threads * 4;
     L.pool = lay(cur, (size_t)pool_slots * row_bytes);
@@ -69,6 +75,37 @@
     if (pairs) { L.pair_row = lay(cur, 4 * (Rr + Lpad)); L.pair_pos = lay(cur, 4 * (Rr + Lpad)); }
     L.total = cur;
     return L;
+}
+
+inline int p16_lds_rows(const int T, const int W, const int CB) {
+    if (const char* e = getenv("SXG_POA_LDS_ROWS")) return std::max(0, std::min(8, atoi(e)));
+    const int wg_per_cu = std::max(1, 16 / std::max(T / 64, 1));
+    const int share = (160 * 1024) / wg_per_cu - 512;
+    const int rows = (share - dp16_lds_bytes(T, W, 0, CB)) / dp16_row_bytes(T, W, CB);
+    return std::max(0, std::min(8, rows));
+}
+
+inline int plane_strips_p16(int T, int W) {
+    if (const char* e = getenv("SXG_POA_BAND_COLS")) {
+        const int cols = std::max(atoi(e), W);
+        return std::min(plane_round4((cols + W - 1) / W), 2 * T);
+    }
+    return p16_band_strips(T, W);
+}
+
+inline bool width2_enabled() {
+    const char* e = getenv("SXG_POA_WIDTH2");
+    return !(e && atoi(e) == 0);
+}
+
+struct P16LaunchSizes { int strips, strips2, lds_rows, smem; };
+inline P16LaunchSizes p16_launch_sizes(int T, int W, int W2, int CB, bool wide_band) {
+    P16LaunchSizes s;
+    s.strips = wide_band ? 2 * T : plane_strips_p16(T, W);
+    s.strips2 = W2 ? (wide_band ? 2 * T : plane_strips_p16(T, W2)) : 0;
+    s.lds_rows = p16_lds_rows(T, W, CB);
+    s.smem = std::max(dp16_lds_bytes(T, W, s.lds_rows, CB), W2 ? dp16_lds_bytes(T, W2, s.lds_rows, CB) : 0);
+    return s;
 }
 
 struct SlotViews {
@@ -141,8 +178,9 @@
 
 __host__ __device__ constexpr int sxg_min_waves(int TMAX, int W, int RM) { return class_traits(TMAX, W, RM, 4).min_waves; }
 
-template <int TMAX, int W, bool CVX, int RM, bool SW, int CB = 4, bool DS = false>
+template <int TMAX, int W, bool CVX, int RM, bool SW, int CB = 4, bool DS = false, int W2 = 0>
 __global__ __launch_bounds__(TMAX, sxg_min_waves(TMAX, W, RM)) void poa_block_kernel(const BlockArgs A) {
+    static_assert(W2 == 0 || (RM == 2 && W2 < W), "a second strip width: packed sweep, narrower than the first");
     constexpr bool H16 = RM != 1;
     constexpr int CPL = RM >= 2 ? 2 * W : W;
     constexpr ClassTraits CT = class_traits(TMAX, W, RM, CB);
@@ -224,46 +262,59 @@
                     PROF(3);
                     if (lds[TBM_FLAG]) { status = ST_INTERNAL; break; }
                 } else if constexpr (RM == 2) {
-                    const int bs_cap = A.lay.band_strips;
-                    int bs = bs_cap;
-                    if (A.band_floor > 0 && bs_cap < 2 * T && s - s0 > A.band_full)
-                        bs = max(p16_drift_strips(band_drift, A.band_margin, W, A.band_floor, bs_cap), band_min);
-                    for (int att = 0;; ++att) {
-                        V.B.band_strips = bs;
-                        if (t == 0) { prof[47] += (unsigned long long)bs; prof[48] += 1; }
+                    auto sweep = [&](auto wk_) {
+                        constexpr int Wk = decltype(wk_)::value;
+                        constexpr int narrow = Wk != W ? 1 : 0;
+                        const int bs_cap = narrow ? A.lay.band_strips2 : A.lay.band_strips;
+                        int bs = bs_cap;
+                        if (A.band_floor > 0 && bs_cap < 2 * T && s - s0 > A.band_full)
+                            bs = max(p16_drift_strips(band_drift, A.band_margin, Wk, A.band_floor, bs_cap), min(plane_round4((band_min + Wk - 1) / Wk), bs_cap));
+                        for (int att = 0;; ++att) {
+                            V.B.band_strips = bs;
+                            if (t == 0) {
+                                prof[47] += (unsigned long long)bs; prof[48] += 1;
+                                prof[49 + narrow] += 1; prof[51 + narrow] += (unsigned long long)(T * 2 * Wk); prof[53 + narrow] += (unsigned long long)N * (unsigned long long)(T * 2 * Wk);
+                            }
 #ifdef SXG_EXP
-                        if (att == 0) { res = dp_fill_p16<W, CVX, SW, CB, CT.rp, CT.tfix, DS, SXG_EXP>(S, V.R, N, seq, len, V.B, smem); __syncthreads(); if (res.best == 0x7fffffff) break; }
+                            if (att == 0) { res = dp_fill_p16<Wk, CVX, SW, CB, CT.rp, CT.tfix, DS, SXG_EXP>(S, V.R, N, seq, len, V.B, smem); __syncthreads(); if (res.best == 0x7fffffff) break; }
 #endif
-                        res = dp_fill_p16<W, CVX, SW, CB, CT.rp, CT.tfix, DS>(S, V.R, N, seq, len, V.B, smem);
-                        __syncthreads();
-                        PROF(2);
-                        if (t == 0) { lds[TBM_FLAG] = 0; lds[TBM_RANGE] = 0; }
-                        __syncthreads();
-                        if (t < 64 && res.bi >= 0)
-                            traceback_p16<false, W, CVX, false, CB>(V.R, V.B, S, seq, len, res.best, T, min(256, (len << 8) / max(N, 1)), res.bi, res.bj,
-                                                                    V.G.posnode, nullptr, nullptr, smem);
-                        __syncthreads();
-                        PROF(3);
-                        if (lds[TBM_RANGE]) { status = ST_RANGE_OVERFLOW; break; }
-                        if (!lds[TBM_FLAG]) break;
-                        if (att == 5) { status = ST_BAND_MISS; break; }
-                        const int mrow = lds[TBM_ROW], mdelta = lds[TBM_DELTA];
-                        __syncthreads();
-                        for (int r2 = t; r2 < mrow; r2 += T) V.R.meta[8 * (size_t)r2 + 7] += mdelta;
-                        for (int i2 = t; i2 < len; i2 += T) V.G.posnode[i2] = -1;
-                        if (t == 0) prof[27] += 1;
-                        band_min = bs = min(plane_round4(2 * bs), bs_cap);
-                        __syncthreads();
-                    }
+                            res = dp_fill_p16<Wk, CVX, SW, CB, CT.rp, CT.tfix, DS>(S, V.R, N, seq, len, V.B, smem);
+                            __syncthreads();
+                            PROF(2);
+                            if (t == 0) { lds[TBM_FLAG] = 0; lds[TBM_RANGE] = 0; }
+                            __syncthreads();
+                            if (t < 64 && res.bi >= 0)
+                                traceback_p16<false, Wk, CVX, false, CB>(V.R, V.B, S, seq, len, res.best, T, min(256, (len << 8) / max(N, 1)), res.bi, res.bj,
+                                                                         V.G.posnode, nullptr, nullptr, smem);
+                            __syncthreads();
+                            PROF(3);
+                            if (lds[TBM_RANGE]) { status = ST_RANGE_OVERFLOW; break; }
+                            if (!lds[TBM_FLAG]) break;
+                            if (att == 5) { status = ST_BAND_MISS; break; }
+                            const int mrow = lds[TBM_ROW], mdelta = lds[TBM_DELTA];
+                            __syncthreads();
+                            for (int r2 = t; r2 < mrow; r2 += T) V.R.meta[8 * (size_t)r2 + 7] += mdelta;
+                            for (int i2 = t; i2 < len; i2 += T) V.G.posnode[i2] = -1;
+                            if (t == 0) prof[27] += 1;
+                            bs = min(plane_round4(2 * bs), bs_cap);
+                            band_min = bs * Wk;
+                            __syncthreads();
+                        }
+                        if (status != ST_OK) return;
+                        if (A.band_floor > 0 && bs_cap < 2 * T) {
+                            int d = 0;
+                            for (int j2 = t; j2 < len; j2 += T) {
+                                const int v = V.G.posnode[j2];
+                                if (v >= 0) d = max(d, abs(j2 + 1 - V.G.xpos[v]));
+                            }
+                            band_drift = max(band_drift, ctx.reduce_max(d));
+                        }
+                    };
+                    if constexpr (W2 != 0) {
+                        if (width_for_len(W, A.lay.W2, T, len) != W) sweep(std::integral_constant<int, W2>{});
+                        else sweep(std::integral_constant<int, W>{});
+                    } else sweep(std::integral_constant<int, W>{});
                     if (status != ST_OK) break;
-                    if (A.band_floor > 0 && bs_cap < 2 * T) {
-                        int d = 0;
-                        for (int j2 = t; j2 < len; j2 += T) {
-                            const int v = V.G.posnode[j2];
-                            if (v >= 0) d = max(d, abs(j2 + 1 - V.G.xpos[v]));
-                        }
-                        band_drift = max(band_drift, ctx.reduce_max(d));
-                    }
                 } else {
                     dp_fill<W, CVX, H16, SW>(S, V.R, N, seq, len, V.B, smem, A.park_in_lds != 0, A.pf_off, res);
                     __syncthreads();
diff --git a/smoothxg_amd/csrc/sxg_poa.hip b/smoothxg_amd/csrc/sxg_poa.hip
--- a/smoothxg_amd/csrc/sxg_poa.hip
+++ b/smoothxg_amd/csrc/sxg_poa.hip
@@ -131,14 +131,6 @@
                         std::string(#x) + ": " + hipGetErrorString(_e));                       \
     } while (0)
 
-static int p16_lds_rows(const int T, const int W, const int CB) {
-    if (const char* e = getenv("SXG_POA_LDS_ROWS")) return std::max(0, std::min(8, atoi(e)));
-    const int wg_per_cu = std::max(1, 16 / std::max(T / 64, 1));
-    const int share = (160 * 1024) / wg_per_cu - 512;
-    const int rows = (share - dp16_lds_bytes(T, W, 0, CB)) / dp16_row_bytes(T, W, CB);
-    return std::max(0, std::min(8, rows));
-}
-
 static int plane_cell_bytes(const Scoring& S) {
     if (const char* e = getenv("SXG_POA_CELL_BYTES")) if (atoi(e) == 4) return 4;
     return p16_delta_fits(S) ? 2 : 4;
@@ -286,6 +278,7 @@
     std::vector<int64_t> bg_node_o, bg_edge_o;
     std::vector<int32_t> bg_counts;
     sxg_poa_stats stats{};
+    sxg_poa_width_stats wstats{};
     ncclComm_t comm = nullptr;
     bool own_comm = false;
     int nranks = 1, rank = 0;
@@ -434,6 +427,12 @@
     return SXG_OK;
 }
 
+extern "C" int sxg_poa_get_width_stats(sxg_poa_handle* h, sxg_poa_width_stats* out) {
+    if (!h || !out) return fail(SXG_E_INVALID, "NULL argument");
+    *out = h->wstats;
+    return SXG_OK;
+}
+
 static uint64_t arena_budget(sxg_poa_handle* h) {
     size_t fr = 0, tot = 0;
     if (hipMemGetInfo(&fr, &tot) != hipSuccess) return 8ull << 30;
@@ -557,14 +556,6 @@
     int smem = 0, pf_off = -1; bool park_lds = true; uint64_t cells = 0, bytes = 0; float ms = 0;
 };
 
-static int plane_strips_p16(int T, int W) {
-    if (const char* e = getenv("SXG_POA_BAND_COLS")) {
-        const int cols = std::max(atoi(e), W);
-        return std::min(plane_round4((cols + W - 1) / W), 2 * T);
-    }
-    return p16_band_strips(T, W);
-}
-
 static void band_adapt_args(BlockArgs& A) {
     A.band_floor = P16_BAND_FLOOR; A.band_margin = P16_BAND_MARGIN; A.band_full = P16_BAND_FULL;
     if (const char* e = getenv("SXG_POA_BAND_ADAPT")) {
@@ -612,17 +603,19 @@
     if (rows_cap >= (1 << 20)) rows_cap = (1 << 20) - 1;
     const int wb = V.RM == 1 ? 8 : 4;
     if (V.RM == 3) pool_slots = 1;
-    P.lay = make_layout(nodes_cap, rows_cap, pool_slots, step_cap, V.T(), Lpad, wb, false,
-                        V.RM == 3 ? (any_adaptive ? BAND_WIN : band_plane_strips(maxlen, V.W)) : (V.RM == 2 ? (P.wide_band ? 2 * V.T() : plane_strips_p16(V.T(), V.W)) : 0),
-                        V.RM >= 2 ? V.CB : 4, any_spoa);
-    P.variant.TMAX = class_tmax(V.W, V.NW, V.RM, V.CB, P.lay.band_strips == 2 * V.T());
+    const int strips1 = V.RM == 3 ? (any_adaptive ? BAND_WIN : band_plane_strips(maxlen, V.W)) : (V.RM == 2 ? p16_launch_sizes(V.T(), V.W, 0, V.CB, P.wide_band).strips : 0);
+    P.variant.TMAX = class_tmax(V.W, V.NW, V.RM, V.CB, strips1 == 2 * V.T());
+    P.variant.W2 = width2_enabled() ? class_w2(CLASS_BLOCK, P.variant, P.sw) : 0;
+    const P16LaunchSizes LS = p16_launch_sizes(V.T(), V.W, P.variant.W2, V.CB, P.wide_band);
+    P.lay = make_layout(nodes_cap, rows_cap, pool_slots, step_cap, V.T(), Lpad, wb, false, strips1, V.RM >= 2 ? V.CB : 4, any_spoa,
+                        V.RM == 2 ? P.variant.W2 : 0, LS.strips2);
     P.kern = block_kernel(P.variant, P.cvx, P.sw);
     const int tfix = class_traits(P.variant.TMAX, V.W, V.RM, V.CB).tfix;
     if (tfix && tfix != V.T()) { P.kern = nullptr; P.why = "kernel class compiled for " + std::to_string(tfix) + " threads asked to run at " + std::to_string(V.T()); }
     if (!P.kern && P.why.empty()) P.why = "no kernel class built for this geometry";
     P.smem = dp_lds_launch_bytes(Lpad, wb);
     P.park_lds = dp_park_in_lds(Lpad, wb);
-    if (V.RM == 2) { P.lay.lds_rows = p16_lds_rows(V.T(), V.W, V.CB); P.smem = dp16_lds_bytes(V.T(), V.W, P.lay.lds_rows, V.CB); P.park_lds = true; }
+    if (V.RM == 2) { P.lay.lds_rows = LS.lds_rows; P.smem = LS.smem; P.park_lds = true; }
     if (V.RM == 3) { P.smem = band_lds_bytes(V.W); P.park_lds = true; }
     P.pf_off = (V.RM < 2 && getenv("SXG_POA_PREFETCH")) ? dp_pf_offset(Lpad, wb, V.T()) : -1;
     if (P.pf_off >= 0) P.smem += dp_pf_bytes(Lpad, wb, V.T());
@@ -706,6 +699,19 @@
     return SXG_OK;
 }
 
+static int width_stats_of(const LaunchPlan& P, const PlanRes& R, sxg_poa_width_stats& w) {
+    if (P.variant.RM != 2 || P.n_slots <= 0) return SXG_OK;
+    constexpr int K0 = 27, K1 = 55;
+    std::vector<unsigned long long> v((size_t)P.n_slots * (K1 - K0));
+    HIPCHK(hipMemcpy2D(v.data(), (K1 - K0) * 8, R.arena.as<uint8_t>() + P.lay.hdr + 64 + K0 * 8, P.lay.total, (K1 - K0) * 8, (size_t)P.n_slots, hipMemcpyDeviceToHost));
+    for (int64_t sl = 0; sl < P.n_slots; ++sl) {
+        const unsigned long long* c = v.data() + (size_t)sl * (K1 - K0);
+        w.hint_shift_repeats += c[27 - K0];
+        for (int k = 0; k < 2; ++k) { w.sweeps[k] += c[49 + k - K0]; w.swept_cols[k] += c[51 + k - K0]; w.swept_cells[k] += c[53 + k - K0]; }
+    }
+    return SXG_OK;
+}
+
 static int debug_plan(sxg_poa_handle* h, LaunchPlan& P, PlanRes& R, int attempt) {
     const Variant V = P.variant;
     unsigned long long acc[8] = {0}, smin = ~0ull, smax = 0;
@@ -726,6 +732,10 @@
         }
         fprintf(stderr, "[sxg]   band: %llu sweeps, mean width %.1f strips of %d (%.0f columns), %llu hint-shift repeats\n", nsw,
                 (double)wsum / (double)std::max(nsw, 1ull), P.lay.band_strips, (double)wsum / (double)std::max(nsw, 1ull) * V.W, rep);
+        sxg_poa_width_stats w{};
+        if (int rcw = width_stats_of(P, R, w)) return rcw;
+        fprintf(stderr, "[sxg]   width: W=%d %llu sweeps %llu columns %.4g cells; W2=%d %llu sweeps %llu columns %.4g cells\n", V.W, (unsigned long long)w.sweeps[0],
+                (unsigned long long)w.swept_cols[0], (double)w.swept_cells[0], P.lay.W2, (unsigned long long)w.sweeps[1], (unsigned long long)w.swept_cols[1], (double)w.swept_cells[1]);
     }
     if (const char* path = getenv("SXG_POA_SLOT_CSV")) {
         if (FILE* f = fopen(path, "a")) {
@@ -867,6 +877,7 @@
     HIPCHK(hipSetDevice(h->device));
     const RoctxRange range_("sxg_poa_batch_execute");
     h->stats = sxg_poa_stats{};
+    h->wstats = sxg_poa_width_stats{};
     const bool dbg = getenv("SXG_POA_DEBUG") != nullptr;
     auto T0 = std::chrono::steady_clock::now();
     auto lap = [&](const char* what) {
@@ -905,11 +916,13 @@
         }
         std::sort(plans.begin(), plans.end(), [](const LaunchPlan& a, const LaunchPlan& b) { return a.variant.Lpad() > b.variant.Lpad(); });
         const double merge_env = getenv("SXG_POA_MERGE") ? atof(getenv("SXG_POA_MERGE")) : 0.0;
+        const bool merge_w2 = getenv("SXG_POA_MERGE_WIDTH2") && atoi(getenv("SXG_POA_MERGE_WIDTH2")) != 0 && width2_enabled();
         for (size_t i = 0; i < plans.size(); ++i)
             for (size_t j = i + 1; j < plans.size();) {
                 const LaunchPlan &a = plans[i], &b = plans[j];
+                const bool join_w2 = merge_w2 && a.variant.NW == b.variant.NW && b.variant.W == class_w2(CLASS_BLOCK, a.variant, a.sw);
                 if (same_kind(a.variant, b.variant) && a.variant.RM != 3 && a.cvx == b.cvx && a.sw == b.sw && a.tier == b.tier && a.wide_band == b.wide_band &&
-                    (double)b.variant.Lpad() >= (merge_env > 0 ? merge_env : (a.variant.Lpad() >= 4096 ? 0.92 : 0.75)) * (double)a.variant.Lpad()) {
+                    (join_w2 || (double)b.variant.Lpad() >= (merge_env > 0 ? merge_env : (a.variant.Lpad() >= 4096 ? 0.92 : 0.75)) * (double)a.variant.Lpad())) {
                     plans[i].work.insert(plans[i].work.end(), b.work.begin(), b.work.end());
                     plans.erase(plans.begin() + (long)j);
                 } else ++j;
@@ -1016,6 +1029,7 @@
             h->stats.dp_launches += 1;
             h->stats.n_slots += (int)plans[i].n_slots;
             h->stats.device_bytes += (uint64_t)plans[i].n_slots * plans[i].lay.total;
+            if (int rcw = width_stats_of(plans[i], *h->planres[i], h->wstats)) return rcw;
             if (dbg) debug_plan(h, plans[i], *h->planres[i], attempt);
         }
         lap("launches");
@@ -1076,6 +1090,7 @@
             h->stats.dom_threads = pl.variant.T(); h->stats.dom_cols_per_lane = pl.variant.W * (pl.variant.RM >= 2 ? 2 : 1);
             h->stats.dom_row_mode = pl.variant.RM;
             h->stats.dom_clock_mhz = pl.clock_mhz;
+            h->wstats.dom_width = pl.variant.W; h->wstats.dom_width2 = pl.lay.W2;
         }
     }
     lap("accounting");
diff --git a/smoothxg_amd/poa.py b/smoothxg_amd/poa.py
--- a/smoothxg_amd/poa.py
+++ b/smoothxg_amd/poa.py
@@ -59,6 +59,11 @@
                 ("dom_row_mode", C.c_int32), ("dom_clock_mhz", C.c_int32), ("bg_ms", C.c_double)]
 
 
+class WidthStats(C.Structure):
+    _fields_ = [("sweeps", C.c_uint64 * 2), ("swept_cols", C.c_uint64 * 2), ("swept_cells", C.c_uint64 * 2),
+                ("hint_shift_repeats", C.c_uint64), ("dom_width", C.c_int32), ("dom_width2", C.c_int32)]
+
+
 class DeviceView(C.Structure):
     _fields_ = [("n_blocks", C.c_int32), ("n_seqs", C.c_int64), ("n_bases", C.c_int64),
                 ("status", C.c_void_p), ("n_nodes", C.c_void_p), ("n_edges", C.c_void_p),
@@ -96,7 +101,7 @@
 EXPORTS = ["sxg_poa_path_sgd_order", "sxg_poa_kmer_jaccard_batch", "sxg_poa_split_mash_batch", "sxg_poa_pair_identity_batch", "sxg_poa_split_batch", "sxg_poa_split_free", "sxg_poa_batch_device_view", "sxg_poa_abi_version", "sxg_poa_device_count", "sxg_poa_last_error", "sxg_poa_create",
            "sxg_poa_destroy", "sxg_poa_batch_run", "sxg_poa_batch_upload", "sxg_poa_batch_execute",
            "sxg_poa_batch_download", "sxg_poa_batch_free", "sxg_poa_align_batch", "sxg_poa_align_free",
-           "sxg_poa_get_stats", "sxg_poa_set_memory_budget", "sxg_xxh64", "sxg_poa_comm_unique_id", "sxg_poa_comm_init",
+           "sxg_poa_get_stats", "sxg_poa_get_width_stats", "sxg_poa_set_memory_budget", "sxg_xxh64", "sxg_poa_comm_unique_id", "sxg_poa_comm_init",
            "sxg_poa_comm_attach", "sxg_poa_comm_destroy", "sxg_poa_batch_run_sharded", "sxg_poa_batch_run_sharded_local",
            "sxg_poa_batch_upload_sharded", "sxg_poa_batch_execute_sharded", "sxg_poa_batch_download_sharded", "sxg_poa_sharded_info",
            "sxg_poa_sharded_timing", "sxg_poa_measure_copy", "sxg_poa_roctx_available"]
@@ -129,6 +134,7 @@
     L.sxg_poa_align_batch.argtypes = [vp, C.POINTER(AlignIn), C.POINTER(AlignOut)]
     L.sxg_poa_align_free.argtypes = [C.POINTER(AlignOut)]
     L.sxg_poa_get_stats.argtypes = [vp, C.POINTER(Stats)]
+    L.sxg_poa_get_width_stats.argtypes = [vp, C.POINTER(WidthStats)]
     L.sxg_poa_set_memory_budget.argtypes = [vp, C.c_uint64]
     L.sxg_poa_measure_copy.argtypes = [vp, C.c_uint64, C.c_int, C.POINTER(C.c_double)]
     L.sxg_poa_comm_unique_id.argtypes = [C.POINTER(C.c_uint8)]
@@ -261,7 +267,12 @@
     def stats(self):
         s = Stats()
         self.lib.sxg_poa_get_stats(self.h, C.byref(s))
-        return {f[0]: getattr(s, f[0]) for f in Stats._fields_}
+        st = {f[0]: getattr(s, f[0]) for f in Stats._fields_}
+        w = WidthStats()
+        self.lib.sxg_poa_get_width_stats(self.h, C.byref(w))
+        st.update(width_sweeps=tuple(w.sweeps), width_swept_cols=tuple(w.swept_cols), width_swept_cells=tuple(w.swept_cells),
+                  hint_shift_repeats=w.hint_shift_repeats, dom_width=w.dom_width, dom_width2=w.dom_width2)
+        return st
 
     def device_view(self):
         v = DeviceView()
```

After: 689.2 (median of 6 runs). 1.02x the previous value.
